# nanoporetech/scrappie

Measured on AMD Instinct MI355X. Metric: raw samples/sec, rgrgr_r94 4k-sample reads, higher is better.
Workload: dtype f32 (3xf16 split products, 22-bit operands, fp32 accumulate)

## Files before the change

### include/scrappie_hip.h

```cpp
#ifndef SCRAPPIE_HIP_H
#define SCRAPPIE_HIP_H

#include <stdbool.h>
#include <stddef.h>
#include <stdint.h>

#ifdef __cplusplus
extern "C" {
#endif


typedef struct {
    char *uuid;
    size_t n;
    size_t start;
    size_t end;
    float *raw;
} raw_table;

typedef struct {
    uint64_t start;
    float length;
    float mean;
    float stdv;
// ... 216 lines not shown
                             const uint64_t *offsets, const uint32_t *lengths, size_t n,
                             const scrappie_hip_params *p);
int scrappie_hip_collect(scrappie_hip_engine *e, const scrappie_hip_params *p,
                         scrappie_hip_call *out, size_t n);

void scrappie_hip_free_calls(scrappie_hip_call *calls, size_t n);

typedef struct { const int *seq; size_t seqlen; const size_t *poslow, *poshigh; } scrappie_hip_map_target;
typedef struct { float score; size_t nblock; int32_t *path; } scrappie_hip_map_result;
int scrappie_hip_read_blocks(scrappie_hip_engine *e, int model, size_t nsample);
int scrappie_hip_model_states(scrappie_hip_engine *e, int model);
int scrappie_hip_map_batch(scrappie_hip_engine *e, int model, const raw_table *reads, const scrappie_hip_map_target *targets,
                           size_t n, const scrappie_hip_params *p, int viterbi, int want_path, scrappie_hip_map_result *out);
void scrappie_hip_free_map_results(scrappie_hip_map_result *r, size_t n);
void scrappie_hip_map_timing(scrappie_hip_engine *e, double out[3]);
size_t scrappie_hip_map_lds_max_seq(void);

typedef struct { const scrappie_hip_map_target *cand; size_t ncand; } scrappie_hip_map_candidates;
typedef struct { float *score; size_t ncand; int best; size_t nblock; int32_t *path; } scrappie_hip_map_multi_result;
int scrappie_hip_map_multi_batch(scrappie_hip_engine *e, int model, const raw_table *reads, const scrappie_hip_map_candidates *cands,
                                 size_t n, const scrappie_hip_params *p, int viterbi, int want_path, scrappie_hip_map_multi_result *out);
void scrappie_hip_free_map_multi_results(scrappie_hip_map_multi_result *r, size_t n);
int scrappie_hip_map_post_multi(const_scrappie_matrix logpost, float stay_pen, float skip_pen, float local_pen,
                                const scrappie_hip_map_target *cand, size_t ncand, int viterbi, float *score);
long scrappie_hip_map_pack_plan(const size_t *seqlen, size_t ncand, size_t pack_cells, int *pack, long long *cell);
size_t scrappie_hip_map_pack_max_cells(void);
void scrappie_hip_map_pack_form_counts(uint64_t forms[4]);

float map_crf_to_sequence_viterbi(const_scrappie_matrix trans, int const *seq, size_t seqlen, int *path);
float map_crf_to_sequence_forward(const_scrappie_matrix trans, int const *seq, size_t seqlen);
float map_crf_to_sequence_viterbi_banded(const_scrappie_matrix trans, int const *seq, size_t seqlen, size_t const *low, size_t const *high, int *path);
float map_crf_to_sequence_forward_banded(const_scrappie_matrix trans, int const *seq, size_t seqlen, size_t const *low, size_t const *high);
int scrappie_hip_map_crf_bounds_sane(const size_t *low, const size_t *high, size_t nblock, size_t seqlen);
int scrappie_hip_map_crf_diagonal_band(size_t nblock, size_t seqlen, size_t halfwidth, size_t *low, size_t *high);
size_t scrappie_hip_map_crf_lds_max_seq(void);
long long scrappie_hip_map_crf_plan_scratch(const size_t *seqlen, const size_t *nblock, size_t n, long long *off);
void scrappie_hip_map_crf_form_counts(uint64_t forms[8]);

int scrappie_hip_map_crf_multi_batch(scrappie_hip_engine *e, int model, const raw_table *reads, const scrappie_hip_map_candidates *cands,
                                     size_t n, const scrappie_hip_params *p, int viterbi, int want_path, scrappie_hip_map_multi_result *out);
int scrappie_hip_map_trans_multi(const_scrappie_matrix trans, const scrappie_hip_map_target *cand, size_t ncand, int viterbi, float *score);
long scrappie_hip_map_crf_pack_plan(const size_t *seqlen, size_t ncand, size_t pack_cells, int *pack, long long *cell);
size_t scrappie_hip_map_crf_pack_max_cells(void);
void scrappie_hip_map_crf_pack_form_counts(uint64_t forms[4]);

typedef struct { const int *seq; size_t seqlen; } scrappie_hip_map_local_target;
typedef struct { float score; size_t nblock, first, last; int32_t *path; } scrappie_hip_map_local_result;
int scrappie_hip_map_local_batch(scrappie_hip_engine *e, int model, const raw_table *reads, const scrappie_hip_map_local_target *targets,
                                 size_t n, const scrappie_hip_params *p, int viterbi, int want_path, scrappie_hip_map_local_result *out);
void scrappie_hip_free_map_local_results(scrappie_hip_map_local_result *r, size_t n);
float map_crf_to_reference_viterbi(const_scrappie_matrix trans, int const *seq, size_t seqlen, size_t *first, size_t *last, int *path);
float map_crf_to_reference_forward(const_scrappie_matrix trans, int const *seq, size_t seqlen);
long long scrappie_hip_map_crf_local_plan(size_t seqlen, size_t nblock, long stride, size_t cap, size_t *first, size_t *ncell, size_t *own,
                                          int *home, long long *scr_off, long long *scr_floats);
size_t scrappie_hip_map_crf_local_stride(size_t seqlen, size_t nblock, long stride);
size_t scrappie_hip_map_crf_local_max_cells(void);
void scrappie_hip_map_crf_local_form_counts(uint64_t forms[8]);

float map_to_reference_viterbi(const_scrappie_matrix logpost, float stay_pen, float skip_pen, float local_pen, int const *seq, size_t seqlen,
                               size_t *first, size_t *last, int *path);
float map_to_reference_forward(const_scrappie_matrix logpost, float stay_pen, float skip_pen, float local_pen, int const *seq, size_t seqlen);
int scrappie_hip_map_post_local_batch(scrappie_hip_engine *e, int model, const raw_table *reads, const scrappie_hip_map_local_target *targets,
                                      size_t n, const scrappie_hip_params *p, int viterbi, int want_path, scrappie_hip_map_local_result *out);
long long scrappie_hip_map_local_plan(size_t seqlen, size_t nblock, size_t nr, long stride, size_t cap, size_t *first, size_t *ncell, size_t *own,
                                      int *home, long long *scr_off, long long *scr_floats);
size_t scrappie_hip_map_local_stride(size_t seqlen, size_t nblock, size_t nr, long stride);
size_t scrappie_hip_map_local_max_cells(size_t nr);
void scrappie_hip_map_local_form_counts(uint64_t forms[8]);

typedef struct { float *score; int32_t *begin, *end; size_t nmotif; float call_score; int best; size_t nblock; } scrappie_hip_find_result;
int scrappie_hip_find_batch(scrappie_hip_engine *e, int model, const raw_table *reads, const scrappie_hip_map_candidates *motifs, size_t n,
                            const scrappie_hip_params *p, int want_pos, scrappie_hip_find_result *out);
void scrappie_hip_free_find_results(scrappie_hip_find_result *r, size_t n);
int find_crf_sequences_viterbi(const_scrappie_matrix trans, const scrappie_hip_map_target *motif, size_t nmotif, float *score, int32_t *begin,
                               int32_t *end, float *call_score);
long scrappie_hip_crf_find_plan(const size_t *seqlen, size_t nmotif, size_t pack_cells, int *pack, long long *cell);
size_t scrappie_hip_crf_find_max_cells(void);
void scrappie_hip_crf_find_form_counts(uint64_t forms[4]);

typedef struct { const float *params; size_t npos, stride; } scrappie_hip_squiggle_target;
typedef struct { float rate, prob_back, local_pen, skip_pen, minscore; } scrappie_hip_squiggle_params;
typedef struct { float score; size_t n; int32_t *path; } scrappie_hip_squiggle_result;
scrappie_hip_squiggle_params scrappie_hip_default_squiggle_params(void);
int scrappie_hip_squiggle_match_batch(scrappie_hip_engine *e, const raw_table *reads, const scrappie_hip_squiggle_target *targets, size_t n,
                                      const scrappie_hip_squiggle_params *p, int viterbi, int want_path, scrappie_hip_squiggle_result *out);
void scrappie_hip_free_squiggle_results(scrappie_hip_squiggle_result *r, size_t n);
void scrappie_hip_squiggle_timing(scrappie_hip_engine *e, double out[3]);
size_t scrappie_hip_squiggle_lds_max_pos(void);
long long scrappie_hip_map_plan_scratch(const size_t *seqlen, const size_t *nblock, size_t n, long long *off);
long long scrappie_hip_squiggle_plan_scratch(const size_t *npos, const size_t *nsample, size_t n, long long *off);
typedef struct { const int32_t *low; size_t width; } scrappie_hip_squiggle_band;
int scrappie_hip_squiggle_match_banded_batch(scrappie_hip_engine *e, const raw_table *reads, const scrappie_hip_squiggle_target *targets,
                                             const scrappie_hip_squiggle_band *bands, size_t n, const scrappie_hip_squiggle_params *p, int viterbi,
                                             int want_path, scrappie_hip_squiggle_result *out);
size_t scrappie_hip_squiggle_diagonal_band(size_t nsample, size_t npos, size_t halfwidth, int32_t *low);
size_t scrappie_hip_squiggle_band_lds_max_width(void);
long long scrappie_hip_squiggle_band_plan(const size_t *npos, const size_t *width, const size_t *nsample, size_t n, int want_path,
                                          long long *scr_off, long long *tb_off);
void scrappie_hip_squiggle_band_form_counts(uint64_t forms[4]);
int scrappie_hip_squiggle_predict_batch(scrappie_hip_engine *e, const char *model, const int *const *seqs, const size_t *n, size_t count,
                                        int transform_units, scrappie_matrix *out);
void scrappie_hip_sqnet_timing(scrappie_hip_engine *e, double out[3]);
size_t scrappie_hip_sqnet_tile(void);
uint64_t scrappie_hip_sqnet_launch_count(void);

long long scrappie_hip_crf_post_plan(const size_t *nblock, size_t n, long long *off);
int scrappie_hip_posterior_crf_batch(scrappie_hip_engine *e, const const_scrappie_matrix *trans, size_t n, scrappie_matrix *out);
int scrappie_hip_basecall_batch_probs(scrappie_hip_engine *e, int model, const raw_table *reads, size_t n, const scrappie_hip_params *p,
                                      scrappie_hip_call *out, scrappie_matrix *probs);
void scrappie_hip_crf_post_timing(scrappie_hip_engine *e, double out[3]);
uint64_t scrappie_hip_crf_post_launch_count(void);
void scrappie_hip_launch_form_counts(uint64_t map_forms[16], uint64_t squig_forms[4]);

int scrappie_hip_set_decoder_input(scrappie_hip_engine *e, const float *d_prob, const uint64_t *prob_off, size_t n_prob);

int scrappie_hip_set_trunk_input(scrappie_hip_engine *e, const float *d_trunk, const uint64_t *trunk_off, size_t n_trunk);

int scrappie_hip_debug_option(scrappie_hip_engine *e, const char *name, int value);
long scrappie_hip_debug_stitch(scrappie_hip_engine *e, const int *path, const float *side, size_t nblock, int nstate, int crf,
                               char *bases, size_t cap, int *pos, int *redo);
long long scrappie_hip_debug_fetch(scrappie_hip_engine *e, const char *what, void *dst, size_t nbytes);
int scrappie_hip_debug_stitch_dwell(scrappie_hip_engine *e, const int *paths, const int *dwells, const size_t *nentry, size_t nread, int ntrail,
                                    const float *prior_num, int nstate, const size_t *cap, char *bases, size_t bases_bytes, int *lengths, int *pos,
                                    int *redo);
size_t scrappie_hip_dwell_capacity(size_t nentry);

scrappie_matrix scrappie_hip_posterior(scrappie_hip_engine *e, int model, const raw_table signal,
                                       float min_prob, float tempW, float tempb, bool return_log);
scrappie_matrix scrappie_hip_trunk(scrappie_hip_engine *e, int model, const raw_table signal, int upto);

int scrappie_hip_event_features(const event_table events, float *out);
scrappie_matrix scrappie_hip_events_posterior(scrappie_hip_engine *e, int model, const float *feature3, size_t nevent,
                                              float min_prob, float tempW, float tempb, bool return_log);

typedef struct { event_table events; int status; } scrappie_hip_event_result;
int scrappie_hip_detect_events_batch(scrappie_hip_engine *e, const raw_table *reads, size_t n, const detector_param *p,
                                     scrappie_hip_event_result *results);
void scrappie_hip_free_event_results(scrappie_hip_event_result *r, size_t n);
void scrappie_hip_event_timing(scrappie_hip_engine *e, double out[3]);
size_t scrappie_hip_event_tile(void);
uint64_t scrappie_hip_event_launch_count(void);
long long scrappie_hip_events_plan_scratch(const size_t *nsample, size_t n, long long *off);
long scrappie_hip_events_plan_launches(const size_t *nsample, size_t n, size_t budget_slots, uint32_t *order, size_t *starts, size_t cap);
int scrappie_hip_basecall_events_batch(scrappie_hip_engine *e, int model, const raw_table *reads, size_t n, const detector_param *p,
                                       const scrappie_hip_params *params, int dwell_correction, scrappie_hip_call *out);
event_table scrappie_hip_detect_events_host(const float *x, size_t n, const detector_param *p, float *tstat1, float *tstat2);

long scrappie_hip_gru_schedule(const int *tile_T, size_t ntile, int ncu, int *nwg, int *capacity,
                               int *lane_off, int *seg, size_t cap);
long scrappie_hip_lane_schedule(const int *tile_T, size_t ntile, int ncu, int lanes_per_wg, int *nwg, int *capacity,
                                int *lane_off, int *seg, size_t cap);

long scrappie_hip_decoder_pieces(const int *tile_T, size_t ntile, int ncu, int *seg, size_t cap);

size_t scrappie_hip_min_samples(scrappie_hip_engine *e, int model);
int scrappie_hip_model_stride(scrappie_hip_engine *e, int model);
void scrappie_hip_set_profiling(scrappie_hip_engine *e, int on);
int scrappie_hip_get_timing(scrappie_hip_engine *e, scrappie_hip_timing *t);
void scrappie_hip_set_max_launch_reads(scrappie_hip_engine *e, size_t n);
void scrappie_hip_set_max_launch_blocks(scrappie_hip_engine *e, size_t n);
long scrappie_hip_plan_groups(const uint32_t *lengths, size_t n, int stride, size_t max_reads, size_t max_blocks,
                              size_t *starts, size_t cap);
unsigned scrappie_hip_host_thread_budget(void);
unsigned scrappie_hip_host_cpu_budget(void);
void *scrappie_hip_device_alloc(scrappie_hip_engine *e, size_t nbytes);
void scrappie_hip_device_free(scrappie_hip_engine *e, void *dptr);
int scrappie_hip_memcpy_h2d(scrappie_hip_engine *e, void *dst, const void *src, size_t nbytes);
int scrappie_hip_synchronize(scrappie_hip_engine *e);

raw_table scrappie_hip_read_raw(const char *filename, bool scale_to_pA);
typedef float *(*scrappie_hip_sample_alloc)(void *ctx, size_t nsample);
raw_table scrappie_hip_read_raw_into(const char *filename, bool scale_to_pA, scrappie_hip_sample_alloc alloc, void *ctx);
int scrappie_hip_have_hdf5(void);
int scrappie_hip_fast5_scaling(const char *filename, float out[3]);

int scrappie_hip_format_fasta(char *buf, size_t buflen, const char *uuid, const char *readname,
                              bool uuid_primary, const char *prefix, const scrappie_hip_call *res,
                              size_t nsample, size_t trim_start, size_t trim_end);
int scrappie_hip_format_sam(char *buf, size_t buflen, const char *uuid, const char *readname,
                            bool uuid_primary, const char *prefix, const scrappie_hip_call *res);

#ifdef __cplusplus
}
#endif
#endif
```

### scrappie_amd/csrc/scrappie_hip.hip

```cpp
#include <hip/hip_runtime.h>
#include <sched.h>

#include <algorithm>
#include <atomic>
#include <cmath>
#include <cstdarg>
#include <cstdio>
#include <cstdlib>
#include <cstring>
#include <mutex>
#include <numeric>
#include <string>
#include <thread>
#include <type_traits>
#include <vector>
#include <chrono>
#include <condition_variable>
#include <deque>
#include <functional>
#include <map>
#include <memory>
#include <set>

#include "scrappie_hip.h"
// ... 32 lines not shown
    }
};

template <auto K>
static DevOnce &attr_once() { static DevOnce once; return once; }
template <auto K, class... A>
static int launch_k(dim3 grid, dim3 block, size_t lds, hipStream_t s, const A &...a) {
    if (auto turn_ = attr_once<K>().first(lds > 48 * 1024))
        HIPCHK(hipFuncSetAttribute((const void *)K, hipFuncAttributeMaxDynamicSharedMemorySize, 160 * 1024));
    hipLaunchKernelGGL(K, grid, block, lds, s, a...);
    return 0;
}

template <int V> using int_c = std::integral_constant<int, V>;
template <int... Vs, class F>
static bool pick_int(int v, int &rc, F &&f) {
    return ((v == Vs && ((rc = f(int_c<Vs>())), true)) || ...);
}
template <class F>
static int pick_bool(F &&f) { return f(); }
template <class F, class... B>
static int pick_bool(F &&f, bool b, B... rest) {
    return b ? pick_bool([&](auto... c) { return f(std::true_type(), c...); }, rest...)
             : pick_bool([&](auto... c) { return f(std::false_type(), c...); }, rest...);
}

struct StampBuf {
    unsigned long long *d = nullptr;
    int calls = 0;
    unsigned long long *dev(size_t words) {
        if (!d) (void)hipMalloc(&d, words * 8);
        return d;
    }
    template <class P>
    void dump_on(int k, hipStream_t s, size_t words, P &&print) {
        if (k && ++calls != k) return;
        (void)sh_stream_wait(s);
        std::vector<unsigned long long> h(words);
        (void)hipMemcpy(h.data(), d, words * 8, hipMemcpyDeviceToHost);
        print(h.data());
    }
};

struct Tunables {
    bool affine_reg, gru_single, gru_stamp, gru_separate, gru_f32, gru_lanes_stamp, proj_stamp, ff_reg, ff_stamp, vit_stamp, ff_separate, fv_single, host_stamp, host_stitch, split_tail, helper_fence, gru_free, gru_barrier, input_order, conv_valu, conv_in_layer, gru32, gru16, gru32_stamp;
    int gru_debug;
    int conv_tchunk;
    double gru_two_ratio;
    bool fake_timeout;
    Tunables() {
        auto on = [](const char *k) { return getenv(k) != nullptr; };
#ifdef SH_EXPERIMENTS
        auto xon = on;
#else
        auto xon = [](const char *) { return false; };
#endif
        affine_reg = xon("SH_AFFINE_REG"); gru_single = xon("SH_GRU_SINGLE"); gru_stamp = xon("SH_GRU_STAMP");
        gru_separate = on("SH_GRU_SEPARATE"); gru_f32 = on("SH_GRU_F32"); gru_lanes_stamp = xon("SH_GRU_LANES_STAMP");
        proj_stamp = xon("SH_PROJ_STAMP"); ff_reg = xon("SH_FF_REG"); ff_stamp = xon("SH_FF_STAMP"); vit_stamp = xon("SH_VIT_STAMP");
        host_stamp = xon("SH_HOST_STAMP");
        gru_free = xon("SH_GRU_FREE");
        gru_barrier = xon("SH_GRU_BARRIER");
        helper_fence = xon("SH_HELPER_FENCE");
        split_tail = on("SH_SPLIT_TAIL");
        host_stitch = on("SH_HOST_STITCH");
        gru32 = xon("SH_GRU32");
        gru16 = xon("SH_GRU16");
        gru32_stamp = xon("SH_GRU32_STAMP");
        conv_in_layer = xon("SH_CONV_IN_LAYER");
        conv_valu = on("SH_CONV_VALU");
        input_order = xon("SH_INPUT_ORDER");
        ff_separate = on("SH_FF_SEPARATE");
        fv_single = on("SH_FV_SINGLE");
        fake_timeout = on("SH_FAKE_HANDOVER_TIMEOUT");
#ifdef SH_EXPERIMENTS
        const char *dm = getenv("SH_GRU_DEBUG");
#else
        const char *dm = nullptr;
#endif
        gru_debug = dm ? atoi(dm) : -1;
        const char *tc = getenv("SH_CONV_TCHUNK");
        conv_tchunk = tc ? std::max(1, std::min(atoi(tc), 256)) : 16;
        const char *tr = getenv("SH_GRU_TWO_RATIO");
        gru_two_ratio = tr ? atof(tr) : 1.8;
    }
};
static const Tunables &tun() { static const Tunables t; return t; }

#ifndef SH_GRU_FREE_DEFAULT
#define SH_GRU_FREE_DEFAULT 0
#endif
#ifndef SH_AFF_NB
#define SH_AFF_NB 3
#endif
#ifndef SH_AFF_NTH
#define SH_AFF_NTH 512
#endif
#ifndef SH_FF_NB
#define SH_FF_NB 4
#endif

static thread_local char g_err[512] = "";
int sh_set_err_v(const char *fmt, va_list ap) {
    vsnprintf(g_err, sizeof(g_err), fmt, ap);
    return -1;
}
extern "C" const char *scrappie_hip_last_error(void) { return g_err; }
extern "C" void sh_set_error(const char *fmt, ...) {
    va_list ap;
    va_start(ap, fmt);
    (void)sh_set_err_v(fmt, ap);
    va_end(ap);
}

#include "sh_eng_weights.inc"
struct DwellJob {
    bool on = false;
    const int *d_dwell = nullptr;
    std::vector<uint64_t> off;
    std::vector<float> num;
    std::vector<const int *> host;
};

struct PostJob {
    bool on = false;
    std::vector<scrappie_matrix *> dst;
};

struct LaunchGroup {
    PostJob post;
    std::vector<long long> post_off;
    long long npost = 0;
    DwellJob dw;
    size_t n = 0, npad = 0, ntile = 0;
    long long ncb = 0;
    long long nseq = 0;
    long long nhp = 0;
    std::vector<int> order;
    std::vector<int> rT, rN;
    std::vector<long long> tile_boff;
    std::vector<long long> seq_off, hp_off, bases_off;
    long long nbases_cap = 0;
    bool dev_stitch = false;
    bool dev_pos = false;
    int model = -1;
    bool hp_on = false;
    bool valid = false;
    int gru_nwg = 0;
    int gru1_nwg = 0;
    bool gru_two = false;
    int gru32_nwg = 0;
    int gru32x2_nwg = 0;
    int vit_nwg = 0;
    const float *d_signal = nullptr;
    std::vector<uint64_t> in_off;
    std::vector<uint32_t> in_len;
    scrappie_hip_params params{};
};

struct BatchReq {
    scrappie_hip_engine *e = nullptr;
    int model = 0;
    const raw_table *reads = nullptr;
    size_t n = 0;
    scrappie_hip_params p{};
    scrappie_hip_call *out = nullptr;
    int rc = -1;
    std::string err;
    int phase = 0;
};
struct BatchCoalescer : ShCoalescer<BatchReq> { BatchCoalescer() { target_pct = 100; window_mul = 4; } };

struct PostStage { HBuf h; DBuf d; std::atomic<int> users{0}; };

struct DpBufs {
    DBuf rd, tb, scr, score, final_state, path_off, paths;
    HBuf h;
    int ensure(size_t n, size_t rec_bytes, long long tb_words, long long scr_floats, long long path_len, size_t h_bytes = 0, size_t fs_bytes = 4) {
        return (rd.ensure(n * rec_bytes) || tb.ensure((size_t)tb_words * 4 + 16) || scr.ensure((size_t)scr_floats * 4 + 16) || score.ensure(n * 4 + 16) ||
                final_state.ensure(n * fs_bytes + 16) || path_off.ensure(n * 8) || paths.ensure((size_t)path_len * 4 + 16) ||
                h.ensure(std::max(h_bytes, n * 4 + (size_t)path_len * 4))) ? -1 : 0;
    }
};

enum SpanField { F_CONV = 0, F_AFFINE, F_GRU, F_FF, F_DECODE, F_BACKTRACE, F_TOTAL, F_FUSED, F_STITCH,
                 F_WAIT, F_LEAD,
                 F_COUNT };

struct Slot {
    LaunchGroup lg;
    bool pending = false;
    hipEvent_t ev[48] = {};
    int nev = 0;
    struct Span { int field, i, j; };
    std::vector<Span> spans;
    scrappie_hip_timing timing{};
    hipEvent_t done = nullptr;
    hipEvent_t kdone = nullptr;
    hipEvent_t hdone = nullptr;
    hipEvent_t pdone = nullptr;
    hipEvent_t up = nullptr;
    DBuf d_meta, d_signal, d_gflag;
    DBuf d_conv;
    DBuf d_bad;
    DBuf d_edge;
    DBuf d_fscore, d_seq, d_hp;
    DBuf d_pos, d_bases, d_blen, d_redo;
    DBuf d_dwmeta; HBuf h_dwmeta;
    DBuf d_post, d_postoff; HBuf h_post, h_postoff;
    hipEvent_t pev[5] = {};
    HBuf h_meta, h_sig, h_err, h_bad, h_edge, h_seq, h_score, h_hp, h_pos, h_bases, h_blen, h_redo;
    size_t pinned_bytes() const {
        size_t tot = 0;
        for (const HBuf *h : {&h_meta, &h_sig, &h_err, &h_bad, &h_edge, &h_seq, &h_score, &h_hp, &h_pos, &h_bases, &h_blen, &h_redo, &h_dwmeta, &h_post, &h_postoff}) tot += h->cap;
        return tot;
    }
    bool create_events() {
        bool ok = true;
        for (auto &x : ev) ok &= hipEventCreate(&x) == hipSuccess;
        for (hipEvent_t *x : {&done, &kdone, &hdone, &pdone, &up}) ok &= hipEventCreateWithFlags(x, hipEventDisableTiming) == hipSuccess;
        return ok;
    }
    ~Slot() {
        for (auto &x : ev) if (x) (void)hipEventDestroy(x);
        for (auto &x : pev) if (x) (void)hipEventDestroy(x);
        for (hipEvent_t x : {done, kdone, hdone, pdone, up}) if (x) (void)hipEventDestroy(x);
    }
};

struct AltInput {
    const float *data = nullptr;
    std::vector<uint64_t> off;
    DBuf d_off;
    uint64_t key = 0; bool valid = false;
    explicit operator bool() const { return data != nullptr; }
    int set(const char *who, const float *d, const uint64_t *o, size_t n) {
        valid = false;
        if (!d) { data = nullptr; off.clear(); return 0; }
        if (!o || n == 0) return set_err("%s: no offsets", who);
        data = d; off.assign(o, o + n);
        return 0;
    }
};

struct scrappie_hip_engine {
    int device = 0;
    hipStream_t stream = nullptr;
    hipStream_t cstream = nullptr;
    hipStream_t ustream = nullptr;
    hipStream_t pstream = nullptr;
    size_t total_mem = (size_t)64 << 30;
    size_t max_launch_blocks = 0;
    std::vector<Model *> models;
    size_t max_launch_reads = 16384;
    bool profiling = false;
    scrappie_hip_timing timing{};
    bool ev_ok = false;
    Slot slots[2];
    int cur = 0;
    int oldest = 0;
    Slot &current() { return slots[cur]; }
    Slot &other(const Slot &sl) { return slots[&sl == &slots[0] ? 1 : 0]; }
    int index(const Slot &sl) const { return (int)(&sl - slots); }
    bool any_pending() const { return slots[0].pending || slots[1].pending; }
    void drain() {
        (void)sh_stream_wait(pstream); (void)sh_stream_wait(stream); (void)sh_stream_wait(cstream);
        slots[0].pending = slots[1].pending = false;
    }
    DBuf d_hstate, d_vstate, d_vflag;
    DBuf d_act[3];
    DBuf d_xaff, d_E, d_sums, d_tb, d_tbend, d_fstate;
    int ncu = 256;
    bool handover = true;
    AltInput alt_prob; DBuf d_Ealt, d_sums_alt;
    AltInput alt_trunk; DBuf d_act_alt;
    bool dbg_ff_separate = false;
    bool dbg_fv_single = false;
    bool dbg_dump_final = false;
    int dbg_fail_run = 0;
    bool dbg_redo_all = false;
    bool dbg_dwell_tight = false;
    int dbg_gru_tiles = 0;
    int dbg_decoder_cus = 0;
    bool dbg_force_f32 = false;
    int dbg_gru32 = -1;
    scrappie_hip_engine *tail = nullptr;
    scrappie_hip_engine *tail2 = nullptr;
    bool is_tail = false;
    int tail_mode = -1;
    int dbg_fail_tail = 0;
    double mem_frac = 0.7;
    struct Blob { std::string name; std::vector<unsigned char> bytes; bool force_f32; };
    std::vector<Blob> blobs;
    unsigned long long n_tail_calls = 0, n_tail_reads = 0;
    struct TailTicket {
        long id = 0; int model = 0; scrappie_hip_params p{};
        std::vector<raw_table> reads; std::vector<scrappie_hip_call> calls;
        std::vector<float> own;
        int rc = 0; std::string err; bool done = false;
    };
    std::thread tail_th, tail_th2;
    bool tail_th_live = false, tail_th2_live = false, tail_stop = false;
    int tail_busy = 0;
    std::mutex tail_mu;
    std::condition_variable tail_cv;
    std::deque<std::shared_ptr<TailTicket>> tail_q;
    std::map<long, std::shared_ptr<TailTicket>> tail_open;
    long tail_next = 1;
    unsigned long long n_redo_tail = 0;
    unsigned long long n_tail_groups = 0;
    unsigned host_thread_budget = 0;
    unsigned long long n_redo = 0;
    struct Carry { bool live = false; int slot = 0; std::vector<uint32_t> perm; scrappie_hip_call *out = nullptr; scrappie_hip_params p{}; } carry;
    std::mutex mu;
    double tail_frac = 0.3;
    double dbg_tail_free_frac = 0;
    BatchCoalescer batch_co;
    ShPresence batch_presence;
    PostStage post_stage[2]; unsigned post_turn = 0;
    HBuf h_dec_in, h_dec_out; DBuf d_dec[7];
    HBuf h_crf_in, h_crf_out; DBuf d_crf[4];
    DpBufs dp_map; DBuf d_map_seq, d_map_band, d_map_post;
    DBuf d_mpk_rd, d_mpk_cell, d_mpk_first, d_mpk_score; HBuf h_mpk;
    int map_pack_cells = -1;
    DpBufs dp_mcl; DBuf d_mcl_seq, d_mcl_first;
    DpBufs dp_ml; DBuf d_ml_seq, d_ml_lohi;
    int map_local_stride = -1;
    DBuf d_cfd_rd, d_cfd_cell, d_cfd_score, d_cfd_pos, d_cfd_call; HBuf h_cfd;
    int crf_find_cells = -1;
    DBuf d_mcp_rd, d_mcp_cell, d_mcp_score; HBuf h_mcp;
    int map_crf_pack_cells = -1;
    int map_crf_local_stride = -1;
    double map_ms[3] = {0, 0, 0};
    DpBufs dp_sq; DBuf d_sq_sig, d_sq_tab;
    double squig_ms[3] = {0, 0, 0};
    DBuf d_sqn[2]; HBuf h_sqn;
    double sqnet_ms[3] = {0, 0, 0};
    DBuf d_ev_sig, d_ev_rd, d_ev_sum, d_ev_sumsq, d_ev_t1, d_ev_t2, d_ev_peaks, d_ev_np, d_ev_off, d_ev_out; HBuf h_ev, h_ev_out;
    double event_ms[3] = {0, 0, 0};
    HBuf h_cp_in, h_cp_out; DBuf d_cp_in, d_cp_out;
    double crf_post_ms[3] = {0, 0, 0};
    size_t dbg_events_budget = 0;
    size_t dbg_sqnet_budget = 0;
    size_t dbg_squig_budget = 0;
    std::mutex call_mu;
    ~scrappie_hip_engine() {
        for (Model *m : models) delete m;
        for (hipStream_t st : {stream, cstream, ustream, pstream}) if (st) (void)hipStreamDestroy(st);
    }
};

static int pick_mt(int mtiles) {
    for (int mt : {6, 4, 3, 2}) if (mtiles % mt == 0) return mt;
    return 1;
}

static void hw_queue_default() {
    static std::once_flag once;
    std::call_once(once, [] { (void)setenv("GPU_MAX_HW_QUEUES", "8", 0); });
}

static int device_count(hipError_t *why) {
    hw_queue_default();
    int n = 0;
    const hipError_t rc = hipGetDeviceCount(&n);
    if (why) *why = rc;
    return rc == hipSuccess ? n : 0;
}
extern "C" int scrappie_hip_device_count(void) { return device_count(nullptr); }
extern "C" int scrappie_hip_device_numa_node(int device) { return sh_device_numa_node(device); }

extern "C" scrappie_hip_engine *scrappie_hip_engine_create(int device) {
    hipError_t why = hipSuccess;
    int n = device_count(&why);
    if (n <= 0) {
        std::string first, second;
        if (FILE *maps = fopen("/proc/self/maps", "r")) {
            char line[1024];
            while (fgets(line, sizeof line, maps)) {
                const char *path = strchr(line, '/');
                if (!path || !strstr(path, "libamdhip64")) continue;
                std::string s(path, strcspn(path, "\n"));
                if (first.empty()) first = s; else if (s != first && second.empty()) second = s;
            }
            fclose(maps);
        }
        if (!second.empty())
            set_err("no HIP device visible (hipGetDeviceCount: %s): two HIP runtimes are loaded in this process (%s and %s); load the "
                    "other user of HIP (e.g. import torch) before this library, see INTEGRATION.md", hipGetErrorString(why), first.c_str(), second.c_str());
        else set_err("no HIP device visible (hipGetDeviceCount: %s)", hipGetErrorString(why));
        return nullptr;
    }
    if (device < 0 || device >= n) { set_err("device %d out of range (have %d)", device, n); return nullptr; }
    if (hipSetDevice(device) != hipSuccess) { set_err("hipSetDevice(%d) failed", device); return nullptr; }
    hipDeviceProp_t prop;
    int ncu = 256;
    size_t total_mem = (size_t)64 << 30;
    if (hipGetDeviceProperties(&prop, device) == hipSuccess) {
        if (prop.multiProcessorCount > 0) ncu = prop.multiProcessorCount;
        if (prop.totalGlobalMem > 0) total_mem = prop.totalGlobalMem;
        if (strncmp(prop.gcnArchName, "gfx950", 6) != 0) {
            set_err("device %d is %s; this library is built for gfx950 (MI355X) only", device, prop.gcnArchName);
            return nullptr;
        }
    }
    (void)tun();
    scrappie_hip_engine *e = new scrappie_hip_engine();
    e->device = device;
    e->ncu = ncu;
    e->total_mem = total_mem;
    { const char *h = getenv("SCRAPPIE_HIP_HANDOVER"); if (h && atoi(h) == 0) e->handover = false; }
    int prio_lo = 0, prio_hi = 0;
    (void)hipDeviceGetStreamPriorityRange(&prio_lo, &prio_hi);
#ifdef SH_EXPERIMENTS
    if (!getenv("SH_STREAM_PRIO"))
#endif
    prio_lo = prio_hi = 0;
    if (hipStreamCreateWithPriority(&e->stream, hipStreamNonBlocking, prio_hi) != hipSuccess ||
        hipStreamCreateWithPriority(&e->cstream, hipStreamNonBlocking, prio_lo) != hipSuccess ||
        hipStreamCreateWithPriority(&e->pstream, hipStreamNonBlocking, prio_lo) != hipSuccess ||
        hipStreamCreateWithFlags(&e->ustream, hipStreamNonBlocking) != hipSuccess) {
        set_err("hipStreamCreate failed");
        delete e;
        return nullptr;
    }
    e->ev_ok = true;
    for (Slot &sl : e->slots) if (!sl.create_events()) e->ev_ok = false;
    return e;
}

extern "C" void scrappie_hip_engine_destroy(scrappie_hip_engine *e) {
    if (!e) return;
    if (e->tail_th_live) {
        { std::lock_guard<std::mutex> lk(e->tail_mu); e->tail_stop = true; }
        e->tail_cv.notify_all();
        e->tail_th.join();
// ... 41 lines not shown
```

### scrappie_amd/csrc/sh_decode.h

```cpp
#ifndef SH_DECODE_H
#define SH_DECODE_H

struct ShVitArgs {
    const float *E;
    const float *sums;
    long long strideT;
    int strideQ, strideB;
    int want_log;
    float min_prob, stay_pen, skip_pen, local_pen;
    int use_slip;
    unsigned *tb;
    int *tb_end;
    int *final_state;
    float *final_score;
    float *hp_side;
    const long long *hp_off;
    unsigned long long *dbg;
    const ShGruSegD *seg;
    float *vstate;
    unsigned *flag;
    unsigned *err;
    int dump_final;
};

__device__ __forceinline__ void argmax_merge(float &v, int &i, float ov, int oi) {
    const bool take = (ov > v) | ((ov == v) & (oi < i));
    v = take ? ov : v;
    i = take ? oi : i;
}

__device__ __forceinline__ void rows_argmax(float &bv, int &bi) {
    float ov = __shfl_xor(bv, 16); int oi = __shfl_xor(bi, 16);
    argmax_merge(bv, bi, ov, oi);
    ov = __shfl_xor(bv, 32); oi = __shfl_xor(bi, 32);
    argmax_merge(bv, bi, ov, oi);
}

#ifndef SH_FVT_GAP
#define SH_FVT_GAP 4.76837158203125e-07f
#endif
#ifndef SH_MAX4_ASM
#define SH_MAX4_ASM 1
#endif
__device__ __forceinline__ float d_max4(const f32x4 v) {
#if !SH_MAX4_ASM
    return __builtin_fmaxf(__builtin_fmaxf(v[0], v[1]), __builtin_fmaxf(v[2], v[3]));
#endif
    float t;
    asm("v_max3_f32 %0, %1, %2, %3" : "=v"(t) : "v"(v[0]), "v"(v[1]), "v"(v[2]));
    asm("v_max_f32 %0, %1, %2" : "=v"(t) : "v"(t), "v"(v[3]));
    return t;
}

#define SH_CODE_LT(E, codes, a, b, x)                                                                                       \
    asm("v_cmp_lt_f32 vcc, %1, %2\n\tv_cndmask_b32_sdwa %0, %0, %3, vcc dst_sel:BYTE_" #E                                   \
        " dst_unused:UNUSED_PRESERVE src0_sel:BYTE_" #E " src1_sel:BYTE_0"                                                  \
        : "+v"(codes) : "v"(a), "v"(b), "v"(x) : "vcc")

#ifndef SH_VIT_RING
#define SH_VIT_RING 4
#endif
template <int NTH, int PPT, bool FIN, bool SLIP, bool SKIP0>
__global__ __launch_bounds__(NTH, NTH / 256) void k_viterbi(ShVitArgs a, ShMeta md) {
    constexpr int RING = (PPT >= SH_VIT_RING) ? SH_VIT_RING : PPT;
    constexpr int QSTR = NTH / 16, NW = NTH / 64;
    constexpr int NQ = QSTR * PPT, NH = 4 * NQ;
    constexpr int NSKIP = NH / 16, NSLIP = (NH / 64 > 0) ? NH / 64 : 1;
    extern __shared__ __attribute__((aligned(16))) float smem[];
    float *scA = smem;
    float *scB = scA + NH * 16;
    float *skv = scB + NH * 16;
    int *ski = (int *)(skv + NSKIP * 16);
    float *slv = (float *)(ski + NSKIP * 16);
    int *sli = (int *)(slv + NSLIP * 16);
    float *redv = (float *)(sli + NSLIP * 16);
    int *redi = (int *)(redv + 2 * NW * 16);

    const int tid = threadIdx.x, b = tid & 15, qq = tid >> 4, wave = tid >> 6, lane = tid & 63;
    const float mp = a.min_prob, mpm1 = 1.0f - a.min_prob;
    const float slip_pen = (float)(2.0 * a.skip_pen);
    constexpr bool slip = SLIP && (NH / 64 > 0);
    unsigned long long vA = 0, vB = 0, vC = 0, vD = 0, vt0 = 0, vt1;
    long long vblocks = 0;
#define VSTAMP(acc) do { if (a.dbg) { vt1 = __builtin_readcyclecounter(); acc += vt1 - vt0; vt0 = vt1; } } while (0)

    int tile = blockIdx.x, s0 = 0, s1 = -1, ord = 0;
    if (a.seg) { const ShGruSegD sg = a.seg[blockIdx.x]; tile = sg.tile; s0 = sg.s0; s1 = sg.s1; ord = sg.pad; }
    tile = __builtin_amdgcn_readfirstlane(tile); s0 = __builtin_amdgcn_readfirstlane(s0); s1 = __builtin_amdgcn_readfirstlane(s1);
    const int Tt = __builtin_amdgcn_readfirstlane(md.tile_T[tile]);
    if (s1 < 0) s1 = Tt;
    const long long boff = __builtin_amdgcn_readfirstlane((int)md.tile_boff[tile]);
    const int rd = tile * 16 + b;
    const int myT = md.rT[rd];
    float pstart = 0.0f, pend = -SH_BIG;
    if (s0 == 0) {
#pragma unroll
        for (int i = 0; i < PPT; i++)
            *(f32x4 *)(scA + ((qq + QSTR * i) * 16 + b) * 4) = (f32x4){-SH_BIG, -SH_BIG, -SH_BIG, -SH_BIG};
        if (lane < 16) { redv[wave * 16 + b] = -SH_BIG - a.local_pen; redi[wave * 16 + b] = 4 * wave; }
    } else {
        if (tid == 0) {
            if (!sh_wait_flag(a.flag + tile, (unsigned)ord, a.err)) __hip_atomic_store(a.err, 1u, __ATOMIC_RELAXED, __HIP_MEMORY_SCOPE_AGENT);
        }
        __syncthreads();
        __builtin_amdgcn_fence(__ATOMIC_ACQUIRE, "agent");
        const float *vst = a.vstate + (long long)tile * (NH * 16 + 32);
        float bv = -INFINITY;
        int bi = 0x7fffffff;
#pragma unroll
        for (int i = 0; i < PPT; i++) {
            const int Q = qq + QSTR * i;
            const f32x4 pv = *(const f32x4 *)(vst + (Q * 16 + b) * 4);
            *(f32x4 *)(scA + (Q * 16 + b) * 4) = pv;
            {
                const float ve = __builtin_fmaxf(__builtin_fmaxf(pv[0], pv[1]), __builtin_fmaxf(pv[2], pv[3])) - a.local_pen;
                bi = (ve > bv) ? Q : bi;
                bv = __builtin_fmaxf(bv, ve);
            }
        }
        pstart = vst[NH * 16 + b];
        pend = vst[NH * 16 + 16 + b];
        float ov = __shfl_xor(bv, 16); int oi = __shfl_xor(bi, 16);
        argmax_merge(bv, bi, ov, oi);
        ov = __shfl_xor(bv, 32); oi = __shfl_xor(bi, 32);
        argmax_merge(bv, bi, ov, oi);
        if (lane < 16) { redv[((s0 & 1) * NW + wave) * 16 + b] = bv; redi[((s0 & 1) * NW + wave) * 16 + b] = bi; }
    }
    __syncthreads();
    float *cur = scA, *nxt = scB;

    f32x4 ring[RING];
    float stay_nx = 0.f, sum_nx = 1.f;
    float hp_nx[4] = {0.f, 0.f, 0.f, 0.f};
    const bool hp_lane = FIN && a.hp_side && qq == 0;
    auto fetch = [&](int t) {
        const float *Ecb = a.E + (boff + t) * a.strideT + b * a.strideB;
        stay_nx = Ecb[NQ * a.strideQ];
        if (FIN) sum_nx = a.sums[(boff + t) * 16 + b];
        if (hp_lane) {
#pragma unroll
            for (int k = 0; k < 4; k++) {
                const int s = k * ((NH - 1) / 3);
                hp_nx[k] = Ecb[(s >> 2) * a.strideQ + (s & 3)];
            }
        }
    };
    const unsigned eofs = (unsigned)(b * a.strideB + qq * a.strideQ);
    const unsigned tofs = (unsigned)(qq * 16 + b);
    auto qload = [&](int t, int i) {
        const float *base = a.E + (boff + t) * a.strideT + (long long)(QSTR * i) * a.strideQ;
        return *(const f32x4 *)(base + eofs);
    };
    if (s1 > s0) {
        fetch(s0);
#pragma unroll
        for (int i = 0; i < RING; i++) ring[i] = qload(s0, i);
    }
    if (a.dbg) vt0 = __builtin_readcyclecounter();
    vblocks += s1 - s0;

    for (int t = s0; t < s1; t++) {
        const long long cb = boff + t;
        const int par = t & 1;
        float stay_lp = stay_nx;
        const float rmf = d_rcp(sum_nx) * mpm1;

        for (int p = tid; p < NSKIP * 16; p += NTH) {
            const int j = p >> 4, bb = p & 15;
            float v = cur[((j >> 2) * 16 + bb) * 4 + (j & 3)];
            int ri = 0;
#pragma unroll
// ... 811 lines not shown
```

### scrappie_amd/csrc/sh_decode_teams.h

```cpp
#ifndef SH_DECODE_TEAMS_H
#define SH_DECODE_TEAMS_H

#ifndef SH_FVT_WBUF
#define SH_FVT_WBUF 3
#endif
#ifndef SH_FVT_PROD_PRIO
#define SH_FVT_PROD_PRIO 1
#endif
#ifndef SH_FVT_ABL
#define SH_FVT_ABL 0
#endif
#ifndef SH_FVT_FLIP
#define SH_FVT_FLIP 3
#endif
#ifndef SH_FVT_STAMP
#ifdef SH_EXPERIMENTS
#define SH_FVT_STAMP 1
#else
#define SH_FVT_STAMP 0
#endif
#endif
__device__ __forceinline__ unsigned long long end_key(float v, int i) {
    const unsigned u = __builtin_bit_cast(unsigned, v);
    const unsigned hi = u ^ ((unsigned)((int)u >> 31) | 0x80000000u);
    return ((unsigned long long)hi << 32) | (unsigned)~i;
}
__device__ __forceinline__ void end_unkey(unsigned long long k, float &v, int &i) {
    const unsigned hi = (unsigned)(k >> 32);
    v = __builtin_bit_cast(float, hi ^ (~(unsigned)((int)hi >> 31) | 0x80000000u));
    i = (int)~(unsigned)k;
}

#define SH_FVT_NTH 768
#define SH_FVT_LDS_FLOATS (1024 * 16 + 64 * 256 + 2 * 64 * 16 + 2 * 2 * 8 * 16 + 4 * 9 * 16 + 65 * 16 + 2 * 3 * 512 + 3 * 2 * 4 * 4 + 16 * 4 + 4 * 16)

template <bool SKIP0, bool DIV, bool NOCLAMP = false>
__global__ __launch_bounds__(SH_FVT_NTH) void k_ff_viterbi_teams(ShFfArgs f, ShVitArgs a, ShMeta md) {
    static_assert(!(DIV && NOCLAMP), "with temperatures the clamp stays");
    constexpr int NCW = 8, NPW = 4, PPT = 8, NQ = 256, NH = 1024, KS = 3, KQ = 6, TPP = 16, HT = 8, NG = 9, WB = SH_FVT_WBUF;
    static_assert(SH_SUM_GROUP == HT, "half a pass of a producer is one row-sum group");
    static_assert(WB >= 2 && WB <= 4, "weight ring");
    extern __shared__ __attribute__((aligned(16))) float smem[];
    float *sc = smem;
    float *ring = sc + NH * 16;
    float *skk = ring + 64 * 256;
    float *redv = skk + 2 * 64 * 16;
    int *redi = (int *)(redv + 2 * NCW * 16);
    typedef __attribute__((address_space(3))) unsigned long long *ldsk;
    ldsk redk = (ldsk)redv;
    float *gsum = (float *)(redi + 2 * NCW * 16);
    float *sBias = gsum + 4 * NG * 16;
    unsigned *xp = (unsigned *)(sBias + 65 * 16);
    unsigned *sStay = xp + 2 * KS * 512;
    float *rec = (float *)(sStay + KS * 2 * 4 * 4);
    float *pendl = rec + 16 * 4;
    int *pT = (int *)(pendl + 16);
    long long *phpo = (long long *)(pT + 16);

    const int tid = threadIdx.x, lane = tid & 63, b = lane & 15, q = lane >> 4;
    const int wave = __builtin_amdgcn_readfirstlane(tid >> 6);
    const bool decoder = wave < NCW;
    const float mp = a.min_prob, mpm1 = 1.0f - a.min_prob;
    const float lbound = (mp > 0.0f) ? 1.0e-3f - __logf(mp) : INFINITY;
    const float lbgap = lbound * SH_FVT_GAP;
    unsigned long long vA = 0, vB = 0, vC = 0, vD = 0, vt0 = 0, vt1 = 0;
    (void)vt0; (void)vt1;
#undef VSTAMP
#if SH_FVT_STAMP
#define VSTAMP(acc) do { if (a.dbg) { vt1 = __builtin_readcyclecounter(); acc += vt1 - vt0; vt0 = vt1; } } while (0)
#else
#define VSTAMP(acc) do { } while (0)
#endif

    if (tid < KS * 2 * 4 * 4) sStay[tid] = f.wpiece[(long long)(64) * KS * 512 + (tid >> 4) * 256 + ((tid >> 2) & 3) * 64 + (tid & 3)];
    for (int j = tid; j < 65 * 16; j += SH_FVT_NTH) sBias[j] = f.bfrag[((j >> 4) * 64 + ((j >> 2) & 3) * 16) * 4 + (j & 3)];

    int tile = blockIdx.x, s0 = 0, s1 = -1, ord = 0;
    if (a.seg) { const ShGruSegD sg = a.seg[blockIdx.x]; tile = sg.tile; s0 = sg.s0; s1 = sg.s1; ord = sg.pad; }
    tile = __builtin_amdgcn_readfirstlane(tile); s0 = __builtin_amdgcn_readfirstlane(s0); s1 = __builtin_amdgcn_readfirstlane(s1);
    const int Tt = __builtin_amdgcn_readfirstlane(md.tile_T[tile]);
    if (s1 < 0) s1 = Tt;
    const long long boff = __builtin_amdgcn_readfirstlane((int)md.tile_boff[tile]);
    const int rd = tile * 16 + b;
    int myT = md.rT[rd];
    asm volatile("" : "+v"(myT));
    const long long hpo = a.hp_side ? a.hp_off[rd] : 0;
    float pstart = 0.0f, pend = -SH_BIG;

    const int cw = decoder ? wave : 0;
    float *myq = sc + cw * 256 + lane * 4;
    const float *mye = ring + cw * 512 + lane * 4;
    const float *mysrc = sc + cw * 64 + b * 4 + q;
#define SH_FVT_MT(i) (16 * ((i) >> 1) + 8 * ((i) & 1))

    if (s0 == 0) {
        if (decoder) {
#pragma unroll
            for (int i = 0; i < PPT; i++) *(f32x4 *)(myq + SH_FVT_MT(i) * 256) = (f32x4){-SH_BIG, -SH_BIG, -SH_BIG, -SH_BIG};
            if (wave == 0 && lane < 16) { redk[b] = end_key(-SH_BIG - a.local_pen, 0); redk[16 + b] = 0; }
        }
    } else {
        if (tid < 32) redk[tid] = 0;
        if (tid == 0) {
            if (!sh_wait_flag(a.flag + tile, (unsigned)ord, a.err)) __hip_atomic_store(a.err, 1u, __ATOMIC_RELAXED, __HIP_MEMORY_SCOPE_AGENT);
        }
        __syncthreads();
        __builtin_amdgcn_fence(__ATOMIC_ACQUIRE, "agent");
        if (decoder) {
            const float *vst = a.vstate + (long long)tile * (NH * 16 + 32);
            float bv = -INFINITY;
            int bi = 0x7fffffff;
#pragma unroll
            for (int i = 0; i < PPT; i++) {
                const int Q = 4 * (SH_FVT_MT(i) + cw) + q;
                const f32x4 pv = *(const f32x4 *)(vst + (Q * 16 + b) * 4);
                *(f32x4 *)(myq + SH_FVT_MT(i) * 256) = pv;
                {
                    const float ve = __builtin_fmaxf(__builtin_fmaxf(pv[0], pv[1]), __builtin_fmaxf(pv[2], pv[3])) - a.local_pen;
                    bi = (ve > bv) ? Q : bi;
                    bv = __builtin_fmaxf(bv, ve);
                }
            }
            pstart = vst[NH * 16 + b];
            float ov = __shfl_xor(bv, 16); int oi = __shfl_xor(bi, 16);
            argmax_merge(bv, bi, ov, oi);
            ov = __shfl_xor(bv, 32); oi = __shfl_xor(bi, 32);
            argmax_merge(bv, bi, ov, oi);
            if (lane < 16) __hip_atomic_fetch_max(redk + b, end_key(bv, bi), __ATOMIC_RELAXED, __HIP_MEMORY_SCOPE_WORKGROUP);
        } else if (wave == NCW + NPW - 1) pend = (a.vstate + (long long)tile * (NH * 16 + 32))[NH * 16 + 16 + b];
    }

    if (!decoder) {
        const int pw = wave - NCW;
#if SH_FVT_PROD_PRIO
        __builtin_amdgcn_s_setprio(SH_FVT_PROD_PRIO);
#endif
        const unsigned *wmine = f.wpiece + (long long)(TPP * pw) * KS * 512;
        ShSplit W[WB][KS];
        const unsigned lofs = (unsigned)lane * 4u;
        typedef const __attribute__((address_space(1))) unsigned *gu32;
        typedef const __attribute__((address_space(1))) u32x4 *gu32x4;
        gu32 wp = (gu32)wmine;
        auto w_load = [&](int k) {
            static_assert(KS == 3, "two bases per tile: immediate offsets reach 4095 bytes");
            gu32 b0 = wp, b1 = wp + 1024;
            asm volatile("" : "+s"(b0), "+s"(b1));
            W[(k % HT) % WB][0].p1 = __builtin_bit_cast(f16x8, *(gu32x4)(b0 + lofs));
            W[(k % HT) % WB][0].p2 = __builtin_bit_cast(f16x8, *(gu32x4)(b0 + 256 + lofs));
            W[(k % HT) % WB][1].p1 = __builtin_bit_cast(f16x8, *(gu32x4)(b0 + 512 + lofs));
            W[(k % HT) % WB][1].p2 = __builtin_bit_cast(f16x8, *(gu32x4)(b0 + 768 + lofs));
            W[(k % HT) % WB][2].p1 = __builtin_bit_cast(f16x8, *(gu32x4)(b1 + lofs));
            W[(k % HT) % WB][2].p2 = __builtin_bit_cast(f16x8, *(gu32x4)(b1 + 256 + lofs));
            wp = (k == TPP - 1) ? (gu32)wmine : wp + KS * 512;
            asm volatile("" : "+s"(wp));
        };
        auto w_prime = [&](int k0) {
#pragma unroll
            for (int k = 0; k < WB - 1; k++) w_load(k0 + k);
        };
        const int xks = pw < KS ? pw : KS - 1;
        f32x4 xr[2][2];
        auto xraw_load = [&](int u) {
#pragma unroll
            for (int j = 0; j < 2; j++) {
                const float *p = f.in + ((boff + min(u + j, s1 - 1)) * KQ + 2 * xks) * 256;
                xr[j][0] = *(const f32x4 *)(p + lofs);
                xr[j][1] = *(const f32x4 *)(p + 256 + lofs);
            }
        };
        auto xp_publish = [&]() {
            if (pw < KS) {
#pragma unroll
                for (int j = 0; j < 2; j++) {
                    f32x4 v0 = xr[j][0], v1 = xr[j][1];
                    if (DIV) { v0 = v0 / f.in_div; v1 = v1 / f.in_div; }
                    const ShSplit sp = split8(v0, v1);
                    unsigned *d = xp + (j * KS + pw) * 512 + lane * 4;
                    *(u32x4 *)d = __builtin_bit_cast(u32x4, sp.p1);
                    *(u32x4 *)(d + 256) = __builtin_bit_cast(u32x4, sp.p2);
                }
            }
        };
        auto e_of = [&](float acc) { return DIV ? d_exp((acc * SH_OINV) / f.out_div) : NOCLAMP ? d_exp_acc_inrange(acc) : d_exp_acc(acc); };
        auto group_out = [&](float part, int u, int g) {
            const float v = rows_sum(part);
            if (lane < 16) gsum[((u & 3) * NG + g) * 16 + b] = v;
        };
        float *myring = ring + (TPP * pw) * 256 + lane * 4;
        auto s1_half = [&](auto Hc, int u) {
            constexpr int H = decltype(Hc)::value;
#if defined(SH_FVT_DBG_ROLE) && SH_FVT_DBG_ROLE == 1
            return;
#endif
            const float *mybias = sBias + (TPP * pw + HT * H) * 16 + 4 * q;
            ShSplit bp[2][KS];
#pragma unroll
            for (int j = 0; j < 2; j++)
#pragma unroll
                for (int ks = 0; ks < KS; ks++) bp[j][ks] = load_pieces(xp + (j * KS + ks) * 512, lane);
            float part0 = 0.0f, part1 = 0.0f;
            auto tile_out = [&](int k, const f32x4 &acc0, const f32x4 &acc1) {
                f32x4 ex0, ex1;
#pragma unroll
                for (int r = 0; r < 4; r++) { ex0[r] = e_of(acc0[r]); ex1[r] = e_of(acc1[r]); }
                part0 += (ex0[0] + ex0[1]) + (ex0[2] + ex0[3]);
                part1 += (ex1[0] + ex1[1]) + (ex1[2] + ex1[3]);
                if (SH_FVT_ABL & 8) {
#pragma unroll
                    for (int r = 0; r < 4; r++) { ex0[r] = fin_log(ex0[r], mpm1, mp); ex1[r] = fin_log(ex1[r], mpm1, mp); }
                }
                *(f32x4 *)(myring + (2 * k) * 256) = ex0;
                *(f32x4 *)(myring + (2 * k + 1) * 256) = ex1;
            };
#pragma unroll
            for (int k = 0; k < HT; k++) {
                f32x4 acc0 = *(const f32x4 *)(mybias + k * 16), acc1 = acc0;
                if (k + WB - 1 < HT) w_load(HT * H + k + WB - 1);
                const ShSplit (&A)[KS] = W[k % WB];
#pragma unroll
                for (int ks = 0; ks < KS; ks++) { acc0 = mfma16(A[ks].p1, bp[0][ks].p2, acc0); acc1 = mfma16(A[ks].p1, bp[1][ks].p2, acc1); }
#pragma unroll
                for (int ks = 0; ks < KS; ks++) { acc0 = mfma16(A[ks].p2, bp[0][ks].p1, acc0); acc1 = mfma16(A[ks].p2, bp[1][ks].p1, acc1); }
#pragma unroll
                for (int ks = 0; ks < KS; ks++) { acc0 = mfma16(A[ks].p1, bp[0][ks].p1, acc0); acc1 = mfma16(A[ks].p1, bp[1][ks].p1, acc1); }
                tile_out(k, acc0, acc1);
                __builtin_amdgcn_sched_barrier(0);
            }
            group_out(part0, u, 2 * pw + H);
            group_out(part1, u + 1, 2 * pw + H);
            if (H == 1 && pw == NPW - 1) {
                ShSplit Ws[KS];
#pragma unroll
                for (int ks = 0; ks < KS; ks++) {
                    const u32x4 a1 = *(const u32x4 *)(sStay + ((ks * 2 + 0) * 4 + q) * 4), a2 = *(const u32x4 *)(sStay + ((ks * 2 + 1) * 4 + q) * 4);
                    const u32x4 z = {0u, 0u, 0u, 0u};
                    Ws[ks].p1 = __builtin_bit_cast(f16x8, b == 0 ? a1 : z);
                    Ws[ks].p2 = __builtin_bit_cast(f16x8, b == 0 ? a2 : z);
                }
#pragma unroll
                for (int j = 0; j < 2; j++) {
                    f32x4 acc = *(const f32x4 *)(sBias + 64 * 16 + 4 * q);
                    acc = split_dot<KS>(Ws, bp[j], acc);
                    f32x4 ex;
#pragma unroll
                    for (int r = 0; r < 4; r++) ex[r] = (4 * q + r < 1) ? e_of(acc[r]) : 0.0f;
                    group_out((ex[0] + ex[1]) + (ex[2] + ex[3]), u + j, NG - 1);
                }
            }
        };
        auto per_read = [&](const int t, auto par_c) {
            constexpr int par = decltype(par_c)::value;
            int ln = (int)__builtin_amdgcn_mbcnt_hi(~0u, __builtin_amdgcn_mbcnt_lo(~0u, 0u));
            asm volatile("" : "+v"(ln));
            const int b = ln & 15;
            const bool low = ln < 16;
            const int myT = pT[b];
            float pend = pendl[b];
            float tot = 0.0f;
#pragma unroll
            for (int w = 0; w < NG; w++) tot += gsum[((t & 3) * NG + w) * 16 + b];
            const float rmf = d_rcp(tot) * mpm1;
            const float stay_lp = fin_log(gsum[((t & 3) * NG + NG - 1) * 16 + b], rmf, mp);
            const bool active = t < myT;
            if (a.hp_side && active && low) (a.hp_side + (phpo[b] + t) * 5)[4] = stay_lp;
            const float rm = active ? rmf : 0.0f;
            const float mpx = active ? mp : 0.0f;
            const float stay_v = active ? stay_lp - a.stay_pen : 0.0f;
            const float stay_act = stay_lp - a.stay_pen;
            const float hold = fmaxf(-a.local_pen, stay_act);
            if (low) *(f32x4 *)(rec + b * 4) = (f32x4){rm, mpx, stay_v, hold};
            float ev; int ei;
            end_unkey(redk[par * 16 + b], ev, ei);
            redk[par * 16 + b] = 0;
            const f32x4 q4 = *(const f32x4 *)(sc + ((ei & (NQ - 1)) * 16 + b) * 4);
            int e0 = 3;
            e0 = (q4[2] - a.local_pen == ev) ? 2 : e0;
            e0 = (q4[1] - a.local_pen == ev) ? 1 : e0;
            e0 = (q4[0] - a.local_pen == ev) ? 0 : e0;
            const int tbe_in = 4 * ei + e0;
            float nend = pend + hold;
            const bool enter_end = ev > nend;
            nend = enter_end ? ev : nend;
            if (active && low) a.tb_end[(boff + t) * 16 + b] = enter_end ? tbe_in : NH + 1;
            if (active && low) pendl[b] = nend;
        };
        const bool serial = pw == NPW - 1;
        if (serial && lane < 16) { pendl[b] = pend; pT[b] = myT; phpo[b] = hpo; }
        const std::integral_constant<int, 0> H0{};
        const std::integral_constant<int, 1> H1{};

        const bool any = s1 > s0;
        if (any) xraw_load(s0);
        __syncthreads();
        if (any) { xp_publish(); w_prime(0); }
        lds_barrier();
        if (any) s1_half(H0, s0);
        lds_barrier();
        if (any) w_prime(HT);
        lds_barrier();
        if (any) { s1_half(H1, s0); __builtin_amdgcn_sched_barrier(0); xraw_load(s0 + 2); }
        lds_barrier();
        if (a.dbg) vt0 = __builtin_readcyclecounter();
        for (int t = s0; t < s1; t += 2) {
            const bool more = (t + 2 < s1) && !(SH_FVT_ABL & 1);
            if (serial) { per_read(t, H0); __builtin_amdgcn_sched_barrier(0); }
            if (more) { xp_publish(); w_prime(0); }
            VSTAMP(vA);
            lds_barrier();
            VSTAMP(vB);
            if (more) s1_half(H0, t + 2);
            VSTAMP(vC);
            lds_barrier();
            VSTAMP(vD);
            if (serial && t + 1 < s1) { per_read(t + 1, H1); __builtin_amdgcn_sched_barrier(0); }
            if (more) w_prime(HT);
            VSTAMP(vA);
            lds_barrier();
            VSTAMP(vB);
            if (more) s1_half(H1, t + 2);
            __builtin_amdgcn_sched_barrier(0);
            xraw_load(t + 4);
            VSTAMP(vC);
            lds_barrier();
            VSTAMP(vD);
        }
        if (serial && lane < 16 && s1 < Tt) (a.vstate + (long long)tile * (NH * 16 + 32))[NH * 16 + 16 + b] = pendl[b];
        if (s1 < Tt) __builtin_amdgcn_fence(__ATOMIC_RELEASE, "agent");
        __syncthreads();
        if (s1 >= Tt) __syncthreads();
        if (a.dbg && lane == 0) { unsigned long long *d = a.dbg + ((long long)blockIdx.x * 12 + wave) * 8; d[0] = vA; d[1] = vB; d[2] = vC; d[3] = vD; d[4] = (unsigned long long)(s1 - s0); }
        return;
    }
    {
        f32x4 eN[2][PPT];
        auto drain = [&](auto a0, auto s0c, auto a1, auto s1c) {
            constexpr int A0 = decltype(a0)::value, S0 = decltype(s0c)::value, A1 = decltype(a1)::value, S1 = decltype(s1c)::value;
#pragma unroll
            for (int rl = 0; rl < PPT / 2; rl++) { eN[A0][2 * rl + S0] = *(const f32x4 *)(mye + rl * 4096); eN[A1][2 * rl + S1] = *(const f32x4 *)(mye + rl * 4096 + 256); }
        };
        const std::integral_constant<int, 0> I0{};
        const std::integral_constant<int, 1> I1{};
        __syncthreads();
        lds_barrier();
        lds_barrier();
        drain(I0, I0, I1, I0);
        lds_barrier();
        lds_barrier();
        if (a.dbg) vt0 = __builtin_readcyclecounter();
        const unsigned tofs = (unsigned)lane;
        auto block = [&](const int t, auto first_c) {
            constexpr bool FIRST = decltype(first_c)::value;
            const f32x4 (&e)[PPT] = eN[FIRST ? 0 : 1];
            const long long cb = boff + t;
            constexpr int par = FIRST ? 0 : 1;
#if defined(SH_FVT_DBG_ROLE) && SH_FVT_DBG_ROLE == 2
            lds_barrier(); lds_barrier(); return;
#endif
            if (!FIRST && t >= s1) {
                drain(I0, I0, I0, I1);
                lds_barrier(); lds_barrier();
                return;
            }

            float sv[PPT];
            int sr[PPT];
#pragma unroll
            for (int i = 0; i < PPT; i++) {
                float v = mysrc[SH_FVT_MT(i) * 64];
                int ri = (int)SH_TB_STEP;
                if (!(SH_FVT_ABL & 2)) {
#pragma unroll
                    for (int r = 1; r < 4; r++) {
                        const float c = mysrc[(r * 64 + SH_FVT_MT(i)) * 64];
                        const bool up = v < c;
                        v = up ? c : v;
                        ri = up ? (int)SH_TB_STEP + r : ri;
                    }
                }
                sv[i] = v; sr[i] = ri;
                if (i == PPT / 2 - 1) __builtin_amdgcn_sched_barrier(0);
            }
#pragma unroll
            for (int c = 0; c < 2; c++) {
                constexpr int KOFS = (int)SH_TB_SKIP - 4 * (int)SH_TB_STEP;
                float v = sv[c];
                int ri = 4 * sr[c] + KOFS;
                if (!(SH_FVT_ABL & 2)) {
#pragma unroll
                    for (int rl = 1; rl < 4; rl++) argmax_merge(v, ri, sv[2 * rl + c], 4 * sr[2 * rl + c] + (rl + KOFS));
                }
                *(f32x2 *)(skk + ((32 * c + 4 * cw + q) * 16 + b) * 2) = (f32x2){v, __builtin_bit_cast(float, ri)};
            }
            static_assert(SH_TB_STEP + 3u < 8u, "a step code in three bits");
            unsigned srp = 0;
#pragma unroll
            for (int i = 0; i < PPT; i++) srp |= (unsigned)sr[i] << (3 * i);
            __builtin_amdgcn_sched_barrier(0);
            if (FIRST) drain(I0, I1, I1, I1);
            else drain(I0, I0, I0, I1);
            VSTAMP(vA);
            lds_barrier();
            VSTAMP(vB);

            const f32x4 rcd = *(const f32x4 *)(rec + b * 4);
            const float rm = rcd[0], mpx = rcd[1], stay_v = rcd[2], hold = rcd[3];
            const bool active = t < myT;
            const unsigned long long actmask = __builtin_amdgcn_ballot_w64(active);
            const float nstart = pstart + hold;
            float bv = -INFINITY;
            int bi = 0x7fffffff;
            typedef __attribute__((address_space(1))) unsigned *gtb;
            gtb tb0 = (gtb)a.tb + ((cb * NQ + 4 * cw) * 16 + 1024), tb1 = tb0 + 2048;
            asm volatile("" : "+s"(tb0), "+s"(tb1));
            f32x4 pv_n; f32x2 kk_n;
            auto q_fetch = [&](int i) {
                pv_n = *(const f32x4 *)(myq + SH_FVT_MT(i) * 256);
                kk_n = *(const f32x2 *)(skk + ((SH_FVT_MT(i) + cw) * 16 + b) * 2);
            };
            q_fetch(0);
            float hpv[4] = {0.f, 0.f, 0.f, 0.f};
#pragma unroll
            for (int i = 0; i < PPT; i++) {
                const int QB = 4 * (SH_FVT_MT(i) + cw);
                const int Q = QB + q;
                const f32x4 pv = pv_n;
                const float kv = kk_n[0];
                const float krf = kk_n[1];
                const unsigned cskip = __builtin_bit_cast(unsigned, krf);
                if (i + 1 < PPT) q_fetch(i + 1);
                f32x4 l4;
#pragma unroll
                for (int k = 0; k < 4; k++) l4[k] = (SH_FVT_ABL & 24) ? e[i][k] : fin_log(e[i][k], rm, mpx);
#pragma unroll
                for (int k = 0; k < 4; k++) {
                    const int s = k * ((NH - 1) / 3), sq = s >> 2;
                    if (i == 2 * (sq >> 6) + ((sq >> 5) & 1)) hpv[k] = l4[s & 3];
                }
                const float svi = sv[i];
                const unsigned cstep = (srp >> (3 * i)) & 7u;
                const unsigned cstart = SH_TB_START;
                unsigned codes;
                f32x4 ns;
                static_assert(SH_TB_STAY == 0u && SH_TB_STEP + 3u < 256u && SH_TB_SKIP + 15u < 256u && SH_TB_START < 256u,
                              "SH_FVT_LT_FIRST copies all 32 bits of x (cstep, cskip, cstart or cm): every code register is zero above its low byte");
#define SH_FVT_LT_FIRST(E, codes, a, b, x)                                                                      \
                asm("v_cmp_lt_f32 vcc, %1, %2\n\tv_cndmask_b32 %0, 0, %3, vcc" : "=v"(codes) : "v"(a), "v"(b), "v"(x) : "vcc")
#define SH_FVT_STATE(E, LT1)                                                                                    \
                {                                                                                               \
                    float s_ = pv[E] + stay_v;                                                  \
                    const float st = l4[E] + svi;                                           \
                    LT1(E, codes, s_, st, cstep);                                                               \
                    s_ = __builtin_fmaxf(s_, st);                                                               \
                    const float sk = SKIP0 ? l4[E] + kv : (l4[E] + kv) - a.skip_pen;        \
                    SH_CODE_LT(E, codes, s_, sk, cskip);                                                        \
                    s_ = __builtin_fmaxf(s_, sk);                                                               \
                    const float fs = pstart + l4[E];                                  \
                    SH_CODE_LT(E, codes, s_, fs, cstart);                                                       \
                    s_ = __builtin_fmaxf(s_, fs);                                                               \
                    ns[E] = s_;                                                                                 \
                }
                bool fast = false;
                float m = 0.f;
                unsigned cm = cstart;
                if (SKIP0) {
                    m = __builtin_fmaxf(__builtin_fmaxf(svi, kv), pstart);
                    const float md = __builtin_amdgcn_fmed3f(svi, kv, pstart);
                    static_assert(SH_FVT_GAP == 4.76837158203125e-07f, "the fused threshold needs a power of two");
                    const unsigned long long unclear = __builtin_amdgcn_fcmpf(m - md, __builtin_fmaf(__builtin_fabsf(m), SH_FVT_GAP, lbgap), 13 );
                    fast = (unclear & actmask) == 0;
                    cm = (kv == m) ? cskip : cm;
                    cm = (svi == m) ? cstep : cm;
                }
                if (__builtin_expect(fast, true)) {
#define SH_FVT_FAST(E, LT1)                                                                                    \
                    {                                                                                           \
                        const float s_ = pv[E] + stay_v;                                        \
                        const float mv = l4[E] + m;                           \
                        LT1(E, codes, s_, mv, cm);                                                              \
                        ns[E] = __builtin_fmaxf(s_, mv);                                                        \
                    }
                    SH_FVT_FAST(0, SH_FVT_LT_FIRST) SH_FVT_FAST(1, SH_CODE_LT) SH_FVT_FAST(2, SH_CODE_LT) SH_FVT_FAST(3, SH_CODE_LT)
#undef SH_FVT_FAST
                } else { SH_FVT_STATE(0, SH_FVT_LT_FIRST) SH_FVT_STATE(1, SH_CODE_LT) SH_FVT_STATE(2, SH_CODE_LT) SH_FVT_STATE(3, SH_CODE_LT) }
#undef SH_FVT_STATE
#undef SH_FVT_LT_FIRST
                *(f32x4 *)(myq + SH_FVT_MT(i) * 256) = ns;
                gtb tbq = i < PPT / 2 ? tb0 : tb1;
                asm volatile("" : "+s"(tbq));
                if (!(SH_FVT_ABL & 4)) (tbq + (512 * (i % (PPT / 2)) - 1024))[tofs] = codes;
                else asm volatile("" :: "v"(codes));
                {
                    const float ve = d_max4(ns) - a.local_pen;
                    bi = (ve > bv) ? Q : bi;
                    bv = __builtin_fmaxf(bv, ve);
                }
                __builtin_amdgcn_sched_barrier(0);
#if SH_FVT_FLIP
                if (cw >= 4) { if (i == PPT - 1) __builtin_amdgcn_s_setprio(1); else if (i == SH_FVT_FLIP - 1) __builtin_amdgcn_s_setprio(0); }
#endif
            }
            if (active) pstart = nstart;
            if (a.hp_side && active) {
#pragma unroll
                for (int k = 0; k < 4; k++) {
                    const int sq = (k * ((NH - 1) / 3)) >> 2;
                    if (cw == ((sq >> 2) & 7) && q == (sq & 3)) (a.hp_side + (hpo + t) * 5)[k] = hpv[k];
                }
            }
            {
                rows_argmax(bv, bi);
                if (lane < 16) __hip_atomic_fetch_max(redk + ((par ^ 1) * 16 + b), end_key(bv, bi), __ATOMIC_RELAXED, __HIP_MEMORY_SCOPE_WORKGROUP);
            }
            VSTAMP(vC);
            lds_barrier();
            VSTAMP(vD);
        };
        for (int t = s0; t < s1; t += 2) {
            block(t, std::true_type{});
            block(t + 1, std::false_type{});
#pragma unroll
            for (int rl = 0; rl < PPT / 2; rl++) eN[1][2 * rl] = eN[0][2 * rl + 1];
        }
    }

    if (s1 < Tt) {
        if (decoder) {
            float *vst = a.vstate + (long long)tile * (NH * 16 + 32);
#pragma unroll
            for (int i = 0; i < PPT; i++) {
                const int Q = 4 * (SH_FVT_MT(i) + cw) + q;
                *(f32x4 *)(vst + (Q * 16 + b) * 4) = *(const f32x4 *)(myq + SH_FVT_MT(i) * 256);
            }
            if (tid < 16) vst[NH * 16 + b] = pstart;
        }
        __builtin_amdgcn_fence(__ATOMIC_RELEASE, "agent");
        __syncthreads();
        if (tid == 0) __hip_atomic_store(a.flag + tile, (unsigned)ord + 1u, __ATOMIC_RELEASE, __HIP_MEMORY_SCOPE_AGENT);
    } else {
        float bv = -INFINITY;
        int bi = 0x7fffffff;
        if (decoder) {
#pragma unroll
            for (int i = 0; i < PPT; i++) {
                const int Q = 4 * (SH_FVT_MT(i) + cw) + q;
                const f32x4 pv = *(const f32x4 *)(myq + SH_FVT_MT(i) * 256);
#pragma unroll
                for (int k = 0; k < 4; k++) argmax_merge(bv, bi, pv[k], 4 * Q + k);
            }
            float ov = __shfl_xor(bv, 16); int oi = __shfl_xor(bi, 16);
            argmax_merge(bv, bi, ov, oi);
            ov = __shfl_xor(bv, 32); oi = __shfl_xor(bi, 32);
            argmax_merge(bv, bi, ov, oi);
        }
        __syncthreads();
        if (decoder && lane < 16) { redv[wave * 16 + b] = bv; redi[wave * 16 + b] = bi; }
        __syncthreads();
        if (tid < 16) {
            pend = pendl[b];
            float ev = redv[b]; int ei = redi[b];
            for (int w = 1; w < NCW; w++) argmax_merge(ev, ei, redv[w * 16 + b], redi[w * 16 + b]);
            if (pstart > ev) { ev = pstart; ei = NH; }
            if (pend > ev) { ev = pend; ei = NH + 1; }
            a.final_state[rd] = ei;
            a.final_score[rd] = ev;
        }
        if (a.dump_final && a.vstate && decoder) {
            float *vst = a.vstate + (long long)tile * (NH * 16 + 32);
#pragma unroll
            for (int i = 0; i < PPT; i++) {
                const int Q = 4 * (SH_FVT_MT(i) + cw) + q;
                *(f32x4 *)(vst + (Q * 16 + b) * 4) = *(const f32x4 *)(myq + SH_FVT_MT(i) * 256);
            }
            if (tid < 16) { vst[NH * 16 + b] = pstart; vst[NH * 16 + 16 + b] = pend; }
        }
    }
    if (a.dbg && lane == 0) { unsigned long long *d = a.dbg + ((long long)blockIdx.x * 12 + wave) * 8; d[0] = vA; d[1] = vB; d[2] = vC; d[3] = vD; d[4] = (unsigned long long)(s1 - s0); }
#undef VSTAMP
#undef SH_FVT_MT
}

#endif
```

### scrappie_amd/csrc/sh_eng_batch.inc

```

#ifndef SH_CHAIN_NS
#define SH_CHAIN_NS 11400.0
#endif
#ifndef SH_WORK_NS
#define SH_WORK_NS 3.5
#endif
extern "C" long scrappie_hip_plan_tail(const uint32_t *lengths, size_t n, int stride, size_t max_long_blocks, unsigned char *is_long) {
    if ((!lengths && n) || stride < 1 || !is_long) return -1;
    memset(is_long, 0, n);
    if (n < 2) return 0;
    double W = 0;
    std::vector<uint32_t> T(n);
    for (size_t i = 0; i < n; i++) { T[i] = (uint32_t)(((unsigned long long)lengths[i] + stride - 1) / stride); W += T[i]; }
    const double thr = std::max(4096.0, W * SH_WORK_NS / SH_CHAIN_NS);
    std::vector<uint32_t> cand;
    for (size_t i = 0; i < n; i++) if ((double)T[i] > thr) cand.push_back((uint32_t)i);
    if (cand.empty() || cand.size() == n) return 0;
    std::stable_sort(cand.begin(), cand.end(), [&](uint32_t a, uint32_t b) { return T[a] > T[b]; });
    double blocks = 0, work = 0;
    long cnt = 0;
    for (size_t k = 0; k < cand.size(); k++) {
        if (k % 16 == 0) { if (max_long_blocks && blocks + T[cand[k]] > (double)max_long_blocks) break; blocks += T[cand[k]]; }
        if (work + T[cand[k]] > 0.15 * W) break;
        work += T[cand[k]];
        is_long[cand[k]] = 1; cnt++;
    }
    return cnt;
}

static int basecall_batch_one(scrappie_hip_engine *e, int model, const raw_table *reads, size_t n, const scrappie_hip_params *p, scrappie_hip_call *out,
                              scrappie_matrix *probs = nullptr);

static bool tail_two_helpers();
static double tail_mem_frac() {
    static const double f = [] { const char *v = getenv("SCRAPPIE_HIP_TAIL_MEM"); const double x = v ? atof(v) : 0; return x > 0 && x <= 0.4 ? x : (tail_two_helpers() ? 0.15 : 0.3); }();
    return f;
}
static bool tail_two_helpers() {
    static const bool on = [] { const char *v = getenv("SCRAPPIE_HIP_TAIL"); return v && atoi(v) == 2; }();
    return on;
}
static bool tail_enabled(const scrappie_hip_engine *e) {
    if (e->is_tail) return false;
    if (e->tail_mode >= 0) return e->tail_mode != 0;
    static const bool env_on = [] { const char *v = getenv("SCRAPPIE_HIP_TAIL"); return !(v && atoi(v) == 0); }();
    return env_on;
}

static scrappie_hip_engine *make_helper(scrappie_hip_engine *e) {
    scrappie_hip_engine *t = scrappie_hip_engine_create(e->device);
    if (!t) return nullptr;
    t->is_tail = true;
    for (const auto &b : e->blobs) {
        t->dbg_force_f32 = b.force_f32;
        const int want = scrappie_hip_find_model(e, b.name.c_str());
        if (load_model_mem_one(t, b.name.c_str(), b.bytes.data(), b.bytes.size()) != want) { scrappie_hip_engine_destroy(t); set_err("helper engine: model '%s' did not load at index %d", b.name.c_str(), want); return nullptr; }
    }
    return t;
}
static void sync_helper(scrappie_hip_engine *e, scrappie_hip_engine *t) {
    t->handover = e->handover; t->max_launch_reads = e->max_launch_reads; t->max_launch_blocks = e->max_launch_blocks;
    t->dbg_ff_separate = e->dbg_ff_separate; t->dbg_fv_single = e->dbg_fv_single; t->dbg_gru32 = e->dbg_gru32; t->dbg_gru_tiles = e->dbg_gru_tiles; t->dbg_decoder_cus = e->dbg_decoder_cus; t->dbg_redo_all = e->dbg_redo_all;
    t->profiling = false;
}
static scrappie_hip_engine *tail_engine(scrappie_hip_engine *e) {
    if (!e->tail) {
        (void)hipSetDevice(e->device);
        double frac = tail_mem_frac();
        size_t fr = 0, tot = 0;
        if (hipMemGetInfo(&fr, &tot) == hipSuccess && e->total_mem) frac = std::min(frac, 0.85 * (double)fr / (double)e->total_mem);
        if (e->dbg_tail_free_frac > 0) frac = std::min(frac, e->dbg_tail_free_frac);
        if (frac < 0.03) { e->tail_mode = 0; return nullptr; }
        e->tail = make_helper(e);
        if (!e->tail) return nullptr;
        e->mem_frac = 0.45; e->tail->mem_frac = frac; e->tail_frac = frac;
    }
    std::lock_guard<std::mutex> lk(e->tail_mu);
    if (e->tail_busy == 0) {
        sync_helper(e, e->tail);
        if (e->tail2) sync_helper(e, e->tail2);
        if (e->dbg_fail_tail) { e->tail->dbg_fail_run = e->dbg_fail_tail; e->dbg_fail_tail = 0; }
    }
    return e->tail;
}

typedef std::shared_ptr<scrappie_hip_engine::TailTicket> TicketPtr;
static void tail_worker(scrappie_hip_engine *e, scrappie_hip_engine *helper) {
    for (;;) {
        std::unique_lock<std::mutex> lk(e->tail_mu);
        e->tail_cv.wait(lk, [&] { return e->tail_stop || !e->tail_q.empty(); });
        if (e->tail_q.empty()) break;
        std::vector<TicketPtr> batch;
        const TicketPtr f = e->tail_q.front();
        while (!e->tail_q.empty() && e->tail_q.front()->model == f->model && memcmp(&e->tail_q.front()->p, &f->p, sizeof f->p) == 0) {
            batch.push_back(e->tail_q.front());
            e->tail_q.pop_front();
        }
        e->tail_busy++;
        lk.unlock();
        std::vector<raw_table> all;
        for (const TicketPtr &t : batch) all.insert(all.end(), t->reads.begin(), t->reads.end());
        std::vector<scrappie_hip_call> calls(all.size());
        const int rc = basecall_batch_one(helper, f->model, all.data(), all.size(), &f->p, calls.data());
        const std::string err = rc ? std::string(g_err) : std::string();
        lk.lock();
        size_t at = 0;
        for (const TicketPtr &t : batch) {
            t->rc = rc; t->err = err;
            if (!rc) t->calls.assign(calls.begin() + (long)at, calls.begin() + (long)(at + t->reads.size()));
            at += t->reads.size();
            t->done = true;
        }
        e->n_tail_groups++;
        e->n_redo_tail += helper->n_redo; helper->n_redo = 0;
        e->tail_busy--;
        lk.unlock();
        e->tail_cv.notify_all();
    }
}
static TicketPtr tail_submit(scrappie_hip_engine *e, int model, const scrappie_hip_params &p, std::vector<raw_table> &&reads, std::vector<float> &&own = std::vector<float>()) {
    if (!e->tail2 && tail_two_helpers()) {
        bool busy;
        { std::lock_guard<std::mutex> lk(e->tail_mu); busy = e->tail_busy > 0 || !e->tail_q.empty(); }
        if (busy) {
            scrappie_hip_engine *t2 = make_helper(e);
            if (t2) { t2->mem_frac = 0.15; sync_helper(e, t2); std::lock_guard<std::mutex> lk(e->tail_mu); e->tail2 = t2; }
            (void)hipSetDevice(e->device);
        }
    }
    TicketPtr t = std::make_shared<scrappie_hip_engine::TailTicket>();
    t->model = model; t->p = p; t->reads = std::move(reads);
    t->own = std::move(own);
    {
        std::lock_guard<std::mutex> lk(e->tail_mu);
        t->id = e->tail_next++;
        e->tail_open[t->id] = t;
        e->tail_q.push_back(t);
        if (!e->tail_th_live) { e->tail_th = std::thread(tail_worker, e, e->tail); e->tail_th_live = true; }
        else if (e->tail2 && !e->tail_th2_live) { e->tail_th2 = std::thread(tail_worker, e, e->tail2); e->tail_th2_live = true; }
    }
    e->tail_cv.notify_all();
    return t;
}
static void tail_wait(scrappie_hip_engine *e, const TicketPtr &t) {
    std::unique_lock<std::mutex> lk(e->tail_mu);
    e->tail_cv.wait(lk, [&] { return t->done; });
}

static long tail_plan_len(scrappie_hip_engine *e, Model *m, const uint32_t *len, size_t n, std::vector<unsigned char> &is_long) {
    is_long.assign(n, 0);
    if (!tail_enabled(e) || n < 2 || e->alt_prob || e->alt_trunk || e->blobs.size() != e->models.size() || e->dbg_fail_run) return 0;
    const int unit = m->arch == 3 ? 1 : std::max(m->stride, 1);
    const size_t tail_cap = (size_t)((e->tail ? e->tail_frac : tail_mem_frac()) * (double)e->total_mem) / bytes_per_block(m, !decoder_fused(e, m));
    long nl = scrappie_hip_plan_tail(len, n, unit, e->max_launch_blocks ? e->max_launch_blocks : tail_cap, is_long.data());
    if (nl > 0 && !e->tail) {
        if (!tail_engine(e)) {
            if (tail_enabled(e)) return -1;
            is_long.assign(n, 0);
            return 0;
        }
        if (e->tail_frac < tail_mem_frac() && !e->max_launch_blocks) {
            const size_t cap2 = (size_t)(e->tail_frac * (double)e->total_mem) / bytes_per_block(m, !decoder_fused(e, m));
            nl = scrappie_hip_plan_tail(len, n, unit, cap2, is_long.data());
        }
    }
    if (nl > 0 && !tail_engine(e)) return -1;
    return nl;
}
static long tail_plan(scrappie_hip_engine *e, Model *m, const raw_table *reads, size_t n, std::vector<unsigned char> &is_long) {
    const size_t per = m->arch == 3 ? (size_t)m->nfeat : 1;
    std::vector<uint32_t> len(n);
    for (size_t i = 0; i < n; i++) {
        const raw_table &rt = reads[i];
        len[i] = (uint32_t)(((rt.raw && rt.end > rt.start) ? rt.end - rt.start : 0) / per);
    }
    return tail_plan_len(e, m, len.data(), n, is_long);
}

extern "C" long scrappie_hip_basecall_batch_deferred(scrappie_hip_engine *e, int model, const raw_table *reads, size_t n,
                                                     const scrappie_hip_params *p, scrappie_hip_call *out, unsigned char *deferred) {
    if (!e || !reads || !out || !deferred) return set_err("basecall_batch_deferred: null argument");
    Model *m = get_model(e, model);
    if (!m) return -1;
    std::vector<unsigned char> is_long;
    const long nl = tail_plan(e, m, reads, n, is_long);
    if (nl < 0) return -1;
    memset(deferred, 0, n);
    if (nl == 0) return basecall_batch_one(e, model, reads, n, p, out) ? -1 : 0;
    std::vector<raw_table> rl, rr;
    std::vector<size_t> ir;
    for (size_t i = 0; i < n; i++) { if (is_long[i]) rl.push_back(reads[i]); else { rr.push_back(reads[i]); ir.push_back(i); } }
    scrappie_hip_params dp = scrappie_hip_default_params();
    const size_t nlong = rl.size();
    auto tk = tail_submit(e, model, p ? *p : dp, std::move(rl));
    std::vector<scrappie_hip_call> orr(rr.size());
    const int rc_main = basecall_batch_one(e, model, rr.data(), rr.size(), p, orr.data());
    for (size_t i = 0; i < n; i++) { out[i].score = NAN; out[i].nblock = 0; out[i].basecall = nullptr; out[i].basecall_length = 0; out[i].pos = nullptr; }
    if (rc_main) {
        const std::string keep = g_err;
        tail_wait(e, tk);
        if (!tk->rc) scrappie_hip_free_calls(tk->calls.data(), tk->calls.size());
        { std::lock_guard<std::mutex> lk(e->tail_mu); e->tail_open.erase(tk->id); }
        return set_err("%s", keep.c_str());
    }
    for (size_t k = 0; k < ir.size(); k++) out[ir[k]] = orr[k];
    for (size_t i = 0; i < n; i++) deferred[i] = is_long[i];
    e->n_tail_calls++; e->n_tail_reads += nlong;
    return tk->id;
}
static long device_deferred(scrappie_hip_engine *e, int model, const float *d_signal, const uint64_t *offsets, const uint32_t *lengths, size_t n,
                            const scrappie_hip_params *p, scrappie_hip_call *out, unsigned char *deferred, bool stream);
extern "C" long scrappie_hip_basecall_device_deferred(scrappie_hip_engine *e, int model, const float *d_signal, const uint64_t *offsets,
                                                      const uint32_t *lengths, size_t n, const scrappie_hip_params *p, scrappie_hip_call *out,
                                                      unsigned char *deferred) {
    return device_deferred(e, model, d_signal, offsets, lengths, n, p, out, deferred, false);
// ... 348 lines not shown
```

### scrappie_amd/csrc/sh_eng_debug.inc

```

extern "C" int scrappie_hip_set_decoder_input(scrappie_hip_engine *e, const float *d_prob, const uint64_t *prob_off, size_t n_prob) {
    if (!e) return set_err("set_decoder_input: null engine");
    if (e->any_pending()) return set_err("set_decoder_input: launch groups are in flight");
    return e->alt_prob.set("set_decoder_input", d_prob, prob_off, n_prob);
}

extern "C" int scrappie_hip_set_trunk_input(scrappie_hip_engine *e, const float *d_trunk, const uint64_t *trunk_off, size_t n_trunk) {
    if (!e) return set_err("set_trunk_input: null engine");
    if (e->any_pending()) return set_err("set_trunk_input: launch groups are in flight");
    return e->alt_trunk.set("set_trunk_input", d_trunk, trunk_off, n_trunk);
}

static scrappie_hip_engine *default_engine();

extern "C" int scrappie_hip_debug_option(scrappie_hip_engine *e, const char *name, int value) {
    if (!e && name && (!strcmp(name, "map_pack_cells") || !strcmp(name, "map_crf_local_stride") || !strcmp(name, "map_local_stride") || !strcmp(name, "crf_find_cells") || !strcmp(name, "map_crf_pack_cells"))) e = default_engine();
    if (!e || !name) return set_err("debug_option: null argument");
    if (e->any_pending()) return set_err("debug_option: launch groups are in flight");
    if (!strcmp(name, "ff_separate")) e->dbg_ff_separate = value != 0;
    else if (!strcmp(name, "fv_single")) e->dbg_fv_single = value != 0;
    else if (!strcmp(name, "dump_final")) e->dbg_dump_final = value != 0;
    else if (!strcmp(name, "fail_run")) e->dbg_fail_run = value;
    else if (!strcmp(name, "redo_all")) e->dbg_redo_all = value != 0;
    else if (!strcmp(name, "dwell_tight")) e->dbg_dwell_tight = value != 0;
    else if (!strcmp(name, "gru_tiles")) e->dbg_gru_tiles = value;
    else if (!strcmp(name, "decoder_cus")) e->dbg_decoder_cus = value > 0 ? value : 0;
    else if (!strcmp(name, "force_f32_layers")) e->dbg_force_f32 = value != 0;
#ifdef SH_EXPERIMENTS
    else if (!strcmp(name, "gru32")) e->dbg_gru32 = value;
#endif
    else if (!strcmp(name, "tail")) e->tail_mode = value;
    else if (!strcmp(name, "fail_tail")) e->dbg_fail_tail = value;
    else if (!strcmp(name, "tail_free_frac")) e->dbg_tail_free_frac = value / 1000.0;
    else if (!strcmp(name, "squiggle_budget_kb")) e->dbg_squig_budget = value > 0 ? (size_t)value << 10 : 0;
    else if (!strcmp(name, "sqnet_budget_kb")) e->dbg_sqnet_budget = value > 0 ? (size_t)value << 10 : 0;
    else if (!strcmp(name, "map_pack_cells")) e->map_pack_cells = value < 0 ? -1 : value;
    else if (!strcmp(name, "map_crf_local_stride")) e->map_crf_local_stride = value < 0 ? -1 : value;
    else if (!strcmp(name, "map_local_stride")) e->map_local_stride = value < 0 ? -1 : value;
    else if (!strcmp(name, "crf_find_cells")) e->crf_find_cells = value < 0 ? -1 : value;
    else if (!strcmp(name, "map_crf_pack_cells")) e->map_crf_pack_cells = value < 0 ? -1 : value;
    else if (!strcmp(name, "events_budget_samples")) e->dbg_events_budget = value > 0 ? (size_t)value : 0;
    else return set_err("debug_option: unknown option '%s'", name);
    return 0;
}

extern "C" long long scrappie_hip_debug_fetch(scrappie_hip_engine *e, const char *what, void *dst, size_t nbytes) {
    if (!e || !what) return set_err("debug_fetch: null argument");
    (void)hipSetDevice(e->device);
    HIPCHK(sh_stream_wait(e->stream));
    HIPCHK(sh_stream_wait(e->cstream));
    const Slot &sl = e->current(); const LaunchGroup &lg = sl.lg;
    if (!lg.valid) return set_err("debug_fetch: no launch group has run");
    Model *m = get_model(e, lg.model);
    if (!m) return -1;
    const size_t NH = (size_t)std::max(m->NS - 1, 0);
    const void *src = nullptr; size_t have = 0; bool host = false;
    const int gru_tiles = lg.gru_two ? 2 : 1;
    if (!strcmp(what, "tb")) { src = e->d_tb.p; have = (size_t)lg.ncb * NH * 16; }
    else if (!strcmp(what, "tb_end")) { src = e->d_tbend.p; have = (size_t)lg.ncb * 16 * 4; }
    else if (!strcmp(what, "final_state")) { src = e->d_fstate.p; have = lg.npad * 4; }
    else if (!strcmp(what, "final_score")) { src = sl.d_fscore.p; have = lg.npad * 4; }
    else if (!strcmp(what, "final_scores")) { src = e->d_vstate.p; have = lg.ntile * (NH * 16 + 32) * 4; }
    else if (!strcmp(what, "order")) { src = lg.order.data(); have = lg.npad * 4; host = true; }
    else if (!strcmp(what, "tile_boff")) { src = lg.tile_boff.data(); have = lg.ntile * 8; host = true; }
    else if (!strcmp(what, "n_redo")) { static thread_local unsigned long long tot; tot = e->n_redo + e->n_redo_tail; src = &tot; have = 8; host = true; }
    else if (!strcmp(what, "n_tail_groups")) { src = &e->n_tail_groups; have = 8; host = true; }
    else if (!strcmp(what, "n_tail_calls")) { src = &e->n_tail_calls; have = 8; host = true; }
    else if (!strcmp(what, "n_tail_reads")) { src = &e->n_tail_reads; have = 8; host = true; }
    else if (!strcmp(what, "gru_tiles")) { src = &gru_tiles; have = 4; host = true; }
    else if (!strcmp(what, "decoder_pieces")) { src = &lg.vit_nwg; have = 4; host = true; }
    else if (!strcmp(what, "pinned_bytes")) {
        static thread_local unsigned long long tot;
        tot = e->slots[0].pinned_bytes() + e->slots[1].pinned_bytes();
        src = &tot; have = 8; host = true;
    }
    else return set_err("debug_fetch: unknown buffer '%s'", what);
    if (!src && have) return set_err("debug_fetch: buffer '%s' was not allocated", what);
    const size_t cnt = std::min(have, nbytes);
    if (dst && cnt) {
        if (host) memcpy(dst, src, cnt);
        else HIPCHK(hipMemcpy(dst, src, cnt, hipMemcpyDeviceToHost));
    }
    return (long long)have;
}

extern "C" long scrappie_hip_debug_stitch(scrappie_hip_engine *e, const int *path, const float *side, size_t nblock, int nstate, int crf,
                                          char *bases, size_t cap, int *pos, int *redo) {
    if (!e || !path || !bases || nblock == 0) { set_err("debug_stitch: bad argument"); return -2; }
    (void)hipSetDevice(e->device);
    std::lock_guard<std::mutex> lk(e->mu);
    const size_t T = nblock, npad = 64, bcap = 5 * (T + 1) + 8;
    DBuf dmeta, dseq, dhp, dpos, dbases, dblen, dredo;
    std::vector<char> hm(npad * 8 * 3 + npad * 4, 0);
    int *rT = (int *)(hm.data() + npad * 24);
    rT[0] = (int)T;
    if (dmeta.ensure(hm.size()) || dseq.ensure((T + 1) * 4) || dpos.ensure((T + 1) * 4) || dbases.ensure(bcap) ||
        dblen.ensure(npad * 4) || dredo.ensure(npad * 4) || (side && dhp.ensure(T * 5 * 4))) return -2;
    hipStream_t s = e->stream;
    if (hipMemcpyAsync(dmeta.p, hm.data(), hm.size(), hipMemcpyHostToDevice, s) != hipSuccess) return -2;
    if (hipMemcpyAsync(dseq.p, path, (T + 1) * 4, hipMemcpyHostToDevice, s) != hipSuccess) return -2;
    if (side && hipMemcpyAsync(dhp.p, side, T * 5 * 4, hipMemcpyHostToDevice, s) != hipSuccess) return -2;
    if (hipMemsetAsync(dredo.p, 0, npad * 4, s) != hipSuccess) return -2;
    if (sh_stream_wait(s) != hipSuccess) return -2;
    char *d = dmeta.as<char>();
    ShMeta md{};
    md.rT = (const int *)(d + npad * 24);
    ShStitchArgs sa;
    sa.seq = dseq.as<int>(); sa.seq_off = (const long long *)d;
    sa.hp = side ? dhp.as<float>() : nullptr; sa.hp_off = (const long long *)(d + npad * 8);
    sa.pos = pos ? dpos.as<int>() : nullptr;
    sa.bases = dbases.as<char>(); sa.bases_off = (const long long *)(d + npad * 16);
    sa.blen = dblen.as<int>(); sa.redo = dredo.as<unsigned>();
    sa.npad = 1; sa.nstate = nstate; sa.crf = crf; sa.sstride = 1;
    hipLaunchKernelGGL(k_stitch, dim3(1), dim3(64), 0, s, sa, md);
    int len = -1; unsigned rd = 0;
    if (hipMemcpyAsync(&len, dblen.p, 4, hipMemcpyDeviceToHost, s) != hipSuccess) return -2;
    if (hipMemcpyAsync(&rd, dredo.p, 4, hipMemcpyDeviceToHost, s) != hipSuccess) return -2;
    if (sh_stream_wait(s) != hipSuccess) { set_err("debug_stitch: %s", hipGetErrorString(hipGetLastError())); return -2; }
    if (redo) *redo = (int)rd;
    if (len >= 0) {
        if ((size_t)len + 1 > cap) { set_err("debug_stitch: %d bases do not fit %zu bytes", len, cap); return -2; }
        if (len && hipMemcpy(bases, dbases.p, (size_t)len, hipMemcpyDeviceToHost) != hipSuccess) return -2;
        bases[len] = 0;
        if (pos && !crf && hipMemcpy(pos, dpos.p, (T + 1) * 4, hipMemcpyDeviceToHost) != hipSuccess) return -2;
    }
    return len;
}

extern "C" int scrappie_hip_debug_stitch_dwell(scrappie_hip_engine *e, const int *paths, const int *dwells, const size_t *nentry, size_t nread, int ntrail,
                                               const float *prior_num, int nstate, const size_t *cap, char *bases, size_t bases_bytes, int *lengths, int *pos,
                                               int *redo) {
    if (!e || !paths || !dwells || !nentry || !prior_num || !cap || !bases || !lengths || nread == 0 || nread > (1u << 20) || (ntrail != 0 && ntrail != 1))
        return set_err("debug_stitch_dwell: bad argument");
    if (nstate != 5 && nstate != 17 && nstate != 65 && nstate != 257 && nstate != 1025) return set_err("debug_stitch_dwell: %d states (4^k + 1 with k <= 5)", nstate);
    (void)hipSetDevice(e->device);
    std::lock_guard<std::mutex> lk(e->mu);
    const size_t npad = (nread + 63) / 64 * 64;
    std::vector<char> hm(npad * 36, 0);
    long long *seq_off = (long long *)hm.data(), *bases_off = seq_off + npad, *dwell_off = bases_off + npad;
    float *num = (float *)(dwell_off + npad);
    int *nd = (int *)(num + npad), *capi = nd + npad;
    size_t nseq = 0, ndw = 0, nb = 0;
    for (size_t i = 0; i < nread; i++) {
        const size_t c = (cap[i] + 15) & ~(size_t)15;
        if (nentry[i] == 0 || nentry[i] > (1u << 28) || c == 0 || c > (1u << 30)) return set_err("debug_stitch_dwell: read %zu: %zu entries, %zu bytes", i, nentry[i], cap[i]);
        seq_off[i] = (long long)nseq; nseq += nentry[i] + (size_t)ntrail;
        dwell_off[i] = (long long)ndw; ndw += nentry[i];
        bases_off[i] = (long long)nb; nb += c;
        num[i] = prior_num[i]; nd[i] = (int)nentry[i]; capi[i] = (int)c;
    }
    if (nb > bases_bytes) return set_err("debug_stitch_dwell: the reservations take %zu bytes, bases holds %zu", nb, bases_bytes);
    DBuf dmeta, dseq, ddw, dpos, dbases, dblen, dredo;
    if (dmeta.ensure(hm.size()) || dseq.ensure(nseq * 4) || ddw.ensure(ndw * 4) || dpos.ensure(nseq * 4) || dbases.ensure(nb) ||
        dblen.ensure(npad * 4) || dredo.ensure(npad * 4)) return -1;
    hipStream_t s = e->stream;
    HIPCHK(hipMemcpyAsync(dmeta.p, hm.data(), hm.size(), hipMemcpyHostToDevice, s));
    HIPCHK(hipMemcpyAsync(dseq.p, paths, nseq * 4, hipMemcpyHostToDevice, s));
    HIPCHK(hipMemcpyAsync(ddw.p, dwells, ndw * 4, hipMemcpyHostToDevice, s));
    HIPCHK(hipMemsetAsync(dbases.p, 0, nb, s));
    HIPCHK(hipMemsetAsync(dpos.p, 0, nseq * 4, s));
    HIPCHK(hipMemsetAsync(dredo.p, 0, npad * 4, s));
    HIPCHK(sh_stream_wait(s));
    char *d = dmeta.as<char>();
    ShStitchArgs sa{};
    sa.seq = dseq.as<int>(); sa.seq_off = (const long long *)d;
    sa.hp = nullptr; sa.hp_off = nullptr;
    sa.pos = pos ? dpos.as<int>() : nullptr;
    sa.bases = dbases.as<char>(); sa.bases_off = (const long long *)(d + npad * 8);
    sa.blen = dblen.as<int>(); sa.redo = dredo.as<unsigned>();
    sa.npad = (int)nread; sa.nstate = nstate; sa.crf = 0; sa.sstride = 1;
    ShDwellArgs da{};
    da.dwell = ddw.as<int>(); da.dwell_off = (const long long *)(d + npad * 16);
    da.prior_num = (const float *)(d + npad * 24);
    da.nd = (const int *)(d + npad * 28); da.cap = (const int *)(d + npad * 32);
    da.ntrail = ntrail;
    hipLaunchKernelGGL(k_stitch_dwell, dim3((unsigned)(npad / 64)), dim3(64), 0, s, sa, da);
    HIPCHK(hipGetLastError());
    std::vector<unsigned> hredo(nread);
    HIPCHK(hipMemcpyAsync(lengths, dblen.p, nread * 4, hipMemcpyDeviceToHost, s));
    HIPCHK(hipMemcpyAsync(hredo.data(), dredo.p, nread * 4, hipMemcpyDeviceToHost, s));
    HIPCHK(hipMemcpyAsync(bases, dbases.p, nb, hipMemcpyDeviceToHost, s));
    if (pos) HIPCHK(hipMemcpyAsync(pos, dpos.p, nseq * 4, hipMemcpyDeviceToHost, s));
    HIPCHK(sh_stream_wait(s));
    if (redo) for (size_t i = 0; i < nread; i++) redo[i] = (int)hredo[i];
    return 0;
}

extern "C" void scrappie_hip_free_calls(scrappie_hip_call *calls, size_t n) {
    if (!calls) return;
    for (size_t i = 0; i < n; i++) { free(calls[i].basecall); free(calls[i].pos); calls[i].basecall = nullptr; calls[i].pos = nullptr; }
}
```

### scrappie_amd/csrc/sh_eng_launch.inc

```

struct MetaPtrs { ShMeta md; const long long *seq_off, *hp_off, *bases_off; ShGruLanes lanes, lanes1; ShGruPairs pairs, pairs2; const ShGruSegD *vseg; ShDwellArgs dw; };

#define SH_DWELL_PER_ENTRY 10
static long long bases_reservation(long long per_entry, long long nentry) { return (per_entry * nentry + 16 + 15) & ~15ll; }
extern "C" size_t scrappie_hip_dwell_capacity(size_t nentry) { return (size_t)bases_reservation(SH_DWELL_PER_ENTRY, (long long)nentry); }

static int build_group(scrappie_hip_engine *e, Slot &sl, Model *m, const uint64_t *offsets, const uint32_t *lengths,
                       size_t n, bool hp_on, MetaPtrs &mp, const DwellJob *dw = nullptr, const PostJob *pj = nullptr) {
    LaunchGroup &lg = sl.lg;
    lg.valid = false;
    lg.n = n; lg.hp_on = hp_on;
    lg.dw = DwellJob();
    if (dw && dw->on) {
        if (m->arch != 3 || dw->off.size() != n || dw->num.size() != n || dw->host.size() != n) return set_err("build_group: %zu reads, dwells of %zu", n, dw->off.size());
        lg.dw = *dw;
    }
    lg.post = PostJob(); lg.npost = 0;
    if (pj && pj->on) {
        if (m->arch != 1 || pj->dst.size() != n) return set_err("build_group: base probabilities of %zu reads for a group of %zu (flip-flop models only)", pj->dst.size(), n);
        lg.post = *pj;
    }
    lg.ntile = (n + 15) / 16; lg.npad = lg.ntile * 16;
    const int st = m->stride;
    std::vector<int> T(n);
    for (size_t i = 0; i < n; i++)
        T[i] = (lengths[i] >= m->min_samples) ? (int)((lengths[i] + st - 1) / st) : 0;
    lg.order.assign(lg.npad, -1);
    std::vector<int> idx(n);
    std::iota(idx.begin(), idx.end(), 0);
    std::stable_sort(idx.begin(), idx.end(), [&](int a, int b) { return T[a] > T[b]; });
    for (size_t i = 0; i < n; i++) lg.order[i] = idx[i];
    lg.rT.assign(lg.npad, 0); lg.rN.assign(lg.npad, 0);
    lg.seq_off.assign(lg.npad, 0); lg.hp_off.assign(lg.npad, 0); lg.bases_off.assign(lg.npad, 0);
    long long nbases = 0;
    const long long per_entry = (m->arch == 1) ? 1 : (lg.dw.on ? (e->dbg_dwell_tight ? 0 : SH_DWELL_PER_ENTRY) : 5);
    std::vector<unsigned long long> sig_off(lg.npad, 0);
    std::vector<int> tile_T(lg.ntile, 0);
    std::vector<long long> &tile_boff = lg.tile_boff;
    tile_boff.assign(lg.ntile, 0);
    long long ncb = 0, nseq = 0, nhp = 0;
    for (size_t i = 0; i < lg.npad; i++) {
        const int o = lg.order[i];
        if (o >= 0 && T[o] > 0) {
            lg.rT[i] = T[o]; lg.rN[i] = (int)lengths[o]; sig_off[i] = offsets[o];
        }
        lg.hp_off[i] = nhp; nhp += lg.rT[i];
        lg.bases_off[i] = nbases; nbases += lg.rT[i] ? bases_reservation(per_entry, (long long)lg.rT[i] + 1) : 0;
        tile_T[i >> 4] = std::max(tile_T[i >> 4], lg.rT[i]);
    }
    for (size_t t = 0; t < lg.ntile; t++) { tile_boff[t] = ncb; ncb += tile_T[t]; }
    for (size_t t = 0; t < lg.ntile; t++) {
        for (int b = 0; b < 16; b++) lg.seq_off[t * 16 + b] = nseq + b;
        nseq += tile_T[t] ? ((long long)tile_T[t] + 1) * SH_SEQ_STRIDE : 0;
    }
    lg.ncb = ncb; lg.nseq = nseq; lg.nhp = nhp; lg.nbases_cap = nbases;
    ShGruSchedule sched;
    sh_lane_schedule(tile_T.data(), lg.ntile, e->ncu, 2, sched, e->handover);
    lg.gru_nwg = sched.nwg;
    ShGruSchedule sched1;
    sh_lane_schedule(tile_T.data(), lg.ntile, e->ncu, 1, sched1, e->handover);
    lg.gru1_nwg = sched1.nwg;
    { long long nlive = 0; int tmax = 0; for (int t : tile_T) { nlive += t > 0; tmax = std::max(tmax, t); }
      const int w1 = sched1.wg_iter.empty() ? 0 : *std::max_element(sched1.wg_iter.begin(), sched1.wg_iter.end());
      const int w2 = sched.wg_iter.empty() ? 0 : *std::max_element(sched.wg_iter.begin(), sched.wg_iter.end());
      lg.gru_two = nlive > e->ncu && tmax < 65536 && (double)w2 * tun().gru_two_ratio < (double)w1;
      if (e->dbg_gru_tiles == 1) lg.gru_two = false;
      if (e->dbg_gru_tiles == 2 && tmax < 65536) lg.gru_two = true; }
    std::vector<int> pair_tile, pair_T;
    for (size_t t = 0; t < lg.ntile; ) {
        const bool two = t + 1 < lg.ntile && tile_T[t] < (1 << 18) && tile_T[t + 1] > 0;
        pair_tile.push_back((int)t); pair_tile.push_back(two ? (int)t + 1 : -1);
        pair_T.push_back(std::max(tile_T[t], two ? tile_T[t + 1] : 0));
        t += two ? 2 : 1;
    }
    ShGruSchedule sched32;
    sh_lane_schedule(pair_T.data(), pair_T.size(), e->ncu, 1, sched32, e->handover);
    lg.gru32_nwg = sched32.nwg;
    ShGruSchedule sched32b;
    sh_lane_schedule(pair_T.data(), pair_T.size(), e->ncu, 2, sched32b, e->handover);
    lg.gru32x2_nwg = sched32b.nwg;
    std::vector<ShGruSeg> vseg;
    sh_piece_schedule(tile_T.data(), lg.ntile, e->dbg_decoder_cus > 0 ? e->dbg_decoder_cus : e->ncu, vseg, e->handover);
    lg.vit_nwg = (int)vseg.size();
    const size_t b_u64 = lg.npad * 8, b_i32 = lg.npad * 4;
    const size_t b_loff = sched.lane_off.size() * 4, b_seg = sched.seg.size() * sizeof(ShGruSeg), b_wit = sched.wg_iter.size() * 4;
    const size_t b_vloff = 0, b_vseg = vseg.size() * sizeof(ShGruSeg);
    const size_t b_loff1 = sched1.lane_off.size() * 4, b_seg1 = sched1.seg.size() * sizeof(ShGruSeg);
    const size_t b_loff32 = sched32.lane_off.size() * 4, b_seg32 = sched32.seg.size() * sizeof(ShGruSeg), b_pt = pair_tile.size() * 4;
    const size_t b_loff32b = sched32b.lane_off.size() * 4, b_seg32b = sched32b.seg.size() * sizeof(ShGruSeg);
    const size_t total = 4 * b_u64 + lg.ntile * 8 + 2 * b_i32 + lg.ntile * 4 + 16 + b_seg + b_loff + b_wit + 16 + b_vseg + b_vloff + 16 + b_seg1 + b_loff1 +
                         16 + b_seg32 + b_loff32 + b_pt + 16 + b_seg32b + b_loff32b;
    if (sl.h_meta.ensure(total + 16) || sl.d_meta.ensure(total + 16)) return -1;
    char *h = sl.h_meta.as<char>();
    size_t o = 0;
    memcpy(h + o, sig_off.data(), b_u64); const size_t o_sig = o; o += b_u64;
    memcpy(h + o, lg.seq_off.data(), b_u64); const size_t o_seq = o; o += b_u64;
    memcpy(h + o, lg.hp_off.data(), b_u64); const size_t o_hp = o; o += b_u64;
    memcpy(h + o, lg.bases_off.data(), b_u64); const size_t o_bs = o; o += b_u64;
    memcpy(h + o, tile_boff.data(), lg.ntile * 8); const size_t o_tb = o; o += lg.ntile * 8;
    memcpy(h + o, lg.rN.data(), b_i32); const size_t o_n = o; o += b_i32;
    memcpy(h + o, lg.rT.data(), b_i32); const size_t o_t = o; o += b_i32;
    memcpy(h + o, tile_T.data(), lg.ntile * 4); const size_t o_tt = o; o += lg.ntile * 4;
    o = (o + 15) & ~(size_t)15;
    memcpy(h + o, sched.seg.data(), b_seg); const size_t o_seg = o; o += b_seg;
    memcpy(h + o, sched.lane_off.data(), b_loff); const size_t o_loff = o; o += b_loff;
    memcpy(h + o, sched.wg_iter.data(), b_wit); const size_t o_wit = o; o += b_wit;
    o = (o + 15) & ~(size_t)15;
    memcpy(h + o, vseg.data(), b_vseg); const size_t o_vseg = o; o += b_vseg;
    o = (o + 15) & ~(size_t)15;
    memcpy(h + o, sched1.seg.data(), b_seg1); const size_t o_seg1 = o; o += b_seg1;
    memcpy(h + o, sched1.lane_off.data(), b_loff1); const size_t o_loff1 = o; o += b_loff1;
    o = (o + 15) & ~(size_t)15;
    memcpy(h + o, sched32.seg.data(), b_seg32); const size_t o_seg32 = o; o += b_seg32;
    memcpy(h + o, sched32.lane_off.data(), b_loff32); const size_t o_loff32 = o; o += b_loff32;
    memcpy(h + o, pair_tile.data(), b_pt); const size_t o_pt = o; o += b_pt;
    o = (o + 15) & ~(size_t)15;
    memcpy(h + o, sched32b.seg.data(), b_seg32b); const size_t o_seg32b = o; o += b_seg32b;
    memcpy(h + o, sched32b.lane_off.data(), b_loff32b); const size_t o_loff32b = o; o += b_loff32b;
    hipStream_t ps = e->ev_ok ? e->pstream : e->stream;
    if (e->ev_ok) {
        const long long n16 = (long long)((total + 15) / 16);
        hipLaunchKernelGGL(k_upload_words, dim3((unsigned)std::min<long long>((n16 + 255) / 256, 64)), dim3(256), 0, ps, (const u32x4 *)h, sl.d_meta.as<u32x4>(), n16);
    } else HIPCHK(hipMemcpyAsync(sl.d_meta.p, h, total, hipMemcpyHostToDevice, ps));
    char *d = sl.d_meta.as<char>();
    mp.md.sig_off = (const unsigned long long *)(d + o_sig);
    mp.seq_off = (const long long *)(d + o_seq);
    mp.hp_off = (const long long *)(d + o_hp);
    mp.bases_off = (const long long *)(d + o_bs);
    mp.md.tile_boff = (const long long *)(d + o_tb);
    mp.md.rN = (const int *)(d + o_n);
    mp.md.rT = (const int *)(d + o_t);
    mp.md.tile_T = (const int *)(d + o_tt);
    static_assert(sizeof(ShGruSeg) == sizeof(ShGruSegD), "segment layout");
    mp.lanes.seg = (const ShGruSegD *)(d + o_seg);
    mp.lanes.lane_off = (const int *)(d + o_loff);
    mp.lanes.wg_iter = (const int *)(d + o_wit);
    mp.lanes.ntile = (int)lg.ntile;
    mp.vseg = (const ShGruSegD *)(d + o_vseg);
    if (e->d_hstate.ensure(std::max<size_t>(lg.ntile, 1) * 12 * 256 * 4) || sl.d_gflag.ensure((lg.ntile + 1) * 4)) return -1;
    mp.lanes.hstate = e->d_hstate.as<float>();
    mp.lanes.flag = sl.d_gflag.as<unsigned>();
    HIPCHK(hipMemsetAsync(sl.d_gflag.p, 0, (lg.ntile + 1) * 4, ps));
    if (sl.d_bad.ensure(lg.npad * 4)) return -1;
    HIPCHK(hipMemsetAsync(sl.d_bad.p, 0, lg.npad * 4, ps));
    mp.lanes1 = mp.lanes;
    mp.lanes1.seg = (const ShGruSegD *)(d + o_seg1);
    mp.lanes1.lane_off = (const int *)(d + o_loff1);
    mp.lanes1.wg_iter = nullptr;
    mp.pairs.seg = (const ShGruSegD *)(d + o_seg32);
    mp.pairs.lane_off = (const int *)(d + o_loff32);
    mp.pairs.pair_tile = (const int *)(d + o_pt);
    mp.pairs.hstate = mp.lanes.hstate;
    mp.pairs.flag = mp.lanes.flag;
    mp.pairs.err = mp.lanes.flag + lg.ntile;
    mp.pairs2 = mp.pairs;
    mp.pairs2.seg = (const ShGruSegD *)(d + o_seg32b);
    mp.pairs2.lane_off = (const int *)(d + o_loff32b);
    mp.dw = ShDwellArgs{};
    if (lg.dw.on) {
        const size_t np = lg.npad, bytes = (np * 16 + 15) & ~(size_t)15;
        if (sl.h_dwmeta.ensure(bytes) || sl.d_dwmeta.ensure(bytes)) return -1;
        long long *hoff = sl.h_dwmeta.as<long long>();
        float *hnum = (float *)(hoff + np);
        int *hcap = (int *)(hnum + np);
        for (size_t i = 0; i < np; i++) {
            const int o2 = lg.order[i];
            const bool live = o2 >= 0 && lg.rT[i] > 0;
            hoff[i] = live ? (long long)lg.dw.off[(size_t)o2] : 0;
            hnum[i] = live ? lg.dw.num[(size_t)o2] : 0.0f;
            hcap[i] = live ? (int)std::min<long long>(bases_reservation(per_entry, (long long)lg.rT[i] + 1), INT32_MAX & ~15) : 0;
        }
        if (e->ev_ok) hipLaunchKernelGGL(k_upload_words, dim3((unsigned)std::min<size_t>((bytes / 16 + 255) / 256, 64)), dim3(256), 0, ps, (const u32x4 *)sl.h_dwmeta.p, sl.d_dwmeta.as<u32x4>(), (long long)(bytes / 16));
        else HIPCHK(hipMemcpyAsync(sl.d_dwmeta.p, sl.h_dwmeta.p, bytes, hipMemcpyHostToDevice, ps));
        char *dd = sl.d_dwmeta.as<char>();
        mp.dw.dwell = lg.dw.d_dwell;
        mp.dw.dwell_off = (const long long *)dd;
        mp.dw.prior_num = (const float *)(dd + np * 8);
        mp.dw.cap = (const int *)(dd + np * 12);
        mp.dw.nd = mp.md.rT;
        mp.dw.ntrail = 1;
    }
    return 0;
}

template <int KQ>
static int launch_affine_k(hipStream_t s, const float *in, float *out, const float *wf, const unsigned *wp, const float *bf,
                           long long ncb, int mtiles) {
    const int mt = pick_mt(mtiles);
    long long gx = std::min<long long>((ncb + 3) / 4, 2048);
    if (gx < 1) gx = 1;
    dim3 grid((unsigned)gx, (unsigned)(mtiles / mt));
    int rc = 0;
    if (pick_int<6, 4, 3, 2, 1>(mt, rc, [&](auto m) { return launch_k<k_affine<KQ, m()>>(grid, dim3(256), 0, s, in, out, wf, wp, bf, ncb, mtiles); })) return rc;
    return set_err("unsupported layer of %d m-tiles", mtiles);
}

template <int KQ>
static int launch_affine_lds_k(hipStream_t s, const float *in, float *out, const float *wf, const unsigned *wp, const float *bf,
                               long long ncb, int mtiles) {
    constexpr int NB = SH_AFF_NB, NTH = SH_AFF_NTH;
    const size_t lds = ((size_t)mtiles * KQ * 256 + (size_t)mtiles * 256) * 4 + 16;
    long long gx = std::min<long long>((ncb + (NTH / 64) * NB - 1) / ((NTH / 64) * NB), 256);
    if (gx < 1) gx = 1;
    return launch_k<k_affine_lds<KQ, NB, NTH>>(dim3((unsigned)gx), dim3(NTH), lds, s, in, out, wf, wp, bf, ncb, mtiles);
}

template <int KQ>
static int launch_affine_f32_k(hipStream_t s, const float *in, float *out, const float *wf, const float *bf, long long ncb, int mtiles) {
    const int mt = (mtiles % 6 == 0) ? 6 : (mtiles % 2 == 0) ? 2 : 1;
    long long gx = std::min<long long>((ncb + 3) / 4, 2048);
    if (gx < 1) gx = 1;
    dim3 grid((unsigned)gx, (unsigned)(mtiles / mt));
    int rc = 0;
    if (pick_int<6, 2, 1>(mt, rc, [&](auto m) { return launch_k<k_affine<KQ, m(), true>>(grid, dim3(256), 0, s, in, out, wf, (const unsigned *)nullptr, bf, ncb, mtiles); })) return rc;
    return set_err("unsupported layer of %d m-tiles", mtiles);
}

static int launch_affine(hipStream_t s, int K, const float *in, float *out, const float *wf, const unsigned *wp, const float *bf_nat,
                         const float *bf_acc, long long ncb, int mtiles, bool force_f32 = false) {
    int rc = 0;
    if (force_f32 && pick_int<2, 4, 6, 8>(K / 16, rc, [&](auto kq) { return launch_affine_f32_k<kq()>(s, in, out, wf, bf_nat, ncb, mtiles); })) return rc;
    if (K % 32 == 0 && (!wp || !bf_acc)) return set_err("layer weights were not cut into pieces (input size %d)", K);
    const float *bf = (K % 32 == 0) ? bf_acc : bf_nat;
    const size_t lds_need = ((size_t)mtiles * (K / 16) * 256 + (size_t)mtiles * 256) * 4;
    if (mtiles >= 12 && lds_need <= 150 * 1024 && ncb >= 4096 && !tun().affine_reg &&
        pick_int<1, 2, 4, 6>(K / 16, rc, [&](auto kq) { return launch_affine_lds_k<kq()>(s, in, out, wf, wp, bf, ncb, mtiles); })) return rc;
    if (pick_int<1, 2, 4, 6, 8>(K / 16, rc, [&](auto kq) { return launch_affine_k<kq()>(s, in, out, wf, wp, bf, ncb, mtiles); })) return rc;
    return set_err("unsupported layer input size %d (need 16, 32, 64, 96 or 128)", K);
}

template <int KQ>
static int launch_affine2_k(hipStream_t s, const float *inF, const float *inB, float *out, const unsigned *wF, const unsigned *wB,
                            const float *bf, long long ncb, int mtiles) {
    long long gx = std::min<long long>((ncb + 3) / 4, 2048);
    if (gx < 1) gx = 1;
    const int mt = mtiles / 2;
    int rc = 0;
    if (mt * 2 == mtiles &&
        pick_int<3, 2, 1>(mt, rc, [&](auto m) { return launch_k<k_affine2_tanh<KQ, m()>>(dim3((unsigned)gx), dim3(512), 0, s, inF, inB, out, wF, wB, bf, ncb, mtiles); })) return rc;
    return set_err("unsupported joining layer of %d m-tiles", mtiles);
}

static int launch_affine2(hipStream_t s, int K, const float *inF, const float *inB, float *out, const unsigned *wF, const unsigned *wB,
                          const float *bf, long long ncb, int mtiles) {
    int rc = 0;
    if (pick_int<2, 4, 6>(K / 16, rc, [&](auto kq) { return launch_affine2_k<kq()>(s, inF, inB, out, wF, wB, bf, ncb, mtiles); })) return rc;
    return set_err("unsupported bi-GRU size %d (need 32, 64 or 96)", K);
}

static int launch_gru(hipStream_t s, int S, const float *xaff, float *out, const float *resid, const float *sW,
                      const float *sW2, const unsigned *sWp, const unsigned *sW2p, const ShMeta &md, int backward, size_t ntile, const ShGruLanes &lanes, int nwg,
                      bool force_f32 = false) {
    const int NU = S / 16;
    int rc = 0;
    if (!tun().gru_single && !tun().gru_stamp && tun().gru_debug < 0 && NU <= 6 && S % 32 == 0) {
        if (nwg <= 0) return 0;
        HIPCHK(hipMemsetAsync(lanes.flag, 0, (size_t)lanes.ntile * 4, s));
        dim3 lgrid((unsigned)nwg);
        const bool stamp = tun().gru_lanes_stamp;
        const bool f32_env = tun().gru_f32 || force_f32;
        if (!stamp && !f32_env) {
            const size_t plds = (size_t)2 * 2 * (NU / 2) * 2 * 64 * 4 * 4;
            if (pick_int<2, 4, 6>(NU, rc, [&](auto nu) { return launch_k<k_gru_split<nu()>>(lgrid, dim3(128 * nu()), plds, s, xaff, out, resid, sWp, sW2p, md, backward, lanes); })) return rc;
            return set_err("unsupported GRU size %d (need 32, 64 or 96 here)", S);
        }
        const size_t lds = (size_t)2 * 2 * NU * 256 * 4;
        static StampBuf st;
        if (!pick_int<2, 4, 6>(NU, rc, [&](auto nu) {
#ifdef SH_EXPERIMENTS
            if constexpr (nu() == 6)
                if (stamp) return launch_k<k_gru_lanes<6, true>>(lgrid, dim3(768), lds, s, xaff, out, resid, sW, sW2, md, backward, lanes, st.dev(4096 * 16 * 8));
#endif
            return launch_k<k_gru_lanes<nu(), false>>(lgrid, dim3(128 * nu()), lds, s, xaff, out, resid, sW, sW2, md, backward, lanes, (unsigned long long *)nullptr);
            })) return set_err("unsupported GRU size %d (need 32, 64 or 96 here)", S);
        if (stamp && NU == 6)
            st.dump_on(7, s, (size_t)nwg * 12 * 8, [&](const unsigned long long *h) {
                for (size_t g : {(size_t)nwg / 2}) for (int w = 0; w < 12; w++) {
                    const unsigned long long *d = &h[(g * 12 + w) * 8];
                    fprintf(stderr, "gru lanes stamp wg %zu wave %2d: phase1 %.0f bar %.0f phase2 %.0f bar %.0f cycles/step (%llu steps)\n",
                            g, w, d[0] / (double)d[4], d[1] / (double)d[4], d[2] / (double)d[4], d[3] / (double)d[4], d[4]);
                }
            });
        return rc;
    }
    if (tun().gru_debug >= 0) backward |= tun().gru_debug << 8;
    static StampBuf st1;
    unsigned long long *dbgbuf = tun().gru_stamp ? st1.dev(4096 * 8 * 8) : nullptr;
    if (dbgbuf)
        st1.dump_on(8, s, ntile * NU * 8, [&](const unsigned long long *h) {
            { unsigned long long first_end = ~0ull, mn = ~0ull, mx = 0; size_t late = 0;
              for (size_t tl = 0; tl < ntile; tl++) { first_end = std::min(first_end, h[tl * NU * 8 + 7]); mn = std::min(mn, h[tl * NU * 8 + 6]); mx = std::max(mx, h[tl * NU * 8 + 7]); }
// ... 330 lines not shown
```

### scrappie_amd/csrc/sh_eng_load.inc

```

static const HostMat *find_mat(const std::vector<std::pair<std::string, HostMat>> &ms, const char *nm) {
    for (auto &kv : ms) if (kv.first == nm) return &kv.second;
    return nullptr;
}

static int load_model_mem_one(scrappie_hip_engine *e, const char *name, const void *blob, size_t nbytes);
static int sqnet_load(Model *m, const std::vector<std::pair<std::string, HostMat>> &mats);
extern "C" int scrappie_hip_load_model_mem(scrappie_hip_engine *e, const char *name, const void *blob, size_t nbytes) {
    const int idx = load_model_mem_one(e, name, blob, nbytes);
    if (idx < 0 || e->is_tail) return idx;
    scrappie_hip_engine::Blob b{name, std::vector<unsigned char>((const unsigned char *)blob, (const unsigned char *)blob + nbytes), e->dbg_force_f32};
    bool found = false;
    for (auto &x : e->blobs) if (x.name == b.name) { x = b; found = true; }
    if (!found) e->blobs.push_back(b);
    if (e->tail || e->tail2) {
        std::unique_lock<std::mutex> lk(e->tail_mu);
        e->tail_cv.wait(lk, [&] { return e->tail_busy == 0 && e->tail_q.empty(); });
    }
    for (scrappie_hip_engine **tp : {&e->tail, &e->tail2}) if (*tp) {
        (*tp)->dbg_force_f32 = e->dbg_force_f32;
        if (load_model_mem_one(*tp, name, blob, nbytes) != idx) return set_err("model '%s' did not load at the same index on the helper engine", name);
    }
    return idx;
}
// ... 148 lines not shown
                return set_err("model '%s': FF%d has a weight of magnitude %g, outside the split products' range (< %g); "
                               "there is no exact-fp32 kernel for this layer", name, k + 1, mx, (double)SH_W_LIMIT);
            }
            const int mt = (m->S + 15) / 16;
            if (upload_u32(m->ff2W[k][0], make_piece_frags(*wf)) || upload_u32(m->ff2W[k][1], make_piece_frags(*wb)) ||
                upload(m->ff2b[k], scaled(make_bias_frags(*bb, mt), SH_OSCALE))) { delete m; return -1; }
        }
    }
    if (m->S % 32 == 0 && !in_split_range(*fw)) {
        const float mx = max_abs(*fw);
        delete m;
        return set_err("model '%s': the output layer has a weight of magnitude %g, outside the split products' range (< %g); "
                       "there is no exact-fp32 kernel for this layer", name, mx, (double)SH_W_LIMIT);
    }
    {
        double worst = 0.0;
        for (int c = 0; c < fw->nc; c++) {
            double acc = c < (int)fb->v.size() ? fabs((double)fb->v[(size_t)c]) : 0.0;
            for (int r = 0; r < fw->nr; r++) acc += fabs((double)fw->v[(size_t)c * fw->nr + r]);
            worst = std::max(worst, acc);
        }
        m->ff_no_clamp = worst < 88.0;
    }
    if (upload(m->ffW, make_frags(*fw, m->ff_mtiles)) || upload(m->ffb, make_bias_frags(*fb, m->ff_mtiles))) { delete m; return -1; }
    if (m->S % 32 == 0 && (upload_u32(m->ffWp, make_piece_frags(*fw)) || upload(m->ffbs, scaled(make_bias_frags(*fb, m->ff_mtiles), SH_OSCALE)))) { delete m; return -1; }
    if (m->arch == 3) {
        m->min_samples = 2;
    } else {
    ShConvGeom &g = m->geom;
    g = conv_geom(m->WL, m->stride, m->F);
    m->min_samples = (size_t)(g.shiftX + 2 * g.nstepX + g.WL);
    if (m->min_samples < (size_t)(g.st + 1)) m->min_samples = (size_t)(g.st + 1);
    }
    std::lock_guard<std::mutex> lk(e->mu);
    for (size_t i = 0; i < e->models.size(); i++)
        if (e->models[i]->name == name) { delete e->models[i]; e->models[i] = m; return (int)i; }
    e->models.push_back(m);
    return (int)e->models.size() - 1;
}

extern "C" int scrappie_hip_load_model(scrappie_hip_engine *e, const char *name, const char *path) {
    if (!path) return set_err("load_model: null path");
    FILE *fh = fopen(path, "rb");
    if (!fh) return set_err("cannot open model file %s", path);
    fseek(fh, 0, SEEK_END);
    long sz = ftell(fh);
    fseek(fh, 0, SEEK_SET);
    std::vector<unsigned char> buf((size_t)std::max(0L, sz));
    const size_t got = fread(buf.data(), 1, buf.size(), fh);
    fclose(fh);
    if (got != buf.size()) return set_err("short read on %s", path);
    return scrappie_hip_load_model_mem(e, name, buf.data(), buf.size());
}

extern "C" int scrappie_hip_find_model(scrappie_hip_engine *e, const char *name) {
    if (!e || !name) return -1;
    std::lock_guard<std::mutex> lk(e->mu);
    for (size_t i = 0; i < e->models.size(); i++) if (e->models[i]->name == name) return (int)i;
    return -1;
}

static Model *get_model(scrappie_hip_engine *e, int model) {
    if (!e || model < 0 || (size_t)model >= e->models.size()) { set_err("invalid model handle %d", model); return nullptr; }
    if (e->models[model]->arch == 4) { set_err("model '%s' predicts squiggles from sequences; it takes no signal", e->models[model]->name.c_str()); return nullptr; }
    return e->models[model];
}

extern "C" size_t scrappie_hip_min_samples(scrappie_hip_engine *e, int model) {
    Model *m = get_model(e, model);
    return m ? m->min_samples : 0;
}
extern "C" int scrappie_hip_model_stride(scrappie_hip_engine *e, int model) {
    Model *m = get_model(e, model);
    return m ? m->stride : -1;
}
extern "C" void scrappie_hip_set_profiling(scrappie_hip_engine *e, int on) { if (e) e->profiling = on != 0; }
static int resolve_spans(scrappie_hip_engine *e, Slot &sl) {
    scrappie_hip_timing &tm = sl.timing;
    float dbg_wait = 0.f, dbg_lead = 0.f;
    float *fields[F_COUNT] = {&tm.conv_ms, &tm.affine_ms, &tm.gru_ms, &tm.ff_ms, &tm.decode_ms, &tm.backtrace_ms, &tm.total_ms, &tm.fused_ms, &tm.stitch_ms,
                              &dbg_wait, &dbg_lead};
    for (auto &sp : sl.spans) {
        float ms = 0;
        HIPCHK(hipEventElapsedTime(&ms, sl.ev[sp.i], sl.ev[sp.j]));
        *fields[sp.field] += ms;
    }
    sl.spans.clear();
    if (tun().host_stamp) fprintf(stderr, "host stamp: main stream waited %.2f ms for the prologue; the convolution had ended %.2f ms before the main stream got there (negative: after)\n", dbg_wait, dbg_lead);
    e->timing = tm;
    return 0;
}

extern "C" int scrappie_hip_get_timing(scrappie_hip_engine *e, scrappie_hip_timing *t) {
    if (!e || !t) return -1;
    (void)hipSetDevice(e->device);
    Slot &sl = e->current();
    if (!sl.spans.empty() && !sl.pending) {
        HIPCHK(sh_stream_wait(e->stream));
        if (resolve_spans(e, sl)) return -1;
    }
    *t = e->timing;
    return 0;
}
extern "C" void scrappie_hip_set_max_launch_reads(scrappie_hip_engine *e, size_t n) { if (e && n >= 16) e->max_launch_reads = n; }
extern "C" void scrappie_hip_set_max_launch_blocks(scrappie_hip_engine *e, size_t n) { if (e) e->max_launch_blocks = n; }
extern "C" void *scrappie_hip_device_alloc(scrappie_hip_engine *e, size_t nbytes) {
    if (!e) return nullptr;
    (void)hipSetDevice(e->device);
    void *p = nullptr;
    if (hipMalloc(&p, nbytes) != hipSuccess) { set_err("hipMalloc(%zu) failed", nbytes); return nullptr; }
    return p;
}
extern "C" void scrappie_hip_device_free(scrappie_hip_engine *e, void *dptr) {
    if (e && dptr) { (void)hipSetDevice(e->device); (void)hipFree(dptr); }
}
extern "C" int scrappie_hip_memcpy_h2d(scrappie_hip_engine *e, void *dst, const void *src, size_t nbytes) {
    if (!e) return -1;
    (void)hipSetDevice(e->device);
    HIPCHK(hipMemcpy(dst, src, nbytes, hipMemcpyHostToDevice));
    return 0;
}
extern "C" int scrappie_hip_synchronize(scrappie_hip_engine *e) {
    if (!e) return -1;
    (void)hipSetDevice(e->device);
    HIPCHK(sh_stream_wait(e->stream));
    return 0;
}

extern "C" long scrappie_hip_lane_schedule(const int *tile_T, size_t ntile, int ncu, int lanes_per_wg, int *nwg, int *capacity,
                                           int *lane_off, int *seg, size_t cap) {
    if (!tile_T || ncu < 1 || lanes_per_wg < 1 || lanes_per_wg > 2) return -1;
    ShGruSchedule sc;
    sh_lane_schedule(tile_T, ntile, ncu, lanes_per_wg, sc);
    if (nwg) *nwg = sc.nwg;
    if (capacity) *capacity = sc.capacity;
    if (lane_off) memcpy(lane_off, sc.lane_off.data(), sc.lane_off.size() * sizeof(int));
    if (seg) for (size_t i = 0; i < sc.seg.size() && i < cap; i++) memcpy(seg + 4 * i, &sc.seg[i], 16);
    return (long)sc.seg.size();
}

extern "C" long scrappie_hip_gru_schedule(const int *tile_T, size_t ntile, int ncu, int *nwg, int *capacity,
                                          int *lane_off, int *seg, size_t cap) {
    return scrappie_hip_lane_schedule(tile_T, ntile, ncu, 2, nwg, capacity, lane_off, seg, cap);
}

extern "C" long scrappie_hip_decoder_pieces(const int *tile_T, size_t ntile, int ncu, int *seg, size_t cap) {
    if (!tile_T || ncu < 1) return -1;
    std::vector<ShGruSeg> v;
    sh_piece_schedule(tile_T, ntile, ncu, v);
    if (seg) for (size_t i = 0; i < v.size() && i < cap; i++) memcpy(seg + 4 * i, &v[i], 16);
    return (long)v.size();
}

extern "C" long scrappie_hip_plan_groups(const uint32_t *lengths, size_t n, int stride, size_t max_reads, size_t max_blocks,
                                         size_t *starts, size_t cap) {
    if ((!lengths && n) || stride < 1 || max_reads < 1) return -1;
    long ng = 0;
    size_t cnt = 0;
    unsigned long long sumT = 0, maxT = 0;
    for (size_t i = 0; i < n; i++) {
        const unsigned long long T = ((unsigned long long)lengths[i] + stride - 1) / stride;
        if (max_blocks && T / 16 + T + 1 > max_blocks) return -1;
        const unsigned long long ns = sumT + T, nm = std::max(maxT, T);
        if (cnt == 0 || cnt >= max_reads || (max_blocks && ns / 16 + nm + 1 > max_blocks)) {
            if (starts && (size_t)ng < cap) starts[ng] = i;
            ng++;
            cnt = 0; sumT = 0; maxT = 0;
        }
        cnt++; sumT += T; maxT = std::max(maxT, T);
    }
    return ng;
}

static bool decoder_fused(const scrappie_hip_engine *e, const Model *m) {
    return m->NS > 25 && !e->alt_prob && m->NS == 1025 && m->S == 96 && !tun().ff_separate && !e->dbg_ff_separate;
}

static size_t bytes_per_block(const Model *m, bool posterior) {
    const size_t S = (size_t)m->S, F = (size_t)m->F, w = std::max(S, F);
    size_t b = ((m->arch == 2 || m->arch == 3) ? 4 : 3) * w * 64 + 128;
    if (posterior) b += (size_t)m->ff_mtiles * 1024;
    if (m->arch == 3 || F != S || S % 32 || S / 16 > 6) b += (size_t)(m->arch == 3 ? 4 : 3) * S * 64;
    if (m->NS > 25) b += (size_t)((m->NS - 1) / 4) * 64;
    else b += 16 * 4 * 4;
    b += 16 * 2 * (4 + 4 + 20 + 5) + 2 * 16 * 4 * (size_t)std::max(m->stride, 1) * (m->arch == 3 ? (size_t)m->nfeat : 1);
    return b;
}

static size_t launch_block_cap(scrappie_hip_engine *e, const Model *m) {
    if (e->max_launch_blocks) return e->max_launch_blocks;
    return (size_t)(e->mem_frac * (double)e->total_mem) / bytes_per_block(m, !decoder_fused(e, m));
}
```

### scrappie_amd/csrc/sh_eng_pipeline.inc

```

enum StopAt { STOP_NONE = 0, STOP_TRUNK = 1, STOP_POST = 2 };

struct RunOut {
    const float *act = nullptr;
    int act_units = 0;
    const float *E = nullptr;
    const float *sums = nullptr;
};

struct HostStamp {
    const std::chrono::steady_clock::time_point t0 = std::chrono::steady_clock::now();
    void operator()(const char *what, const char *after = "") const {
        if (tun().host_stamp) fprintf(stderr, "host stamp: %s %.2f ms%s\n", what, std::chrono::duration<double, std::milli>(std::chrono::steady_clock::now() - t0).count(), after);
    }
};

struct Marks {
    enum Mark { PROLOGUE_BEGIN, PROLOGUE_END,
                WAIT_BEGIN, MAIN_BEGIN,
                LAYER_BEGIN, LAYER_SPLIT, LAYER_END,
                S1_BEGIN, S1_END, DECODE_END, MAIN_END,
                WALK_BEGIN, WALK_END, STITCH_BEGIN, STITCH_END,
                N_MARKS };
    Slot *sl = nullptr;
// ... 112 lines not shown
                              : areg     ? act(k_conv_mfma<0, 6, 3, true>, k_conv_mfma<1, 6, 3, true>)
                              : kst == 3 ? (bg ? act(k_conv_mfma_bg<0, 6, 3, false>, k_conv_mfma_bg<1, 6, 3, false>) : act(k_conv_mfma<0, 6, 3, false>, k_conv_mfma<1, 6, 3, false>))
                                         : (bg ? act(k_conv_mfma_bg<0, 6, 5, false>, k_conv_mfma_bg<1, 6, 5, false>) : act(k_conv_mfma<0, 6, 5, false>, k_conv_mfma<1, 6, 5, false>));
        if (fake == 1) HIPCHK(hipMemsetAsync(c.abuf[0], 0, c.act_bytes, ps));
        else if (fake != 2) hipLaunchKernelGGL(kern, grid, dim3(256), lds, ps, c.d_signal, c.mp.md, m->conv_W.as<float>(), m->conv_b.as<float>(), m->geom, c.abuf[0], tchunk, sl.d_bad.as<unsigned>());
    }
    if (c.pf.mark(Marks::PROLOGUE_END, ps)) return -1;
    c.pf.span(F_CONV, Marks::PROLOGUE_BEGIN, Marks::PROLOGUE_END);
    c.stamp("prologue enqueued at");
    if (c.pf.mark(Marks::WAIT_BEGIN, s)) return -1;
    if (e->ev_ok && ps != s) { HIPCHK(hipEventRecord(sl.pdone, ps)); HIPCHK(hipStreamWaitEvent(s, sl.pdone, 0)); }
    c.stamp("wait enqueued at");
    if (c.pf.mark(Marks::MAIN_BEGIN, s)) return -1;
    c.pf.span(F_WAIT, Marks::WAIT_BEGIN, Marks::MAIN_BEGIN); c.pf.span(F_LEAD, Marks::PROLOGUE_END, Marks::WAIT_BEGIN);
    if (tun().helper_fence && e->ev_ok && e->other(sl).pending) HIPCHK(hipStreamWaitEvent(s, e->other(sl).hdone, 0));
    return 0;
}

static int recurrent_layer(Slot &sl, Model *m, GroupRun &c, int l, int I, const float *in, float *out, int backward) {
    scrappie_hip_engine *e = c.e;
    const LaunchGroup &lg = sl.lg; const MetaPtrs &mp = c.mp;
    const hipStream_t s = c.s;
    const bool lstm = m->arch == 3;
    const int S = m->S, gates = lstm ? 4 : 3;
    const float *resid = m->arch == 1 ? in : nullptr;
    const bool f32 = !lstm && m->layer_f32[l];
    const bool one_kernel = !tun().gru_separate && (lstm ? (I == S || I == 16) && S % 32 == 0 : gru_proj_ok(I, S) && !f32);
    if (c.pf.mark(Marks::LAYER_BEGIN, s)) return -1;
#ifdef SH_EXPERIMENTS
    if (l == 0 && c.fuse_conv) {
        if (c.pf.mark(Marks::LAYER_SPLIT, s)) return -1;
        ShConvFuse cf;
        cf.sig = c.d_signal; cf.W = m->conv_W.as<float>(); cf.bias = m->conv_b.as<float>(); cf.edge = sl.d_edge.as<int>();
        cf.bad = sl.d_bad.as<unsigned>(); cf.g = m->geom;
        if (launch_gru_conv(s, (m->WL + 3) / 4, m->conv_act, out, m->iWp[l].as<unsigned>(), m->ibs[l].as<float>(), m->sWp[l].as<unsigned>(),
                            m->sW2p[l].as<unsigned>(), mp.md, 1, mp.lanes1, lg.gru1_nwg, mp.lanes, lg.gru_nwg, lg.gru_two, cf)) return -1;
    } else if (!lstm && one_kernel && use_gru32(e) && S == 96 && I == 96 && m->has32) {
        if (c.pf.mark(Marks::LAYER_SPLIT, s)) return -1;
        if (use_gru32(e) == 2 ? launch_gru_proj32x2(s, in, out, m->arch == 1, m->iWp32[l].as<unsigned>(), m->ib32[l].as<float>(), m->sWp32[l].as<unsigned>(),
                                                    m->sW2p32[l].as<unsigned>(), mp.md, backward, mp.pairs2, lg.gru32x2_nwg, lg.ntile)
                              : launch_gru_proj32(s, in, out, m->arch == 1, m->iWp32[l].as<unsigned>(), m->ib32[l].as<float>(), m->sWp32[l].as<unsigned>(),
                                                  m->sW2p32[l].as<unsigned>(), mp.md, backward, mp.pairs, lg.gru32_nwg, lg.ntile)) return -1;
    } else
#endif
    if (one_kernel) {
        if (c.pf.mark(Marks::LAYER_SPLIT, s)) return -1;
        if (lstm ? launch_lstm_proj(s, S, I, in, out, m->iWp[l].as<unsigned>(), m->ibs[l].as<float>(), m->sWp[l].as<unsigned>(), m->lp[l].as<float>(),
                                    mp.md, backward, mp.lanes1, lg.gru1_nwg)
                 : launch_gru_proj(s, S, in, out, resid, m->iWp[l].as<unsigned>(), m->ibs[l].as<float>(), m->sWp[l].as<unsigned>(), m->sW2p[l].as<unsigned>(),
                                   mp.md, backward, mp.lanes1, lg.gru1_nwg, mp.lanes, lg.gru_nwg, lg.gru_two)) return -1;
    } else {
        if (e->d_xaff.ensure((size_t)c.ncb * gates * S * 16 * 4)) return -1;
        if (launch_affine(s, I, in, e->d_xaff.as<float>(), m->iW[l].as<float>(), m->iWp[l].as<unsigned>(), m->ib[l].as<float>(), m->ibs[l].as<float>(), c.ncb, gates * S / 16, f32)) return -1;
        if (c.pf.mark(Marks::LAYER_SPLIT, s)) return -1;
        if (lstm ? launch_lstm(s, S, e->d_xaff.as<float>(), out, m->sWp[l].as<unsigned>(), m->lp[l].as<float>(), mp.md, backward, mp.lanes, lg.gru_nwg)
                 : launch_gru(s, S, e->d_xaff.as<float>(), out, resid, m->sW[l].as<float>(), m->sW2[l].as<float>(), m->sWp[l].as<unsigned>(), m->sW2p[l].as<unsigned>(),
                              mp.md, backward, lg.ntile, mp.lanes, lg.gru_nwg, f32)) return -1;
    }
    if (c.pf.mark(Marks::LAYER_END, s)) return -1;
    c.pf.span(F_AFFINE, Marks::LAYER_BEGIN, Marks::LAYER_SPLIT);
    c.pf.span(F_GRU, Marks::LAYER_SPLIT, Marks::LAYER_END);
    if (c.pf.on) {
        scrappie_hip_timing &tm = sl.timing;
        const double af = 2.0 * I * gates * S * 16.0 * (double)c.ncb, gf = 2.0 * gates * S * S * 16.0 * (double)c.ncb;
        tm.n_affine_launches++; tm.n_gru_launches++; tm.affine_flops += af; tm.gru_flops += gf;
        if (one_kernel) { tm.n_fused_launches++; tm.fused_flops += af + gf; }
    }
    if (one_kernel) c.pf.span(F_FUSED, Marks::LAYER_SPLIT, Marks::LAYER_END);
    return 0;
}

static int stage_trunk(Slot &sl, Model *m, GroupRun &c, int *top) {
    const hipStream_t s = c.s;
    const int S = m->S, F = m->F;
    float **abuf = c.abuf; *top = 0;
    if (m->arch == 2 || m->arch == 3) {
        for (int lvl = 0; lvl < 2 && lvl < c.trunk_upto; lvl++) {
            for (int dir = 0; dir < 2; dir++) if (recurrent_layer(sl, m, c, 2 * lvl + dir, lvl == 0 ? F : S, abuf[0], abuf[1 + dir], dir)) return -1;
            if (c.pf.mark(Marks::LAYER_BEGIN, s)) return -1;
            if (launch_affine2(s, S, abuf[1], abuf[2], abuf[0], m->ff2W[lvl][0].as<unsigned>(), m->ff2W[lvl][1].as<unsigned>(), m->ff2b[lvl].as<float>(), c.ncb, S / 16)) return -1;
            if (c.pf.mark(Marks::LAYER_SPLIT, s)) return -1;
            c.pf.span(F_AFFINE, Marks::LAYER_BEGIN, Marks::LAYER_SPLIT);
            if (c.pf.on) sl.timing.affine_flops += 2.0 * 2 * S * S * 16.0 * (double)c.ncb;
        }
    } else {
        for (int l = 0; l < 5 && l < c.trunk_upto; l++, *top ^= 1)
            if (recurrent_layer(sl, m, c, l, l == 0 ? F : S, abuf[*top], abuf[*top ^ 1], (l % 2 == 0) ? 1 : 0)) return -1;
    }
    HIPCHK(hipGetLastError());
    c.stamp("layers enqueued at");
    return 0;
}

template <class Grow, class Launch>
static int inject_alt(const Slot &sl, GroupRun &c, AltInput &alt, uint64_t seed, Grow grow, Launch launch) {
    const LaunchGroup &lg = sl.lg;
    std::vector<unsigned long long> aoff(lg.npad, ~0ull);
    uint64_t key = 1469598103934665603ull ^ seed;
    for (size_t i = 0; i < lg.npad; i++) {
        const int o = lg.order[i];
        if (o >= 0 && lg.rT[i] > 0) aoff[i] = alt.off[(size_t)o % alt.off.size()];
        key = (key ^ (uint64_t)(aoff[i] + 0x9e3779b97f4a7c15ull * (uint64_t)(lg.rT[i] + 1))) * 1099511628211ull;
    }
    if (alt.valid && key == alt.key) return 0;
    if (grow() || alt.d_off.ensure(lg.npad * 8)) return -1;
    HIPCHK(hipMemcpyAsync(alt.d_off.p, aoff.data(), lg.npad * 8, hipMemcpyHostToDevice, c.s));
    HIPCHK(sh_stream_wait(c.s));
    launch(dim3((unsigned)lg.ntile, (unsigned)std::min(longest_tile(lg), 1024)), alt.d_off.as<unsigned long long>());
    alt.key = key; alt.valid = true;
    return 0;
}

static int stage_decode_transducer(Slot &sl, Model *m, GroupRun &c, const float *top, bool fused, bool *stopped) {
    scrappie_hip_engine *e = c.e;
    LaunchGroup &lg = sl.lg; const MetaPtrs &mp = c.mp;
    const hipStream_t s = c.s; const scrappie_hip_params *p = c.p;
    const int S = m->S, mtiles = m->ff_mtiles;
    const long long ncb = c.ncb;
    if (e->d_sums.ensure((size_t)ncb * 16 * 4)) return -1;
    if (c.pf.mark(Marks::S1_BEGIN, s)) return -1;
    if (!fused && launch_ff(s, S, top, e->d_E.as<float>(), e->d_sums.as<float>(), m->ffWp.as<unsigned>(), m->ffbs.as<float>(),
                            ncb, mtiles, m->NS, p->tempW / p->tempb, p->tempb, e->ncu)) return -1;
    if (c.pf.mark(Marks::S1_END, s)) return -1;
    c.pf.span(F_FF, Marks::S1_BEGIN, Marks::S1_END);
    if (c.pf.on) sl.timing.ff_flops += 2.0 * S * m->NS * 16.0 * (double)ncb;
    const float *E_use = e->d_E.as<float>(), *sums_use = e->d_sums.as<float>();
    if (e->alt_prob) {
        if (inject_alt(sl, c, e->alt_prob, (uint64_t)lg.model,
                       [&] { return e->d_Ealt.ensure((size_t)ncb * mtiles * 256 * 4) || e->d_sums_alt.ensure((size_t)ncb * 16 * 4); },
                       [&](dim3 grid, const unsigned long long *off) {
                           hipLaunchKernelGGL(k_inject_prob, grid, dim3(256), 0, s, e->alt_prob.data, off, mp.md, m->NS, mtiles, e->d_Ealt.as<float>(), e->d_sums_alt.as<float>());
                       })) return -1;
        E_use = e->d_Ealt.as<float>(); sums_use = e->d_sums_alt.as<float>();
    }
    if (c.ro) { c.ro->E = E_use; c.ro->sums = sums_use; }
    if (c.stop == STOP_POST) { HIPCHK(hipGetLastError()); *stopped = true; return 0; }
    const int NH = m->NS - 1, NQ = NH / 4;
    if (e->d_tb.ensure((size_t)ncb * NQ * 16 * 4) || e->d_tbend.ensure((size_t)ncb * 16 * 4) || e->d_fstate.ensure(lg.npad * 4)) return -1;
    if (c.hp_on && sl.d_hp.ensure((size_t)std::max<long long>(lg.nhp, 1) * 5 * 4)) return -1;
    ShVitArgs va;
    va.E = E_use; va.sums = sums_use;
    va.strideT = (long long)mtiles * 256; va.strideQ = 64; va.strideB = 4;
    va.want_log = 1; va.min_prob = p->min_prob;
    va.stay_pen = p->stay_pen; va.skip_pen = p->skip_pen; va.local_pen = p->local_pen; va.use_slip = p->use_slip;
    va.tb = e->d_tb.as<unsigned>(); va.tb_end = e->d_tbend.as<int>();
    va.final_state = e->d_fstate.as<int>(); va.final_score = sl.d_fscore.as<float>();
    va.hp_side = c.hp_on ? sl.d_hp.as<float>() : nullptr; va.hp_off = mp.hp_off;
    va.dbg = nullptr;
    va.dump_final = e->dbg_dump_final ? 1 : 0;
    static StampBuf vst;
    if (tun().vit_stamp) va.dbg = vst.dev(4096 * 16 * 8);
    if (e->d_vstate.ensure(std::max<size_t>(lg.ntile, 1) * ((size_t)NH * 16 + 32) * 4) || e->d_vflag.ensure(std::max<size_t>(lg.ntile, 1) * 4)) return -1;
    HIPCHK(hipMemsetAsync(e->d_vflag.p, 0, std::max<size_t>(lg.ntile, 1) * 4, s));
    va.seg = mp.vseg;
    va.vstate = e->d_vstate.as<float>(); va.flag = e->d_vflag.as<unsigned>(); va.err = sl.d_gflag.as<unsigned>() + lg.ntile;
    if (e->ev_ok && e->other(sl).pending) HIPCHK(hipStreamWaitEvent(s, e->other(sl).done, 0));
    if (fused) {
        ShFfArgs fa;
        fa.in = top; fa.wpiece = m->ffWp.as<unsigned>(); fa.bfrag = m->ffbs.as<float>();
        fa.in_div = p->tempW / p->tempb; fa.out_div = p->tempb;
        fa.no_clamp = (m->ff_no_clamp && !e->alt_trunk) ? 1 : 0;
        va.E = nullptr; va.sums = nullptr;
        if (launch_ff_viterbi(s, fa, va, mp.md, (size_t)lg.vit_nwg, tun().fv_single || e->dbg_fv_single)) return -1;
    } else if (launch_viterbi(s, NH, va, mp.md, (size_t)lg.vit_nwg)) return -1;
    if (va.dbg) vst.dump_on(0, s, (size_t)std::max(lg.vit_nwg, 1) * 16 * 8, [&](const unsigned long long *h) {
        const int nwv = (fused && !va.use_slip && !(tun().fv_single || e->dbg_fv_single)) ? 12 : 8;
        for (int w = 0; w < nwv; w++) { const unsigned long long *d = &h[((size_t)(lg.vit_nwg / 2) * nwv + w) * 8]; fprintf(stderr, "vit stamp wave %d: phaseB %.0f bar %.0f phaseC %.0f bar %.0f cycles/block\n", w, d[0] / (double)d[4], d[1] / (double)d[4], d[2] / (double)d[4], d[3] / (double)d[4]); }
    });
    if (c.pf.mark(Marks::DECODE_END, s)) return -1;
    c.pf.span(F_DECODE, Marks::S1_END, Marks::DECODE_END);
    c.stamp("decoder enqueued at");
    c.walk_on_cs = e->ev_ok;
    if (c.walk_on_cs) { HIPCHK(hipEventRecord(sl.kdone, s)); HIPCHK(hipStreamWaitEvent(e->cstream, sl.kdone, 0)); }
    c.fold_tail = c.walk_on_cs && !tun().split_tail && !tun().host_stitch;
    if (!c.fold_tail) {
        hipStream_t bs = c.walk_on_cs ? e->cstream : s;
        if (c.pf.mark(Marks::WALK_BEGIN, bs)) return -1;
        hipLaunchKernelGGL(k_backtrace, dim3((unsigned)((lg.npad + 63) / 64)), dim3(64), 0, bs, e->d_tb.as<unsigned>(), e->d_tbend.as<int>(),
                           e->d_fstate.as<int>(), mp.md, mp.seq_off, sl.d_seq.as<int>(), (int)lg.npad, NQ, SH_SEQ_STRIDE);
        if (c.pf.mark(Marks::WALK_END, bs)) return -1;
        c.pf.span(F_BACKTRACE, Marks::WALK_BEGIN, Marks::WALK_END);
    }
    return 0;
}

static int stage_decode_crf(Slot &sl, Model *m, GroupRun &c, const float *top, bool *stopped) {
    scrappie_hip_engine *e = c.e;
    LaunchGroup &lg = sl.lg; const MetaPtrs &mp = c.mp;
    const hipStream_t s = c.s;
    const int S = m->S, mtiles = m->ff_mtiles;
    const long long ncb = c.ncb;
    if (c.pf.mark(Marks::S1_BEGIN, s)) return -1;
    if (launch_affine(s, S, top, e->d_E.as<float>(), m->ffW.as<float>(), m->ffWp.as<unsigned>(), m->ffb.as<float>(), m->ffbs.as<float>(), ncb, mtiles)) return -1;
    if (c.pf.mark(Marks::S1_END, s)) return -1;
    c.pf.span(F_FF, Marks::S1_BEGIN, Marks::S1_END);
    if (c.pf.on) sl.timing.ff_flops += 2.0 * S * m->NS * 16.0 * (double)ncb;
    if (e->d_tb.ensure((size_t)ncb * 16 * 8)) return -1;
    if (e->ev_ok && e->other(sl).pending) HIPCHK(hipStreamWaitEvent(s, e->other(sl).done, 0));
    const bool probs = lg.post.on && c.stop == STOP_NONE;
    hipLaunchKernelGGL((c.ro || c.stop == STOP_POST || probs) ? k_crf<true> : k_crf<false>, dim3((unsigned)(lg.npad / 16)), dim3(128), 0, s, e->d_E.as<float>(), mp.md,
                       e->d_tb.as<unsigned char>(), mp.seq_off, sl.d_seq.as<int>(), sl.d_fscore.as<float>(), (int)lg.npad, SH_SEQ_STRIDE);
    if (c.pf.mark(Marks::DECODE_END, s)) return -1;
    c.pf.span(F_DECODE, Marks::S1_END, Marks::DECODE_END);
    if (c.ro) { c.ro->E = e->d_E.as<float>(); c.ro->sums = nullptr; }
    if (c.stop == STOP_POST) { HIPCHK(hipGetLastError()); *stopped = true; }
    if (probs && crf_post_enqueue(sl, c)) return -1;
    return 0;
}

static int stage_tail(Slot &sl, Model *m, GroupRun &c) {
    scrappie_hip_engine *e = c.e;
    LaunchGroup &lg = sl.lg; const MetaPtrs &mp = c.mp;
    const hipStream_t s = c.s, cs = c.cs;
    if (sl.h_score.ensure(lg.npad * 4)) return -1;
    if (sl.h_err.ensure(4) || sl.h_bad.ensure(lg.npad * 4)) return -1;
    if (c.pf.mark(Marks::MAIN_END, s)) return -1;
    c.pf.span(F_TOTAL, Marks::MAIN_BEGIN, Marks::MAIN_END);
    if (e->ev_ok && !c.walk_on_cs) { HIPCHK(hipEventRecord(sl.kdone, s)); HIPCHK(hipStreamWaitEvent(cs, sl.kdone, 0)); }
    lg.dev_stitch = !tun().host_stitch;
    lg.dev_pos = lg.dev_stitch && c.p->want_pos != 0 && c.transducer;
    if (lg.dev_stitch) {
        const size_t nseq = (size_t)std::max<long long>(lg.nseq, 1), ncap = (size_t)std::max<long long>(lg.nbases_cap, 1);
        if (sl.d_bases.ensure(ncap) || sl.d_blen.ensure(lg.npad * 4) || sl.d_redo.ensure(lg.npad * 4) ||
            sl.h_bases.ensure(ncap) || sl.h_blen.ensure(lg.npad * 4) || sl.h_redo.ensure(lg.npad * 4)) return -1;
        if (lg.dev_pos && (sl.d_pos.ensure(nseq * 4 + 16) || sl.h_pos.ensure(nseq * 4 + 16))) return -1;
        ShStitchArgs sa;
        sa.seq = sl.d_seq.as<int>(); sa.seq_off = mp.seq_off;
        sa.hp = c.hp_on ? sl.d_hp.as<float>() : nullptr; sa.hp_off = mp.hp_off;
        sa.pos = lg.dev_pos ? sl.d_pos.as<int>() : nullptr;
        sa.bases = sl.d_bases.as<char>(); sa.bases_off = mp.bases_off;
        sa.blen = sl.d_blen.as<int>(); sa.redo = sl.d_redo.as<unsigned>();
        sa.npad = (int)lg.npad; sa.nstate = m->NS; sa.crf = c.transducer ? 0 : 1; sa.sstride = SH_SEQ_STRIDE;
        ShResultArgs ra;
        ra.d_bases = sl.d_bases.as<char>(); ra.h_bases = sl.h_bases.as<char>(); ra.bases_off = mp.bases_off;
        ra.d_blen = sl.d_blen.as<int>(); ra.h_blen = sl.h_blen.as<int>();
        ra.d_redo = sl.d_redo.as<unsigned>(); ra.h_redo = sl.h_redo.as<unsigned>();
        ra.d_score = sl.d_fscore.as<float>(); ra.h_score = sl.h_score.as<float>();
        ra.d_bad = sl.d_bad.as<unsigned>(); ra.h_bad = sl.h_bad.as<unsigned>();
        ra.d_err = sl.d_gflag.as<unsigned>() + lg.ntile; ra.h_err = sl.h_err.as<unsigned>();
        ra.npad = (int)lg.npad;
        if (c.pf.mark(Marks::STITCH_BEGIN, cs)) return -1;
        const bool dwell = lg.dw.on && c.transducer;
        if (c.fold_tail) {
            ShWalkArgs wa;
            wa.tb = e->d_tb.as<unsigned>(); wa.tb_end = e->d_tbend.as<int>(); wa.final_state = e->d_fstate.as<int>();
            wa.seq_off = mp.seq_off; wa.seq = sl.d_seq.as<int>(); wa.NQ = (m->NS - 1) / 4;
            if (dwell) hipLaunchKernelGGL(k_walk_dwell_out, dim3((unsigned)((lg.npad + 63) / 64)), dim3(64), 0, cs, wa, sa, mp.dw, ra, mp.md);
            else hipLaunchKernelGGL(k_walk_stitch_out, dim3((unsigned)((lg.npad + 63) / 64)), dim3(64), 0, cs, wa, sa, ra, mp.md);
        } else if (dwell)
            hipLaunchKernelGGL(k_stitch_dwell, dim3((unsigned)((lg.npad + 63) / 64)), dim3(64), 0, cs, sa, mp.dw);
        else
            hipLaunchKernelGGL(k_stitch, dim3((unsigned)((lg.npad + 63) / 64)), dim3(64), 0, cs, sa, mp.md);
        if (c.pf.mark(Marks::STITCH_END, cs)) return -1;
        c.pf.span(F_STITCH, Marks::STITCH_BEGIN, Marks::STITCH_END);
        if (e->ev_ok) HIPCHK(hipEventRecord(sl.hdone, cs));
        c.stamp("stitch enqueued at");
        if (!c.fold_tail) hipLaunchKernelGGL(k_results_out, dim3((unsigned)((lg.npad + 3) / 4)), dim3(256), 0, cs, ra);
        if (lg.dev_pos) {
            const long long n16 = (lg.nseq * 4 + 15) / 16;
            hipLaunchKernelGGL(k_upload_words, dim3((unsigned)std::min<long long>((n16 + 255) / 256, 256)), dim3(256), 0, cs, (const u32x4 *)sl.d_pos.p, sl.h_pos.as<u32x4>(), n16);
        }
    } else {
        if (sl.h_seq.ensure((size_t)std::max<long long>(lg.nseq, 1) * 4)) return -1;
        if (c.hp_on && sl.h_hp.ensure((size_t)std::max<long long>(lg.nhp, 1) * 5 * 4)) return -1;
        HIPCHK(hipMemcpyAsync(sl.h_seq.p, sl.d_seq.p, (size_t)lg.nseq * 4, hipMemcpyDeviceToHost, cs));
        if (c.hp_on) HIPCHK(hipMemcpyAsync(sl.h_hp.p, sl.d_hp.p, (size_t)lg.nhp * 5 * 4, hipMemcpyDeviceToHost, cs));
        HIPCHK(hipMemcpyAsync(sl.h_score.p, sl.d_fscore.p, lg.npad * 4, hipMemcpyDeviceToHost, cs));
        HIPCHK(hipMemcpyAsync(sl.h_err.p, sl.d_gflag.as<unsigned>() + lg.ntile, 4, hipMemcpyDeviceToHost, cs));
        HIPCHK(hipMemcpyAsync(sl.h_bad.p, sl.d_bad.p, lg.npad * 4, hipMemcpyDeviceToHost, cs));
    }
    if (lg.post.on && crf_post_download(sl, c)) return -1;
    HIPCHK(hipGetLastError());
    c.stamp("copies enqueued at");
    if (e->ev_ok) HIPCHK(hipEventRecord(sl.done, cs));
    return 0;
}

static int run_pipeline(scrappie_hip_engine *e, Model *m, const float *d_signal, const uint64_t *offsets,
                        const uint32_t *lengths, size_t n, const scrappie_hip_params *p, StopAt stop,
                        int trunk_upto, RunOut *ro, const DwellJob *dw = nullptr, const PostJob *pj = nullptr) {
    (void)hipSetDevice(e->device);
    if (n == 0) return set_err("empty batch");
    GroupRun c;
    c.e = e; c.d_signal = d_signal; c.offsets = offsets; c.p = p; c.stop = stop; c.trunk_upto = trunk_upto; c.ro = ro; c.dw = dw; c.pj = pj;
    c.transducer = (m->arch != 1);
    c.hp_on = c.transducer && p->homopolymer == HOMOPOLYMER_MEAN && stop == STOP_NONE;
    c.s = e->stream; c.ps = e->ev_ok ? e->pstream : e->stream; c.cs = e->ev_ok ? e->cstream : e->stream;
    Slot *slp = nullptr; bool empty = false;
    if (begin_group(e, m, lengths, n, c, &slp, &empty)) return -1;
    if (empty) return 0;
    Slot &sl = *slp;
    LaunchGroup &lg = sl.lg;
    const long long ncb = c.ncb = lg.ncb;
    const int S = m->S, F = m->F;
    c.act_bytes = (size_t)ncb * std::max(S, F) * 16 * 4;
    if (e->d_act[1].ensure(c.act_bytes)) return -1;
    bool any_f32 = false;
    for (bool b : m->layer_f32) any_f32 |= b;
    const bool need_xaff = m->arch == 3 || !gru_proj_ok(F, S) || tun().gru_separate || any_f32;
    if (need_xaff && e->d_xaff.ensure((size_t)ncb * (m->arch == 3 ? 4 : 3) * S * 16 * 4)) return -1;
    if ((m->arch == 2 || m->arch == 3) && e->d_act[2].ensure(c.act_bytes)) return -1;
    c.pf.sl = &sl; c.pf.on = e->profiling && e->ev_ok;
    if (c.pf.on) { memset(&sl.timing, 0, sizeof sl.timing); sl.nev = 0; sl.spans.clear(); }
    if (stage_prologue(sl, m, c)) return -1;
    if (lg.post.on && e->ev_ok && crf_post_mark(sl, 0, c.s)) return -1;
    int cur = 0;
    if (stage_trunk(sl, m, c, &cur)) return -1;
    if (ro) { ro->act = c.abuf[cur]; ro->act_units = (trunk_upto == 0) ? F : S; }
    lg.model = (int)(std::find(e->models.begin(), e->models.end(), m) - e->models.begin());
    if (stop == STOP_TRUNK) { lg.valid = true; return 0; }
    const float *top = c.abuf[cur];
    if (e->alt_trunk) {
        if (inject_alt(sl, c, e->alt_trunk, (uint64_t)lg.model ^ ((uint64_t)S << 32),
                       [&] { return e->d_act_alt.ensure((size_t)ncb * S * 16 * 4); },
                       [&](dim3 grid, const unsigned long long *off) {
                           hipLaunchKernelGGL(k_inject_trunk, grid, dim3(256), 0, c.s, e->alt_trunk.data, off, c.mp.md, S, e->d_act_alt.as<float>());
                       })) return -1;
        top = e->d_act_alt.as<float>();
    }
    const bool fused = c.transducer && stop == STOP_NONE && decoder_fused(e, m);
// ... 40 lines not shown
```

### scrappie_amd/csrc/sh_eng_surface.inc

```

struct PostReq {
    int model = -1;
    raw_table sig{};
    float min_prob = 0.f, tempW = 1.f, tempb = 1.f;
    bool want_log = true;
    StopAt stop = STOP_POST;
    int upto = 5;
    scrappie_matrix out = nullptr;
    size_t nr = 0, nc = 0;
    const float *src = nullptr;
    size_t nbytes = 0;
    std::atomic<int> *users = nullptr;
    int phase = 0;
    char err[256] = "";
};
static void post_fail(PostReq *r, const char *fmt, ...) {
    va_list ap;
    va_start(ap, fmt);
    vsnprintf(r->err, sizeof r->err, fmt, ap);
    va_end(ap);
}
static void posterior_batch(scrappie_hip_engine *e, std::vector<PostReq *> &reqs) {
    if (reqs.empty()) return;
    Model *m = get_model(e, reqs[0]->model);
// ... 147 lines not shown
    if (!e || !name) return -1;
    std::lock_guard<std::mutex> lk(g_models_mu);
    const int h = scrappie_hip_load_model(e, name, path);
    if (h >= 0) g_models[name] = h;
    return h;
}

static int default_model(scrappie_hip_engine *e, const char *name) {
    std::lock_guard<std::mutex> lk(g_models_mu);
    auto it = g_models.find(name);
    if (it != g_models.end()) return it->second;
    int h = scrappie_hip_find_model(e, name);
    if (h < 0) {
        const char *dir = getenv("SCRAPPIE_MODEL_DIR");
        if (!dir) { set_err("model '%s' is not registered and SCRAPPIE_MODEL_DIR is unset (weights are not compiled in)", name); return -1; }
        std::string path = std::string(dir) + "/" + name + ".scrm";
        h = scrappie_hip_load_model(e, name, path.c_str());
    }
    if (h >= 0) g_models[name] = h;
    return h;
}

static scrappie_matrix named_posterior(const char *name, const raw_table signal, float min_prob, float tempW, float tempb, bool return_log) {
    if (signal.n == 0 || !signal.raw) return nullptr;
    scrappie_hip_engine *e = default_engine();
    if (!e) return nullptr;
    const int h = default_model(e, name);
    if (h < 0) return nullptr;
    if (coalesce_on()) return coalesced_posterior(e, h, signal, min_prob, tempW, tempb, return_log);
    return scrappie_hip_posterior(e, h, signal, min_prob, tempW, tempb, return_log);
}

extern "C" scrappie_matrix scrappie_hip_events_posterior(scrappie_hip_engine *e, int model, const float *feature3, size_t nevent,
                                                         float min_prob, float tempW, float tempb, bool return_log) {
    Model *m = get_model(e, model);
    if (!m) return nullptr;
    if (m->arch != 3) { set_err("events_posterior: model '%s' is not an events model", m->name.c_str()); return nullptr; }
    if (!feature3 || nevent == 0) { set_err("events_posterior: empty read"); return nullptr; }
    raw_table rt = {nullptr, nevent * (size_t)m->nfeat, 0, nevent * (size_t)m->nfeat, const_cast<float *>(feature3)};
    return scrappie_hip_posterior(e, model, rt, min_prob, tempW, tempb, return_log);
}

extern "C" scrappie_matrix nanonet_posterior(const event_table events, float min_prob, float tempW, float tempb, bool return_log) {
    if (events.n == 0 || !events.event || events.end <= events.start) return nullptr;
    scrappie_hip_engine *e = default_engine();
    if (!e) return nullptr;
    const int model = default_model(e, "nanonet_events");
    if (model < 0) return nullptr;
    const size_t n = events.end - events.start;
    std::vector<float> f3(n * 12);
    if (scrappie_hip_event_features(events, f3.data())) return nullptr;
    if (coalesce_on()) {
        raw_table rt = {nullptr, n * 12, 0, n * 12, f3.data()};
        return coalesced_posterior(e, model, rt, min_prob, tempW, tempb, return_log);
    }
    return scrappie_hip_events_posterior(e, model, f3.data(), n, min_prob, tempW, tempb, return_log);
}

extern "C" scrappie_matrix nanonet_raw_posterior(const raw_table s, float mp, float tw, float tb, bool lg) { return named_posterior("raw_r94", s, mp, tw, tb, lg); }
extern "C" scrappie_matrix nanonet_rgrgr_r94_posterior(const raw_table s, float mp, float tw, float tb, bool lg) { return named_posterior("rgrgr_r94", s, mp, tw, tb, lg); }
extern "C" scrappie_matrix nanonet_rgrgr_r941_posterior(const raw_table s, float mp, float tw, float tb, bool lg) { return named_posterior("rgrgr_r941", s, mp, tw, tb, lg); }
extern "C" scrappie_matrix nanonet_rgrgr_r10_posterior(const raw_table s, float mp, float tw, float tb, bool lg) { return named_posterior("rgrgr_r10", s, mp, tw, tb, lg); }
extern "C" scrappie_matrix nanonet_rnnrf_r94_transitions(const raw_table s, float mp, float tw, float tb, bool lg) { return named_posterior("rnnrf_r94", s, mp, tw, tb, lg); }

extern "C" posterior_function_ptr get_posterior_function(const enum raw_model_type model) {
    switch (model) {
    case SCRAPPIE_MODEL_RAW: return nanonet_raw_posterior;
    case SCRAPPIE_MODEL_RGRGR_R9_4: return nanonet_rgrgr_r94_posterior;
    case SCRAPPIE_MODEL_RGRGR_R9_4_1: return nanonet_rgrgr_r941_posterior;
    case SCRAPPIE_MODEL_RGRGR_R10: return nanonet_rgrgr_r10_posterior;
    case SCRAPPIE_MODEL_RNNRF_R9_4: return nanonet_rnnrf_r94_transitions;
    default:
        fprintf(stderr, "scrappie_hip: model enum %d has no posterior function\n", (int)model);
        exit(EXIT_FAILURE);
    }
}

extern "C" int get_raw_model_stride(const enum raw_model_type model) {
    scrappie_hip_engine *e = default_engine();
    if (!e) return -1;
    const int h = default_model(e, raw_model_string(model));
    return h < 0 ? -1 : e->models[h]->stride;
}

extern "C" int get_raw_model_stride_from_string(const char *modelstr) {
    const enum raw_model_type t = get_raw_model(modelstr);
    if (t == SCRAPPIE_MODEL_INVALID) return -1;
    return get_raw_model_stride(t);
}

struct DecReq {
    const_scrappie_matrix post = nullptr;
    float stay_pen = 0.f, skip_pen = 0.f, local_pen = 0.f;
    bool slip = false;
    int *seq = nullptr;
    float score = NAN;
    int phase = 0;
    float *dst = nullptr;
};
struct DecCoalescer : ShCoalescer<DecReq> { HBuf &stage = *new HBuf; };
static DecCoalescer g_dc;

static void decode_batch(scrappie_hip_engine *e, std::vector<DecReq *> &reqs, const float *staged) {
    const size_t n = reqs.size();
    const DecReq *f = reqs[0];
    const int NH = (int)f->post->nr - 1, NQ = NH / 4;
    const size_t stride = f->post->stride;
    (void)hipSetDevice(e->device);
    std::lock_guard<std::mutex> lk(e->mu);
    hipStream_t s = e->stream;
    const size_t npad = 16 * n;
    long long ncb = 0;
    for (const DecReq *r : reqs) ncb += (long long)r->post->nc;
    std::vector<char> hm(npad * 24 + n * 8 + npad * 8 + n * 4, 0);
    long long *seq_off = (long long *)(hm.data() + npad * 8);
    long long *tboff = (long long *)(hm.data() + npad * 24);
    int *rN = (int *)(hm.data() + npad * 24 + n * 8), *rT = rN + npad, *tT = rT + npad;
    long long nseq = 0, boff = 0;
    for (size_t k = 0; k < n; k++) {
        const int T = (int)reqs[k]->post->nc;
        tboff[k] = boff; tT[k] = T;
        for (int b = 0; b < 16; b++) { rN[k * 16 + b] = 1; rT[k * 16 + b] = T; seq_off[k * 16 + b] = nseq; }
        nseq += T + 1; boff += T;
    }
    DBuf &dmeta = e->d_dec[0], &dpost = e->d_dec[1], &dtb = e->d_dec[2], &dtbe = e->d_dec[3], &dfs = e->d_dec[4], &dfsc = e->d_dec[5], &dseq = e->d_dec[6];
    bool ok = false;
    do {
        const size_t pbytes = (size_t)ncb * stride * 4;
        if (dmeta.ensure(hm.size()) || dpost.ensure(pbytes) || dtb.ensure((size_t)ncb * NQ * 16 * 4) || dtbe.ensure((size_t)ncb * 16 * 4) ||
            dfs.ensure(npad * 4) || dfsc.ensure(npad * 4) || dseq.ensure((size_t)nseq * 4) || e->h_dec_out.ensure((size_t)nseq * 4 + npad * 4)) break;
        if (!staged) {
            if (e->h_dec_in.ensure(pbytes)) break;
            float *h = e->h_dec_in.as<float>();
            for (size_t k = 0; k < n; k++) memcpy(h + (size_t)tboff[k] * stride, reqs[k]->post->data.f, (size_t)reqs[k]->post->nc * stride * 4);
            staged = h;
        }
        if (hipMemcpyAsync(dmeta.p, hm.data(), hm.size(), hipMemcpyHostToDevice, s) != hipSuccess) break;
        if (hipMemcpyAsync(dpost.p, staged, pbytes, hipMemcpyHostToDevice, s) != hipSuccess) break;
        char *d = dmeta.as<char>();
        ShMeta md;
        md.sig_off = (const unsigned long long *)d;
        md.tile_boff = (const long long *)(d + npad * 24);
        md.rN = (const int *)(d + npad * 24 + n * 8);
        md.rT = md.rN + npad;
        md.tile_T = md.rT + npad;
        ShVitArgs va;
        va.E = dpost.as<float>(); va.sums = nullptr;
        va.strideT = (long long)stride; va.strideQ = 4; va.strideB = 0;
        va.want_log = 0; va.min_prob = 0.f;
        va.stay_pen = f->stay_pen; va.skip_pen = f->skip_pen; va.local_pen = f->local_pen; va.use_slip = f->slip ? 1 : 0;
        va.tb = dtb.as<unsigned>(); va.tb_end = dtbe.as<int>();
        va.final_state = dfs.as<int>(); va.final_score = dfsc.as<float>();
        va.hp_side = nullptr; va.hp_off = nullptr; va.dbg = nullptr; va.dump_final = 0;
        va.seg = nullptr; va.vstate = nullptr; va.flag = nullptr; va.err = nullptr;
        if (launch_viterbi(s, NH, va, md, n)) break;
        hipLaunchKernelGGL(k_backtrace_lane0, dim3((unsigned)((n + 63) / 64)), dim3(64), 0, s, dtb.as<unsigned>(), dtbe.as<int>(), dfs.as<int>(), md,
                           (const long long *)(d + npad * 8), dseq.as<int>(), (int)n, NQ);
        int *hseq = e->h_dec_out.as<int>();
        if (hipMemcpyAsync(hseq, dseq.p, (size_t)nseq * 4, hipMemcpyDeviceToHost, s) != hipSuccess) break;
        if (hipMemcpyAsync(hseq + nseq, dfsc.p, npad * 4, hipMemcpyDeviceToHost, s) != hipSuccess) break;
        if (sh_stream_wait(s) != hipSuccess) break;
        const float *hsc = (const float *)(hseq + nseq);
        for (size_t k = 0; k < n; k++) {
            memcpy(reqs[k]->seq, hseq + seq_off[k * 16], ((size_t)reqs[k]->post->nc + 1) * 4);
            reqs[k]->score = hsc[k * 16];
        }
        ok = true;
    } while (0);
    if (!ok) { (void)hipGetLastError(); for (DecReq *r : reqs) r->score = NAN; }
}

static float coalesced_decode(scrappie_hip_engine *e, const_scrappie_matrix logpost, float stay_pen, float skip_pen, float local_pen, int *seq, bool allow_slip) {
    constexpr size_t MAX_READS = 1024;
    constexpr long long MAX_BLOCKS = 200000;
    ShInside inside(g_presence);
    DecReq r;
    r.post = logpost; r.stay_pen = stay_pen; r.skip_pen = skip_pen; r.local_pen = local_pen; r.slip = allow_slip; r.seq = seq;
    g_dc.run(r, g_presence, MAX_READS, true,
        [&](std::deque<DecReq *> &q, std::vector<DecReq *> &batch) {
            take_compatible(q, batch, MAX_READS, MAX_BLOCKS,
                            [](const DecReq *f, const DecReq *c) {
                                return c->post->nr == f->post->nr && c->post->stride == f->post->stride && c->stay_pen == f->stay_pen && c->skip_pen == f->skip_pen &&
                                       c->local_pen == f->local_pen && c->slip == f->slip;
                            },
                            [](const DecReq *c) { return (long long)c->post->nc; });
        },
        [&](std::vector<DecReq *> &batch) {
            const size_t stride = batch[0]->post->stride;
            size_t ncb = 0;
            for (const DecReq *c : batch) ncb += c->post->nc;
            if (g_dc.stage.ensure(ncb * stride * 4) != 0) return false;
            float *at = g_dc.stage.as<float>();
            for (DecReq *c : batch) { c->dst = at; at += c->post->nc * stride; }
            return true;
        },
        [](DecReq &c) { memcpy(c.dst, c.post->data.f, (size_t)c.post->nc * c.post->stride * 4); },
        [&](std::vector<DecReq *> &batch) { decode_batch(e, batch, g_dc.stage.as<float>()); });
    return r.score;
}
extern "C" void scrappie_hip_decode_coalescer_stats(unsigned long long out[3]) {
    std::lock_guard<std::mutex> lk(g_dc.mu);
    out[0] = g_dc.n_batches; out[1] = g_dc.n_reads; out[2] = g_dc.max_batch;
    if (getenv("SCRAPPIE_HIP_COALESCE_TIMES")) fprintf(stderr, "decode coalescer: %llu launches took %.1f ms in all\n", g_dc.n_batches, g_dc.service_us / 1e3);
}

extern "C" float decode_transducer(const_scrappie_matrix logpost, float stay_pen, float skip_pen, float local_pen, int *seq, bool allow_slip) {
    if (!logpost || !seq) return NAN;
    scrappie_hip_engine *e = default_engine();
    if (!e) return NAN;
    const int NH = (int)logpost->nr - 1, T = (int)logpost->nc;
    if (NH % 64 != 0 || (allow_slip && NH % 256 != 0) || T <= 0) return NAN;
    if (NH != 64 && NH != 256 && NH != 1024) return NAN;
    if (coalesce_on('d')) return coalesced_decode(e, logpost, stay_pen, skip_pen, local_pen, seq, allow_slip);
    DecReq r;
    r.post = logpost; r.stay_pen = stay_pen; r.skip_pen = skip_pen; r.local_pen = local_pen; r.slip = allow_slip; r.seq = seq;
    std::vector<DecReq *> one{&r};
    decode_batch(e, one, nullptr);
    return r.score;
}

__global__ void k_crf_viterbi_batch(const float *__restrict__ trans, int stride, const long long *__restrict__ coff, const int *__restrict__ Ts, int n,
                                    unsigned *__restrict__ tbbuf, int *__restrict__ path, float *__restrict__ score) {
    const int r = blockIdx.x * blockDim.x + threadIdx.x;
    if (r >= n) return;
    const int T = Ts[r];
    const float *tr0 = trans + coff[r] * stride;
    unsigned *tb = tbbuf + coff[r];
    int *pth = path + coff[r] + r;
    float prev[5] = {0.f, 0.f, 0.f, 0.f, 0.f}, curr[5];
    for (int t = 0; t < T; t++) {
        const float *tr = tr0 + (long long)t * stride;
        unsigned pack = 0;
        for (int to = 0; to < 5; to++) {
            float best = tr[to * 5] + prev[0];
            unsigned from = 0;
            for (int fr = 1; fr < 5; fr++) {
                const float sc = tr[to * 5 + fr] + prev[fr];
                if (sc > best) { best = sc; from = fr; }
            }
            curr[to] = best;
            pack |= from << (3 * to);
        }
        tb[t] = pack;
        for (int i = 0; i < 5; i++) prev[i] = curr[i];
    }
    float best = prev[0];
    int arg = 0;
    for (int i = 1; i < 5; i++) if (prev[i] > best) { best = prev[i]; arg = i; }
    score[r] = best;
    pth[T] = arg;
    for (int blk = T; blk > 0; blk--) { arg = (tb[blk - 1] >> (3 * arg)) & 7u; pth[blk - 1] = arg; }
}

struct CrfReq { const_scrappie_matrix trans = nullptr; int *path = nullptr; float score = NAN; int phase = 0; };
static ShCoalescer<CrfReq> g_cc;

static void crf_batch(scrappie_hip_engine *e, std::vector<CrfReq *> &reqs) {
    const size_t n = reqs.size(), stride = reqs[0]->trans->stride;
    long long ncol = 0;
    for (CrfReq *r : reqs) ncol += (long long)r->trans->nc;
    const size_t fbytes = (size_t)ncol * stride * 4, in_bytes = fbytes + n * 8 + n * 4;
    (void)hipSetDevice(e->device);
    std::lock_guard<std::mutex> lk(e->mu);
    DBuf &din = e->d_crf[0], &dtb = e->d_crf[1], &dpath = e->d_crf[2], &dsc = e->d_crf[3];
    bool ok = false;
    do {
        if (e->h_crf_in.ensure(in_bytes) || e->h_crf_out.ensure(((size_t)ncol + n) * 4 + n * 4) || din.ensure(in_bytes) || dtb.ensure((size_t)ncol * 4) ||
            dpath.ensure(((size_t)ncol + n) * 4) || dsc.ensure(n * 4)) break;
        char *h = e->h_crf_in.as<char>();
        long long *coff = (long long *)(h + fbytes);
        int *Ts = (int *)(h + fbytes + n * 8);
        long long c = 0;
        for (size_t k = 0; k < n; k++) {
            const size_t T = reqs[k]->trans->nc;
            memcpy(h + (size_t)c * stride * 4, reqs[k]->trans->data.f, T * stride * 4);
            coff[k] = c; Ts[k] = (int)T; c += (long long)T;
        }
        hipStream_t s = e->stream;
        if (hipMemcpyAsync(din.p, h, in_bytes, hipMemcpyHostToDevice, s) != hipSuccess) break;
        const char *d = din.as<char>();
        hipLaunchKernelGGL(k_crf_viterbi_batch, dim3((unsigned)((n + 63) / 64)), dim3(64), 0, s, (const float *)d, (int)stride, (const long long *)(d + fbytes),
                           (const int *)(d + fbytes + n * 8), (int)n, dtb.as<unsigned>(), dpath.as<int>(), dsc.as<float>());
        int *hp = e->h_crf_out.as<int>();
        if (hipMemcpyAsync(hp, dpath.p, ((size_t)ncol + n) * 4, hipMemcpyDeviceToHost, s) != hipSuccess) break;
        if (hipMemcpyAsync(hp + ncol + n, dsc.p, n * 4, hipMemcpyDeviceToHost, s) != hipSuccess) break;
        if (sh_stream_wait(s) != hipSuccess) break;
        const float *hs = (const float *)(hp + ncol + n);
        for (size_t k = 0; k < n; k++) {
            memcpy(reqs[k]->path, hp + coff[k] + (long long)k, ((size_t)Ts[k] + 1) * 4);
            reqs[k]->score = hs[k];
        }
        ok = true;
    } while (0);
    if (!ok) { (void)hipGetLastError(); for (CrfReq *r : reqs) r->score = NAN; }
}

static float coalesced_decode_crf(scrappie_hip_engine *e, const_scrappie_matrix trans, int *path) {
    constexpr size_t MAX_READS = 4096;
    constexpr long long MAX_COLS = 4000000;
    ShInside inside(g_presence);
    CrfReq r;
    r.trans = trans; r.path = path;
    g_cc.run(r, g_presence, MAX_READS, false,
        [&](std::deque<CrfReq *> &q, std::vector<CrfReq *> &batch) {
            take_compatible(q, batch, MAX_READS, MAX_COLS, [](const CrfReq *f, const CrfReq *c) { return c->trans->stride == f->trans->stride; },
                            [](const CrfReq *c) { return (long long)c->trans->nc; });
        },
// ... 22 lines not shown
```

### scrappie_amd/csrc/sh_sched.h

```cpp
#ifndef SH_SCHED_H
#define SH_SCHED_H
#include <algorithm>
#include <vector>

struct ShGruSeg { int tile, s0, s1, pad; };

struct ShGruSchedule {
    int nwg = 0;
    int capacity = 0;
    std::vector<int> lane_off;
    std::vector<ShGruSeg> seg;
    std::vector<int> wg_iter;
};

static inline void sh_lane_schedule(const int *tile_T, size_t ntile, int ncu, int lpw, ShGruSchedule &out,
                                    bool allow_split = true) {
    out = ShGruSchedule();
    std::vector<int> live;
    long long W = 0;
    int maxT = 0;
    for (size_t t = 0; t < ntile; t++) if (tile_T[t] > 0) { live.push_back((int)t); W += tile_T[t]; maxT = std::max(maxT, tile_T[t]); }
    if (live.empty()) { out.lane_off.assign(1, 0); return; }
    const long long nlive = (long long)live.size();
    const int nwg = (int)std::min<long long>(ncu, nlive);
    const int L = lpw * nwg;
    std::vector<std::vector<ShGruSeg>> pos(L);
    int M;
    if (nlive <= L) {
        M = maxT;
        std::vector<int> bylen(live);
        std::stable_sort(bylen.begin(), bylen.end(), [&](int x, int y) { return tile_T[x] > tile_T[y]; });
        for (long long i = 0; i < nlive; i++) {
            const int sub = (int)(i / nwg), j = (int)(i % nwg);
            const int wg = (sub & 1) ? (int)std::min<long long>(nwg, nlive - (long long)sub * nwg) - 1 - j : j;
            const int t = bylen[i];
            pos[L - 1 - (wg * lpw + sub)].push_back({t, 0, tile_T[t], 0});
        }
    } else if (!allow_split) {
        std::vector<int> load(L, 0);
        for (long long i = 0; i < nlive; i++) {
            const int p = (int)(std::min_element(load.begin(), load.end()) - load.begin());
            pos[p].push_back({live[i], 0, tile_T[live[i]], 0});
            load[p] += tile_T[live[i]];
        }
        M = *std::max_element(load.begin(), load.end());
    } else {
        M = (int)std::max<long long>(maxT, (W + L - 1) / L);
        int p = 0, used = 0;
        for (int t : live) {
            const int T = tile_T[t];
            const int room = M - used;
            if (T <= room) {
                pos[p].push_back({t, 0, T, 0});
                used += T;
            } else {
                if (room > 0) pos[p].push_back({t, T - room, T, 0});
                p++;
                pos[p].push_back({t, 0, T - room, 0});
                used = T - room;
            }
            if (used == M && p + 1 < L) { p++; used = 0; }
        }
    }
    out.nwg = nwg; out.capacity = M;
    out.lane_off.assign(L + 1, 0);
    out.wg_iter.assign(nwg, 0);
    for (int ln = 0; ln < L; ln++) {
        const std::vector<ShGruSeg> &v = pos[L - 1 - ln];
        int steps = 0;
        for (const ShGruSeg &sg : v) { out.seg.push_back(sg); steps += sg.s1 - sg.s0; }
        out.lane_off[ln + 1] = (int)out.seg.size();
        out.wg_iter[ln / lpw] = std::max(out.wg_iter[ln / lpw], steps);
    }
}
static inline void sh_gru_schedule(const int *tile_T, size_t ntile, int ncu, ShGruSchedule &out) {
    sh_lane_schedule(tile_T, ntile, ncu, 2, out);
}

static inline int sh_pieces_per_tile(long long nlive, int ncu) {
    if (nlive <= ncu) return 1;
    int best = 1;
    double bestv = 1e30;
    for (int k = 1; k <= 4; k++) {
        const double v = (double)((nlive * k + ncu - 1) / ncu) / k;
        if (v < bestv - 1e-9) { bestv = v; best = k; }
    }
    return best;
}
static inline void sh_piece_schedule(const int *tile_T, size_t ntile, int ncu, std::vector<ShGruSeg> &seg,
                                     bool allow_split = true) {
    seg.clear();
    long long nlive = 0;
    for (size_t t = 0; t < ntile; t++) nlive += tile_T[t] > 0;
    const int K = allow_split ? sh_pieces_per_tile(nlive, ncu) : 1;
    for (int k = 0; k < K; k++)
        for (size_t t = 0; t < ntile; t++) {
            const int T = tile_T[t];
            if (T <= 0) continue;
            const int len = (T + K - 1) / K;
            const int s0 = std::min(T, k * len), s1 = std::min(T, (k + 1) * len);
            if (s1 > s0) seg.push_back({(int)t, s0, s1, k});
        }
}
#endif
```

Baseline: 1.632 billion.

## Schedule fused decoder teams as persistent lanes over multiple tile segments

The fused ff+viterbi teams kernel now loops over a list of segments per workgroup, read through a lane_off table, instead of handling exactly one piece per block. A new sh_decoder_lanes scheduler packs tile time-steps in pairs into at most ncu workgroups with balanced splits, and the pipeline launches that many workgroups when the teams path is used. Kernel arguments are reread from the kernarg segment on each iteration, and some register init hints are added. The goal is fewer blocks and less tail imbalance and launch overhead. The cost is extra per-segment prologue and barriers, and more sequential handover between split pieces.

```diff
diff --git a/include/scrappie_hip.h b/include/scrappie_hip.h
--- a/include/scrappie_hip.h
+++ b/include/scrappie_hip.h
@@ -392,6 +392,7 @@
                                 int *lane_off, int *seg, size_t cap);
 
 long scrappie_hip_decoder_pieces(const int *tile_T, size_t ntile, int ncu, int *seg, size_t cap);
+long scrappie_hip_decoder_lanes(const int *tile_T, size_t ntile, int ncu, int *nwg, int *capacity, int *lane_off, int *seg, size_t cap);
 
 size_t scrappie_hip_min_samples(scrappie_hip_engine *e, int model);
 int scrappie_hip_model_stride(scrappie_hip_engine *e, int model);
diff --git a/scrappie_amd/csrc/scrappie_hip.hip b/scrappie_amd/csrc/scrappie_hip.hip
--- a/scrappie_amd/csrc/scrappie_hip.hip
+++ b/scrappie_amd/csrc/scrappie_hip.hip
@@ -208,6 +208,10 @@
     int gru32_nwg = 0;
     int gru32x2_nwg = 0;
     int vit_nwg = 0;
+    int vit_lane_nwg = 0;
+    int vit_lane_nseg = 0;
+    int vit_launched = 0;
+    int vit_launched_wg = 0;
     const float *d_signal = nullptr;
     std::vector<uint64_t> in_off;
     std::vector<uint32_t> in_len;
@@ -338,6 +342,7 @@
     bool dbg_dwell_tight = false;
     int dbg_gru_tiles = 0;
     int dbg_decoder_cus = 0;
+    int dbg_decoder_lanes = 0;
     bool dbg_force_f32 = false;
     int dbg_gru32 = -1;
     scrappie_hip_engine *tail = nullptr;
diff --git a/scrappie_amd/csrc/sh_decode.h b/scrappie_amd/csrc/sh_decode.h
--- a/scrappie_amd/csrc/sh_decode.h
+++ b/scrappie_amd/csrc/sh_decode.h
@@ -17,6 +17,7 @@
     const long long *hp_off;
     unsigned long long *dbg;
     const ShGruSegD *seg;
+    const int *lane_off;
     float *vstate;
     unsigned *flag;
     unsigned *err;
diff --git a/scrappie_amd/csrc/sh_decode_teams.h b/scrappie_amd/csrc/sh_decode_teams.h
--- a/scrappie_amd/csrc/sh_decode_teams.h
+++ b/scrappie_amd/csrc/sh_decode_teams.h
@@ -35,7 +35,7 @@
 #define SH_FVT_LDS_FLOATS (1024 * 16 + 64 * 256 + 2 * 64 * 16 + 2 * 2 * 8 * 16 + 4 * 9 * 16 + 65 * 16 + 2 * 3 * 512 + 3 * 2 * 4 * 4 + 16 * 4 + 4 * 16)
 
 template <bool SKIP0, bool DIV, bool NOCLAMP = false>
-__global__ __launch_bounds__(SH_FVT_NTH) void k_ff_viterbi_teams(ShFfArgs f, ShVitArgs a, ShMeta md) {
+__global__ __launch_bounds__(SH_FVT_NTH) void k_ff_viterbi_teams(ShFfArgs f_, ShVitArgs a_, ShMeta md_) {
     static_assert(!(DIV && NOCLAMP), "with temperatures the clamp stays");
     constexpr int NCW = 8, NPW = 4, PPT = 8, NQ = 256, NH = 1024, KS = 3, KQ = 6, TPP = 16, HT = 8, NG = 9, WB = SH_FVT_WBUF;
     static_assert(SH_SUM_GROUP == HT, "half a pass of a producer is one row-sum group");
@@ -57,26 +57,57 @@
     int *pT = (int *)(pendl + 16);
     long long *phpo = (long long *)(pT + 16);
 
-    const int tid = threadIdx.x, lane = tid & 63, b = lane & 15, q = lane >> 4;
-    const int wave = __builtin_amdgcn_readfirstlane(tid >> 6);
+    const int wave_ = __builtin_amdgcn_readfirstlane(threadIdx.x >> 6);
+    unsigned long long vA = 0, vB = 0, vC = 0, vD = 0, vt0 = 0, vt1 = 0, vP = 0, vp0 = 0;
+    unsigned vblk = 0, vseg = 0;
+    (void)vt0; (void)vt1; (void)vP; (void)vp0;
+#undef VSTAMP
+#undef VSTAMP_SEG
+#undef VSTAMP_LOOP
+#if SH_FVT_STAMP
+#define VSTAMP(acc) do { if (a.dbg) { vt1 = __builtin_readcyclecounter(); acc += vt1 - vt0; vt0 = vt1; } } while (0)
+#define VSTAMP_SEG() do { if (a.dbg) vp0 = __builtin_readcyclecounter(); } while (0)
+#define VSTAMP_LOOP() do { if (a.dbg) vP += vt0 - vp0; } while (0)
+#else
+#define VSTAMP(acc) do { } while (0)
+#define VSTAMP_SEG() do { } while (0)
+#define VSTAMP_LOOP() do { } while (0)
+#endif
+
+    if (threadIdx.x < KS * 2 * 4 * 4) { const int j = threadIdx.x; sStay[j] = f_.wpiece[(long long)(64) * KS * 512 + (j >> 4) * 256 + ((j >> 2) & 3) * 64 + (j & 3)]; }
+    for (int j = threadIdx.x; j < 65 * 16; j += SH_FVT_NTH) sBias[j] = f_.bfrag[((j >> 4) * 64 + ((j >> 2) & 3) * 16) * 4 + (j & 3)];
+
+#define SH_FVT_MT(i) (16 * ((i) >> 1) + 8 * ((i) & 1))
+    int sgi = blockIdx.x, sge = blockIdx.x + 1;
+    if (a_.lane_off) { sgi = a_.lane_off[blockIdx.x]; sge = a_.lane_off[blockIdx.x + 1]; }
+    sgi = __builtin_amdgcn_readfirstlane(sgi); sge = __builtin_amdgcn_readfirstlane(sge);
+    for (int si = sgi; si < sge; si++) {
+    if (si > sgi) __syncthreads();
+    typedef const __attribute__((address_space(4))) char *kargp;
+    kargp ka = (kargp)__builtin_amdgcn_kernarg_segment_ptr();
+    asm volatile("" : "+s"(ka));
+    constexpr size_t KA_A = (sizeof(ShFfArgs) + 7) & ~(size_t)7, KA_MD = (KA_A + sizeof(ShVitArgs) + 7) & ~(size_t)7;
+    static_assert(alignof(ShFfArgs) == 8 && alignof(ShVitArgs) == 8 && alignof(ShMeta) == 8, "kernarg layout");
+    const __attribute__((address_space(4))) ShFfArgs &f = *(const __attribute__((address_space(4))) ShFfArgs *)ka;
+    const __attribute__((address_space(4))) ShVitArgs &a = *(const __attribute__((address_space(4))) ShVitArgs *)(ka + KA_A);
+    const __attribute__((address_space(4))) ShMeta &md = *(const __attribute__((address_space(4))) ShMeta *)(ka + KA_MD);
+    VSTAMP_SEG();
+    int wave = wave_;
+    asm volatile("" : "+s"(wave));
     const bool decoder = wave < NCW;
+    int lane = (int)__builtin_amdgcn_mbcnt_hi(~0u, __builtin_amdgcn_mbcnt_lo(~0u, 0u));
+    asm volatile("" : "+v"(lane));
+    lane &= 63;
+    const int tid = wave * 64 + lane, b = lane & 15, q = lane >> 4;
     const float mp = a.min_prob, mpm1 = 1.0f - a.min_prob;
     const float lbound = (mp > 0.0f) ? 1.0e-3f - __logf(mp) : INFINITY;
     const float lbgap = lbound * SH_FVT_GAP;
-    unsigned long long vA = 0, vB = 0, vC = 0, vD = 0, vt0 = 0, vt1 = 0;
-    (void)vt0; (void)vt1;
-#undef VSTAMP
-#if SH_FVT_STAMP
-#define VSTAMP(acc) do { if (a.dbg) { vt1 = __builtin_readcyclecounter(); acc += vt1 - vt0; vt0 = vt1; } } while (0)
-#else
-#define VSTAMP(acc) do { } while (0)
-#endif
-
-    if (tid < KS * 2 * 4 * 4) sStay[tid] = f.wpiece[(long long)(64) * KS * 512 + (tid >> 4) * 256 + ((tid >> 2) & 3) * 64 + (tid & 3)];
-    for (int j = tid; j < 65 * 16; j += SH_FVT_NTH) sBias[j] = f.bfrag[((j >> 4) * 64 + ((j >> 2) & 3) * 16) * 4 + (j & 3)];
-
-    int tile = blockIdx.x, s0 = 0, s1 = -1, ord = 0;
-    if (a.seg) { const ShGruSegD sg = a.seg[blockIdx.x]; tile = sg.tile; s0 = sg.s0; s1 = sg.s1; ord = sg.pad; }
+    const int cw = decoder ? wave : 0;
+    float *myq = sc + cw * 256 + lane * 4;
+    const float *mye = ring + cw * 512 + lane * 4;
+    const float *mysrc = sc + cw * 64 + b * 4 + q;
+    int tile = si, s0 = 0, s1 = -1, ord = 0;
+    if (a.seg) { const ShGruSegD sg = a.seg[si]; tile = sg.tile; s0 = sg.s0; s1 = sg.s1; ord = sg.pad; }
     tile = __builtin_amdgcn_readfirstlane(tile); s0 = __builtin_amdgcn_readfirstlane(s0); s1 = __builtin_amdgcn_readfirstlane(s1);
     const int Tt = __builtin_amdgcn_readfirstlane(md.tile_T[tile]);
     if (s1 < 0) s1 = Tt;
@@ -86,12 +117,7 @@
     asm volatile("" : "+v"(myT));
     const long long hpo = a.hp_side ? a.hp_off[rd] : 0;
     float pstart = 0.0f, pend = -SH_BIG;
-
-    const int cw = decoder ? wave : 0;
-    float *myq = sc + cw * 256 + lane * 4;
-    const float *mye = ring + cw * 512 + lane * 4;
-    const float *mysrc = sc + cw * 64 + b * 4 + q;
-#define SH_FVT_MT(i) (16 * ((i) >> 1) + 8 * ((i) & 1))
+    vblk += (unsigned)(s1 - s0); vseg++;
 
     if (s0 == 0) {
         if (decoder) {
@@ -137,6 +163,10 @@
 #endif
         const unsigned *wmine = f.wpiece + (long long)(TPP * pw) * KS * 512;
         ShSplit W[WB][KS];
+#pragma unroll
+        for (int k = 0; k < WB; k++)
+#pragma unroll
+            for (int ks = 0; ks < KS; ks++) asm volatile("" : "=v"(W[k][ks].p1), "=v"(W[k][ks].p2));
         const unsigned lofs = (unsigned)lane * 4u;
         typedef const __attribute__((address_space(1))) unsigned *gu32;
         typedef const __attribute__((address_space(1))) u32x4 *gu32x4;
@@ -160,6 +190,7 @@
         };
         const int xks = pw < KS ? pw : KS - 1;
         f32x4 xr[2][2];
+        asm volatile("" : "=v"(xr[0][0]), "=v"(xr[0][1]), "=v"(xr[1][0]), "=v"(xr[1][1]));
         auto xraw_load = [&](int u) {
 #pragma unroll
             for (int j = 0; j < 2; j++) {
@@ -271,7 +302,11 @@
             if (low) *(f32x4 *)(rec + b * 4) = (f32x4){rm, mpx, stay_v, hold};
             float ev; int ei;
             end_unkey(redk[par * 16 + b], ev, ei);
-            redk[par * 16 + b] = 0;
+            {
+                unsigned zl, zh;
+                asm volatile("v_mov_b32 %0, 0\n\tv_mov_b32 %1, 0" : "=v"(zl), "=v"(zh));
+                redk[par * 16 + b] = ((unsigned long long)zh << 32) | zl;
+            }
             const f32x4 q4 = *(const f32x4 *)(sc + ((ei & (NQ - 1)) * 16 + b) * 4);
             int e0 = 3;
             e0 = (q4[2] - a.local_pen == ev) ? 2 : e0;
@@ -301,6 +336,7 @@
         if (any) { s1_half(H1, s0); __builtin_amdgcn_sched_barrier(0); xraw_load(s0 + 2); }
         lds_barrier();
         if (a.dbg) vt0 = __builtin_readcyclecounter();
+        VSTAMP_LOOP();
         for (int t = s0; t < s1; t += 2) {
             const bool more = (t + 2 < s1) && !(SH_FVT_ABL & 1);
             if (serial) { per_read(t, H0); __builtin_amdgcn_sched_barrier(0); }
@@ -328,11 +364,12 @@
         if (s1 < Tt) __builtin_amdgcn_fence(__ATOMIC_RELEASE, "agent");
         __syncthreads();
         if (s1 >= Tt) __syncthreads();
-        if (a.dbg && lane == 0) { unsigned long long *d = a.dbg + ((long long)blockIdx.x * 12 + wave) * 8; d[0] = vA; d[1] = vB; d[2] = vC; d[3] = vD; d[4] = (unsigned long long)(s1 - s0); }
-        return;
+        continue;
     }
     {
         f32x4 eN[2][PPT];
+#pragma unroll
+        for (int i = 0; i < PPT; i++) asm volatile("" : "=v"(eN[0][i]), "=v"(eN[1][i]));
         auto drain = [&](auto a0, auto s0c, auto a1, auto s1c) {
             constexpr int A0 = decltype(a0)::value, S0 = decltype(s0c)::value, A1 = decltype(a1)::value, S1 = decltype(s1c)::value;
 #pragma unroll
@@ -347,6 +384,7 @@
         lds_barrier();
         lds_barrier();
         if (a.dbg) vt0 = __builtin_readcyclecounter();
+        VSTAMP_LOOP();
         const unsigned tofs = (unsigned)lane;
         auto block = [&](const int t, auto first_c) {
             constexpr bool FIRST = decltype(first_c)::value;
@@ -574,8 +612,11 @@
             if (tid < 16) { vst[NH * 16 + b] = pstart; vst[NH * 16 + 16 + b] = pend; }
         }
     }
-    if (a.dbg && lane == 0) { unsigned long long *d = a.dbg + ((long long)blockIdx.x * 12 + wave) * 8; d[0] = vA; d[1] = vB; d[2] = vC; d[3] = vD; d[4] = (unsigned long long)(s1 - s0); }
+    }
+    if (a_.dbg && (threadIdx.x & 63) == 0) { unsigned long long *d = a_.dbg + ((long long)blockIdx.x * 12 + wave_) * 8; d[0] = vA; d[1] = vB; d[2] = vC; d[3] = vD; d[4] = vblk; d[5] = vP; d[6] = vseg; }
 #undef VSTAMP
+#undef VSTAMP_SEG
+#undef VSTAMP_LOOP
 #undef SH_FVT_MT
 }
 
diff --git a/scrappie_amd/csrc/sh_eng_batch.inc b/scrappie_amd/csrc/sh_eng_batch.inc
--- a/scrappie_amd/csrc/sh_eng_batch.inc
+++ b/scrappie_amd/csrc/sh_eng_batch.inc
@@ -60,7 +60,7 @@
 }
 static void sync_helper(scrappie_hip_engine *e, scrappie_hip_engine *t) {
     t->handover = e->handover; t->max_launch_reads = e->max_launch_reads; t->max_launch_blocks = e->max_launch_blocks;
-    t->dbg_ff_separate = e->dbg_ff_separate; t->dbg_fv_single = e->dbg_fv_single; t->dbg_gru32 = e->dbg_gru32; t->dbg_gru_tiles = e->dbg_gru_tiles; t->dbg_decoder_cus = e->dbg_decoder_cus; t->dbg_redo_all = e->dbg_redo_all;
+    t->dbg_ff_separate = e->dbg_ff_separate; t->dbg_fv_single = e->dbg_fv_single; t->dbg_gru32 = e->dbg_gru32; t->dbg_gru_tiles = e->dbg_gru_tiles; t->dbg_decoder_cus = e->dbg_decoder_cus; t->dbg_decoder_lanes = e->dbg_decoder_lanes; t->dbg_redo_all = e->dbg_redo_all;
     t->profiling = false;
 }
 static scrappie_hip_engine *tail_engine(scrappie_hip_engine *e) {
diff --git a/scrappie_amd/csrc/sh_eng_debug.inc b/scrappie_amd/csrc/sh_eng_debug.inc
--- a/scrappie_amd/csrc/sh_eng_debug.inc
+++ b/scrappie_amd/csrc/sh_eng_debug.inc
@@ -25,6 +25,7 @@
     else if (!strcmp(name, "dwell_tight")) e->dbg_dwell_tight = value != 0;
     else if (!strcmp(name, "gru_tiles")) e->dbg_gru_tiles = value;
     else if (!strcmp(name, "decoder_cus")) e->dbg_decoder_cus = value > 0 ? value : 0;
+    else if (!strcmp(name, "decoder_lanes")) e->dbg_decoder_lanes = value > 0 ? value : 0;
     else if (!strcmp(name, "force_f32_layers")) e->dbg_force_f32 = value != 0;
 #ifdef SH_EXPERIMENTS
     else if (!strcmp(name, "gru32")) e->dbg_gru32 = value;
@@ -68,7 +69,8 @@
     else if (!strcmp(what, "n_tail_calls")) { src = &e->n_tail_calls; have = 8; host = true; }
     else if (!strcmp(what, "n_tail_reads")) { src = &e->n_tail_reads; have = 8; host = true; }
     else if (!strcmp(what, "gru_tiles")) { src = &gru_tiles; have = 4; host = true; }
-    else if (!strcmp(what, "decoder_pieces")) { src = &lg.vit_nwg; have = 4; host = true; }
+    else if (!strcmp(what, "decoder_pieces")) { src = &lg.vit_launched; have = 4; host = true; }
+    else if (!strcmp(what, "decoder_wgs")) { src = &lg.vit_launched_wg; have = 4; host = true; }
     else if (!strcmp(what, "pinned_bytes")) {
         static thread_local unsigned long long tot;
         tot = e->slots[0].pinned_bytes() + e->slots[1].pinned_bytes();
diff --git a/scrappie_amd/csrc/sh_eng_launch.inc b/scrappie_amd/csrc/sh_eng_launch.inc
--- a/scrappie_amd/csrc/sh_eng_launch.inc
+++ b/scrappie_amd/csrc/sh_eng_launch.inc
@@ -1,5 +1,5 @@
 
-struct MetaPtrs { ShMeta md; const long long *seq_off, *hp_off, *bases_off; ShGruLanes lanes, lanes1; ShGruPairs pairs, pairs2; const ShGruSegD *vseg; ShDwellArgs dw; };
+struct MetaPtrs { ShMeta md; const long long *seq_off, *hp_off, *bases_off; ShGruLanes lanes, lanes1; ShGruPairs pairs, pairs2; const ShGruSegD *vseg, *vlseg; const int *vloff; ShDwellArgs dw; };
 
 #define SH_DWELL_PER_ENTRY 10
 static long long bases_reservation(long long per_entry, long long nentry) { return (per_entry * nentry + 16 + 15) & ~15ll; }
@@ -82,13 +82,18 @@
     std::vector<ShGruSeg> vseg;
     sh_piece_schedule(tile_T.data(), lg.ntile, e->dbg_decoder_cus > 0 ? e->dbg_decoder_cus : e->ncu, vseg, e->handover);
     lg.vit_nwg = (int)vseg.size();
+    ShGruSchedule vlanes;
+    if (e->dbg_decoder_cus > 0 && e->dbg_decoder_lanes <= 0) sh_pieces_as_lanes(vseg, vlanes);
+    else sh_decoder_lanes(tile_T.data(), lg.ntile, e->dbg_decoder_lanes > 0 ? e->dbg_decoder_lanes : e->ncu, vlanes, e->handover);
+    lg.vit_lane_nwg = vlanes.nwg; lg.vit_lane_nseg = (int)vlanes.seg.size();
     const size_t b_u64 = lg.npad * 8, b_i32 = lg.npad * 4;
     const size_t b_loff = sched.lane_off.size() * 4, b_seg = sched.seg.size() * sizeof(ShGruSeg), b_wit = sched.wg_iter.size() * 4;
-    const size_t b_vloff = 0, b_vseg = vseg.size() * sizeof(ShGruSeg);
+    const size_t b_vseg = vseg.size() * sizeof(ShGruSeg);
+    const size_t b_vloff = vlanes.lane_off.size() * 4, b_vlseg = vlanes.seg.size() * sizeof(ShGruSeg);
     const size_t b_loff1 = sched1.lane_off.size() * 4, b_seg1 = sched1.seg.size() * sizeof(ShGruSeg);
     const size_t b_loff32 = sched32.lane_off.size() * 4, b_seg32 = sched32.seg.size() * sizeof(ShGruSeg), b_pt = pair_tile.size() * 4;
     const size_t b_loff32b = sched32b.lane_off.size() * 4, b_seg32b = sched32b.seg.size() * sizeof(ShGruSeg);
-    const size_t total = 4 * b_u64 + lg.ntile * 8 + 2 * b_i32 + lg.ntile * 4 + 16 + b_seg + b_loff + b_wit + 16 + b_vseg + b_vloff + 16 + b_seg1 + b_loff1 +
+    const size_t total = 4 * b_u64 + lg.ntile * 8 + 2 * b_i32 + lg.ntile * 4 + 16 + b_seg + b_loff + b_wit + 16 + b_vseg + 16 + b_vlseg + b_vloff + 16 + b_seg1 + b_loff1 +
                          16 + b_seg32 + b_loff32 + b_pt + 16 + b_seg32b + b_loff32b;
     if (sl.h_meta.ensure(total + 16) || sl.d_meta.ensure(total + 16)) return -1;
     char *h = sl.h_meta.as<char>();
@@ -107,6 +112,9 @@
     memcpy(h + o, sched.wg_iter.data(), b_wit); const size_t o_wit = o; o += b_wit;
     o = (o + 15) & ~(size_t)15;
     memcpy(h + o, vseg.data(), b_vseg); const size_t o_vseg = o; o += b_vseg;
+    o = (o + 15) & ~(size_t)15;
+    memcpy(h + o, vlanes.seg.data(), b_vlseg); const size_t o_vlseg = o; o += b_vlseg;
+    memcpy(h + o, vlanes.lane_off.data(), b_vloff); const size_t o_vloff = o; o += b_vloff;
     o = (o + 15) & ~(size_t)15;
     memcpy(h + o, sched1.seg.data(), b_seg1); const size_t o_seg1 = o; o += b_seg1;
     memcpy(h + o, sched1.lane_off.data(), b_loff1); const size_t o_loff1 = o; o += b_loff1;
@@ -137,6 +145,8 @@
     mp.lanes.wg_iter = (const int *)(d + o_wit);
     mp.lanes.ntile = (int)lg.ntile;
     mp.vseg = (const ShGruSegD *)(d + o_vseg);
+    mp.vlseg = (const ShGruSegD *)(d + o_vlseg);
+    mp.vloff = (const int *)(d + o_vloff);
     if (e->d_hstate.ensure(std::max<size_t>(lg.ntile, 1) * 12 * 256 * 4) || sl.d_gflag.ensure((lg.ntile + 1) * 4)) return -1;
     mp.lanes.hstate = e->d_hstate.as<float>();
     mp.lanes.flag = sl.d_gflag.as<unsigned>();
diff --git a/scrappie_amd/csrc/sh_eng_load.inc b/scrappie_amd/csrc/sh_eng_load.inc
--- a/scrappie_amd/csrc/sh_eng_load.inc
+++ b/scrappie_amd/csrc/sh_eng_load.inc
@@ -324,6 +324,17 @@
     return (long)v.size();
 }
 
+extern "C" long scrappie_hip_decoder_lanes(const int *tile_T, size_t ntile, int ncu, int *nwg, int *capacity, int *lane_off, int *seg, size_t cap) {
+    if (!tile_T || ncu < 1) return -1;
+    ShGruSchedule sc;
+    sh_decoder_lanes(tile_T, ntile, ncu, sc);
+    if (nwg) *nwg = sc.nwg;
+    if (capacity) *capacity = sc.capacity;
+    if (lane_off) memcpy(lane_off, sc.lane_off.data(), sc.lane_off.size() * sizeof(int));
+    if (seg) for (size_t i = 0; i < sc.seg.size() && i < cap; i++) memcpy(seg + 4 * i, &sc.seg[i], 16);
+    return (long)sc.seg.size();
+}
+
 extern "C" long scrappie_hip_plan_groups(const uint32_t *lengths, size_t n, int stride, size_t max_reads, size_t max_blocks,
                                          size_t *starts, size_t cap) {
     if ((!lengths && n) || stride < 1 || max_reads < 1) return -1;
diff --git a/scrappie_amd/csrc/sh_eng_pipeline.inc b/scrappie_amd/csrc/sh_eng_pipeline.inc
--- a/scrappie_amd/csrc/sh_eng_pipeline.inc
+++ b/scrappie_amd/csrc/sh_eng_pipeline.inc
@@ -288,7 +288,11 @@
     if (tun().vit_stamp) va.dbg = vst.dev(4096 * 16 * 8);
     if (e->d_vstate.ensure(std::max<size_t>(lg.ntile, 1) * ((size_t)NH * 16 + 32) * 4) || e->d_vflag.ensure(std::max<size_t>(lg.ntile, 1) * 4)) return -1;
     HIPCHK(hipMemsetAsync(e->d_vflag.p, 0, std::max<size_t>(lg.ntile, 1) * 4, s));
-    va.seg = mp.vseg;
+    va.seg = mp.vseg; va.lane_off = nullptr;
+    const bool teams = fused && !p->use_slip && !(tun().fv_single || e->dbg_fv_single);
+    if (teams) { va.seg = mp.vlseg; va.lane_off = mp.vloff; }
+    const int vit_nwg = teams ? lg.vit_lane_nwg : lg.vit_nwg;
+    lg.vit_launched = teams ? lg.vit_lane_nseg : lg.vit_nwg; lg.vit_launched_wg = vit_nwg;
     va.vstate = e->d_vstate.as<float>(); va.flag = e->d_vflag.as<unsigned>(); va.err = sl.d_gflag.as<unsigned>() + lg.ntile;
     if (e->ev_ok && e->other(sl).pending) HIPCHK(hipStreamWaitEvent(s, e->other(sl).done, 0));
     if (fused) {
@@ -297,11 +301,16 @@
         fa.in_div = p->tempW / p->tempb; fa.out_div = p->tempb;
         fa.no_clamp = (m->ff_no_clamp && !e->alt_trunk) ? 1 : 0;
         va.E = nullptr; va.sums = nullptr;
-        if (launch_ff_viterbi(s, fa, va, mp.md, (size_t)lg.vit_nwg, tun().fv_single || e->dbg_fv_single)) return -1;
-    } else if (launch_viterbi(s, NH, va, mp.md, (size_t)lg.vit_nwg)) return -1;
-    if (va.dbg) vst.dump_on(0, s, (size_t)std::max(lg.vit_nwg, 1) * 16 * 8, [&](const unsigned long long *h) {
-        const int nwv = (fused && !va.use_slip && !(tun().fv_single || e->dbg_fv_single)) ? 12 : 8;
-        for (int w = 0; w < nwv; w++) { const unsigned long long *d = &h[((size_t)(lg.vit_nwg / 2) * nwv + w) * 8]; fprintf(stderr, "vit stamp wave %d: phaseB %.0f bar %.0f phaseC %.0f bar %.0f cycles/block\n", w, d[0] / (double)d[4], d[1] / (double)d[4], d[2] / (double)d[4], d[3] / (double)d[4]); }
+        if (launch_ff_viterbi(s, fa, va, mp.md, (size_t)vit_nwg, !teams)) return -1;
+    } else if (launch_viterbi(s, NH, va, mp.md, (size_t)vit_nwg)) return -1;
+    if (va.dbg) vst.dump_on(0, s, (size_t)std::max(vit_nwg, 1) * 16 * 8, [&](const unsigned long long *h) {
+        const int nwv = teams ? 12 : 8;
+        for (int w = 0; w < nwv; w++) {
+            const unsigned long long *d = &h[((size_t)(vit_nwg / 2) * nwv + w) * 8];
+            fprintf(stderr, "vit stamp wave %d: phaseB %.0f bar %.0f phaseC %.0f bar %.0f cycles/block", w, d[0] / (double)d[4], d[1] / (double)d[4], d[2] / (double)d[4], d[3] / (double)d[4]);
+            if (teams && d[6]) fprintf(stderr, "; %llu blocks in %llu segments, prologue %.0f cycles/segment", d[4], d[6], d[5] / (double)d[6]);
+            fprintf(stderr, "\n");
+        }
     });
     if (c.pf.mark(Marks::DECODE_END, s)) return -1;
     c.pf.span(F_DECODE, Marks::S1_END, Marks::DECODE_END);
diff --git a/scrappie_amd/csrc/sh_eng_surface.inc b/scrappie_amd/csrc/sh_eng_surface.inc
--- a/scrappie_amd/csrc/sh_eng_surface.inc
+++ b/scrappie_amd/csrc/sh_eng_surface.inc
@@ -323,7 +323,7 @@
         va.tb = dtb.as<unsigned>(); va.tb_end = dtbe.as<int>();
         va.final_state = dfs.as<int>(); va.final_score = dfsc.as<float>();
         va.hp_side = nullptr; va.hp_off = nullptr; va.dbg = nullptr; va.dump_final = 0;
-        va.seg = nullptr; va.vstate = nullptr; va.flag = nullptr; va.err = nullptr;
+        va.seg = nullptr; va.lane_off = nullptr; va.vstate = nullptr; va.flag = nullptr; va.err = nullptr;
         if (launch_viterbi(s, NH, va, md, n)) break;
         hipLaunchKernelGGL(k_backtrace_lane0, dim3((unsigned)((n + 63) / 64)), dim3(64), 0, s, dtb.as<unsigned>(), dtbe.as<int>(), dfs.as<int>(), md,
                            (const long long *)(d + npad * 8), dseq.as<int>(), (int)n, NQ);
diff --git a/scrappie_amd/csrc/sh_sched.h b/scrappie_amd/csrc/sh_sched.h
--- a/scrappie_amd/csrc/sh_sched.h
+++ b/scrappie_amd/csrc/sh_sched.h
@@ -102,4 +102,25 @@
             if (s1 > s0) seg.push_back({(int)t, s0, s1, k});
         }
 }
+
+static inline void sh_decoder_lanes(const int *tile_T, size_t ntile, int ncu, ShGruSchedule &out, bool allow_split = true) {
+    std::vector<int> pairs(ntile);
+    for (size_t t = 0; t < ntile; t++) pairs[t] = tile_T[t] > 0 ? (tile_T[t] + 1) / 2 : 0;
+    sh_lane_schedule(pairs.data(), ntile, ncu, 1, out, allow_split);
+    out.capacity *= 2;
+    for (int &w : out.wg_iter) w *= 2;
+    for (ShGruSeg &sg : out.seg) {
+        sg.s0 *= 2;
+        sg.s1 = std::min(2 * sg.s1, tile_T[sg.tile]);
+        sg.pad = sg.s0 > 0 ? 1 : 0;
+    }
+}
+static inline void sh_pieces_as_lanes(const std::vector<ShGruSeg> &piece, ShGruSchedule &out) {
+    out = ShGruSchedule();
+    out.nwg = (int)piece.size();
+    out.seg = piece;
+    out.lane_off.resize(piece.size() + 1);
+    for (size_t i = 0; i <= piece.size(); i++) out.lane_off[i] = (int)i;
+    for (const ShGruSeg &sg : piece) { out.wg_iter.push_back(sg.s1 - sg.s0); out.capacity = std::max(out.capacity, sg.s1 - sg.s0); }
+}
 #endif
```

New measurement: 1.653 billion, median of 6. 1.01x the previous value.
